# wolfbox/snappy

Measured on AMD Instinct MI355X. Metric: GiB/s hashed (whole node), bit-exact hashes.yaml, 10k x 1 MiB tree, higher is better.
Workload: dtype u64; 1 GPU; C2: ONE on-disk tree (tmpfs) of 10001 files (10 000 x 1 MiB + the 1 MiB archive stand-in) -> hashes.yaml, sharded over 1 rank(s) on 1 distinct GPU(s); bytes=10486808576, kernel=sha512_split_kernel<true>, tree_home=/dev/shm

## Files before the change

### snappy_amd/csrc/hostfill.cpp

```cpp
#include "hostfill.h"

#include <new>

#include <ctype.h>
#include <dirent.h>
#include <errno.h>
#include <sched.h>
#include <stdio.h>
#include <string.h>
#include <sys/syscall.h>
#include <unistd.h>

#include <algorithm>
#include <atomic>

#if defined(__x86_64__)
#include <immintrin.h>
#endif

namespace snaphash {

namespace {

bool read_small_file(const std::string& path, std::string& out)
{
    FILE* f = fopen(path.c_str(), "r");
    if (!f) return false;
    char buf[4096];
    out.clear();
    size_t r;
    while ((r = fread(buf, 1, sizeof buf, f)) > 0) out.append(buf, r);
    fclose(f);
    return true;
}

constexpr int kMpolDefault = 0, kMpolPreferred = 1;
constexpr unsigned kMpolFNode = 1u << 0, kMpolFAddr = 1u << 1;

}

std::vector<int> parse_cpulist(const std::string& text)
{
    std::vector<int> out;
    const char* p = text.c_str();
    while (*p) {
        while (*p && !isdigit((unsigned char)*p)) ++p;
        if (!*p) break;
        char* end = nullptr;
        const long a = strtol(p, &end, 10);
        long b = a;
        p = end;
        if (*p == '-') { b = strtol(p + 1, &end, 10); p = end; }
        if (a < 0 || b < a || b - a > 65536) break;
        for (long c = a; c <= b; ++c) out.push_back((int)c);
    }
    return out;
}

int numa_node_of_pci(const std::string& sysfs_root, const std::string& bdf_in)
{
    std::string bdf = bdf_in;
    for (char& c : bdf) c = (char)tolower((unsigned char)c);
    if (bdf.empty()) return -1;
    std::string text;
    if (!read_small_file(sysfs_root + "/bus/pci/devices/" + bdf + "/numa_node", text)) return -1;
    char* end = nullptr;
    const long v = strtol(text.c_str(), &end, 10);
    if (end == text.c_str()) return -1;
    return v < 0 ? -1 : (int)v;
}

std::vector<int> numa_cpus_of_node(const std::string& sysfs_root, int node)
{
    std::string text;
    if (node < 0 || !read_small_file(sysfs_root + "/devices/system/node/node" + std::to_string(node) + "/cpulist", text)) return {};
    return parse_cpulist(text);
}

std::vector<int> slice_cpus(const std::vector<int>& all, size_t pos, size_t m)
{
    if (m < 2 || pos >= m) return all;
    std::vector<int> mine;
    for (size_t a = 0; a < all.size();) {
        size_t b = a + 1;
        while (b < all.size() && all[b] == all[b - 1] + 1) ++b;
        const size_t len = b - a;
        for (size_t i = a + len * pos / m; i < a + len * (pos + 1) / m; ++i) mine.push_back(all[i]);
        a = b;
    }
    return mine;
}

int numa_node_count(const std::string& sysfs_root)
{
    int n = 0;
    if (DIR* d = opendir((sysfs_root + "/devices/system/node").c_str())) {
        while (struct dirent* de = readdir(d))
            if (!strncmp(de->d_name, "node", 4) && isdigit((unsigned char)de->d_name[4])) ++n;
        closedir(d);
    }
    return n;
}

bool numa_prefer_node(int node, SavedMemPolicy* saved)
{
#if defined(SYS_set_mempolicy) && defined(SYS_get_mempolicy)
    if (node < 0 || node >= 1024) return false;
    saved->valid = syscall(SYS_get_mempolicy, &saved->mode, saved->mask, (unsigned long)1024 + 1, nullptr, 0ul) == 0;
    unsigned long mask[1024 / (8 * sizeof(unsigned long))] = {0};
    mask[(size_t)node / (8 * sizeof(unsigned long))] |= 1ul << ((size_t)node % (8 * sizeof(unsigned long)));
    return syscall(SYS_set_mempolicy, kMpolPreferred, mask, (unsigned long)1024 + 1) == 0;
#else
    (void)node; (void)saved;
    return false;
#endif
}

void numa_restore_policy(const SavedMemPolicy& saved)
{
#if defined(SYS_set_mempolicy)
    if (saved.valid && saved.mode != kMpolDefault &&
        syscall(SYS_set_mempolicy, saved.mode, saved.mask, (unsigned long)1024 + 1) == 0)
        return;
    (void)syscall(SYS_set_mempolicy, kMpolDefault, nullptr, 0ul);
#else
    (void)saved;
#endif
}

int numa_node_of_address(const void* addr)
{
#if defined(SYS_get_mempolicy)
    int node = -1;
    if (syscall(SYS_get_mempolicy, &node, nullptr, 0ul, addr, (unsigned long)(kMpolFNode | kMpolFAddr)) != 0) return -1;
    return node;
#else
    (void)addr;
    return -1;
#endif
}

unsigned cgroup_cpu_quota(const std::string& sysfs_cgroup_root, const std::string& proc_self_cgroup)
{
    std::string text;
    if (!read_small_file(proc_self_cgroup, text)) return 0;
    double best = 0;
    auto take = [&](double quota, double period) {
        if (quota > 0 && period > 0) { const double c = quota / period; if (best == 0 || c < best) best = c; }
    };
    size_t pos = 0;
    while (pos < text.size()) {
        size_t eol = text.find('\n', pos);
        if (eol == std::string::npos) eol = text.size();
        const std::string line = text.substr(pos, eol - pos);
        pos = eol + 1;
        const size_t c1 = line.find(':'), c2 = c1 == std::string::npos ? c1 : line.find(':', c1 + 1);
        if (c2 == std::string::npos) continue;
        const std::string ctrl = line.substr(c1 + 1, c2 - c1 - 1);
        std::string path = line.substr(c2 + 1);
        const bool v2 = ctrl.empty();
        if (!v2) {
            bool has_cpu = false;
            for (size_t a = 0; a <= ctrl.size();) {
                size_t b = ctrl.find(',', a);
                if (b == std::string::npos) b = ctrl.size();
                if (ctrl.compare(a, b - a, "cpu") == 0) has_cpu = true;
                a = b + 1;
            }
            if (!has_cpu) continue;
        }
        const std::string base = sysfs_cgroup_root + (v2 ? "" : "/" + ctrl);
        for (;;) {
            std::string v;
            if (v2) {
                if (read_small_file(base + path + "/cpu.max", v) && v.compare(0, 3, "max") != 0) {
                    char* end = nullptr;
                    const double q = strtod(v.c_str(), &end);
                    const double per = end ? strtod(end, nullptr) : 0;
                    take(q, per);
                }
            } else {
                std::string pv;
                if (read_small_file(base + path + "/cpu.cfs_quota_us", v) && read_small_file(base + path + "/cpu.cfs_period_us", pv))
                    take(strtod(v.c_str(), nullptr), strtod(pv.c_str(), nullptr));
            }
            if (path.empty() || path == "/") break;
            const size_t slash = path.rfind('/');
            path = slash == 0 || slash == std::string::npos ? "/" : path.substr(0, slash);
        }
    }
    if (best <= 0) return 0;
    return (unsigned)std::max(1.0, best + 0.5);
}

unsigned usable_cpus()
{
    unsigned n = 0;
    cpu_set_t set;
    CPU_ZERO(&set);
    if (sched_getaffinity(0, sizeof set, &set) == 0) {
        const int c = CPU_COUNT(&set);
        if (c > 0) n = (unsigned)c;
    }
    if (n == 0) n = std::max(1u, std::thread::hardware_concurrency());
    static const unsigned quota = cgroup_cpu_quota("/sys/fs/cgroup", "/proc/self/cgroup");
    if (quota && quota < n) n = quota;
    return n;
}


FillPool::~FillPool() { stop(); }

void FillPool::stop()
{
    {
        std::lock_guard<std::mutex> lk(mu_);
        quit_ = true;
    }
    cv_work_.notify_all();
    for (auto& t : th_) if (t.joinable()) t.join();
    th_.clear();
    quit_ = false;
}

void FillPool::configure(unsigned max_threads, const std::vector<int>& cpus)
{
    stop();
    max_threads_ = max_threads;
    cpus_ = cpus;
}

void FillPool::worker(unsigned id)
{
    if (!cpus_.empty()) {
        cpu_set_t set, allowed;
        CPU_ZERO(&set);
        CPU_ZERO(&allowed);
        const bool have_allowed = sched_getaffinity(0, sizeof allowed, &allowed) == 0;
        for (int c : cpus_)
            if (c >= 0 && c < CPU_SETSIZE && (!have_allowed || CPU_ISSET(c, &allowed))) CPU_SET(c, &set);
        if (CPU_COUNT(&set) > 0) (void)sched_setaffinity(0, sizeof set, &set);
    }
    uint64_t seen = 0;
    for (;;) {
        const std::function<void(size_t)>* fn;
        size_t n;
        std::atomic<size_t>* next;
        {
            std::unique_lock<std::mutex> lk(mu_);
            cv_work_.wait(lk, [&] { return quit_ || (epoch_ != seen && id < want_); });
            if (quit_) return;
            seen = epoch_;
            fn = fn_; n = n_; next = next_;
        }
        try {
            for (;;) {
                const size_t i = next->fetch_add(1);
                if (i >= n) break;
                (*fn)(i);
            }
        } catch (...) {
            fn_threw_.store(true);
        }
        {
            std::lock_guard<std::mutex> lk(mu_);
            if (--running_ == 0) cv_done_.notify_all();
        }
    }
}

void FillPool::parallel_for(size_t n, unsigned threads, const std::function<void(size_t)>& fn)
{
    if (n == 0) return;
    unsigned helpers = threads > 1 ? std::min(threads - 1, max_threads_) : 0u;
    if (helpers > n - 1) helpers = (unsigned)(n - 1);
    std::atomic<size_t> next{0};
    if (helpers) {
        std::lock_guard<std::mutex> lk(mu_);
        try {
            while (th_.size() < helpers) { const unsigned id = (unsigned)th_.size(); th_.emplace_back(&FillPool::worker, this, id); }
        } catch (...) {
            helpers = (unsigned)th_.size();
        }
        if (helpers) {
            fn_ = &fn; n_ = n; next_ = &next;
            want_ = helpers;
            running_ = helpers;
            ++epoch_;
        }
    }
    if (helpers) cv_work_.notify_all();
    bool threw = false;
    try {
        for (;;) {
            const size_t i = next.fetch_add(1);
            if (i >= n) break;
            fn(i);
        }
    } catch (...) {
        threw = true;
        next.store(n);
    }
    if (helpers) {
        std::unique_lock<std::mutex> lk(mu_);
        cv_done_.wait(lk, [&] { return running_ == 0; });
        want_ = 0;
        fn_ = nullptr; next_ = nullptr;
    }
    if (fn_threw_.exchange(false) || threw) throw std::bad_alloc();
}


void run_on_threads(unsigned T, const std::function<void(unsigned)>& fn)
{
    if (T <= 1) { fn(0); return; }
    static std::mutex mu;
    static FillPool* pool = [] {
        FillPool* p = new FillPool();
        p->configure(64, {});
        return p;
    }();
    static const pid_t born_in = getpid();
    if (T <= 65 && getpid() == born_in && mu.try_lock()) {
        std::lock_guard<std::mutex> lk(mu, std::adopt_lock);
        pool->parallel_for(T, T, [&fn](size_t t) { fn((unsigned)t); });
        return;
    }
    ThreadJoiner th;
    for (unsigned t = 1; t < T; ++t) th.spawn(fn, t);
    fn(0);
    th.join_all();
}


#if defined(__x86_64__)
namespace {
__attribute__((target("avx2"))) void copy_nt_avx2(uint8_t* dst, const uint8_t* src, size_t n)
{
    const size_t head = (64 - ((uintptr_t)dst & 63)) & 63;
    if (head) { memcpy(dst, src, head); dst += head; src += head; n -= head; }
    size_t lines = n / 64;
    while (lines--) {
        const __m256i a = _mm256_loadu_si256((const __m256i*)src);
        const __m256i b = _mm256_loadu_si256((const __m256i*)(src + 32));
        _mm256_stream_si256((__m256i*)dst, a);
        _mm256_stream_si256((__m256i*)(dst + 32), b);
        src += 64; dst += 64;
    }
    n &= 63;
    if (n) memcpy(dst, src, n);
    _mm_sfence();
}
const bool g_have_avx2 = __builtin_cpu_supports("avx2");
}
#endif

void copy_to_staging(void* dst, const void* src, size_t n)
{
#if defined(__x86_64__)
    if (n >= (32u << 10) && g_have_avx2) { copy_nt_avx2((uint8_t*)dst, (const uint8_t*)src, n); return; }
#endif
    memcpy(dst, src, n);
}

}
```

### snappy_amd/csrc/hostfill.h

```cpp
#pragma once
#include <stddef.h>
#include <stdint.h>

#include <atomic>
#include <condition_variable>
#include <functional>
#include <mutex>
#include <new>
#include <string>
#include <thread>
#include <vector>

namespace snaphash {

int numa_node_of_pci(const std::string& sysfs_root, const std::string& bdf);
std::vector<int> numa_cpus_of_node(const std::string& sysfs_root, int node);
std::vector<int> parse_cpulist(const std::string& text);
int numa_node_count(const std::string& sysfs_root);
std::vector<int> slice_cpus(const std::vector<int>& all, size_t pos, size_t m);

struct SavedMemPolicy {
    bool valid = false;
    int mode = 0;
    unsigned long mask[1024 / (8 * sizeof(unsigned long)) + 1] = {0};
};
bool numa_prefer_node(int node, SavedMemPolicy* saved);
void numa_restore_policy(const SavedMemPolicy& saved);
int numa_node_of_address(const void* addr);
unsigned usable_cpus();
unsigned cgroup_cpu_quota(const std::string& sysfs_cgroup_root, const std::string& proc_self_cgroup);

struct ThreadJoiner {
    std::vector<std::thread> th;
    std::atomic<bool> worker_threw{false};
    ThreadJoiner() = default;
    ThreadJoiner(const ThreadJoiner&) = delete;
    ThreadJoiner& operator=(const ThreadJoiner&) = delete;
    ~ThreadJoiner() { join_quietly(); }
    template <class F, class... A> void spawn(F&& f, A&&... a)
    {
        th.emplace_back([this](auto fn, auto... args) {
            try { fn(args...); } catch (...) { worker_threw.store(true); }
        }, std::forward<F>(f), std::forward<A>(a)...);
    }
    void join_quietly()
    {
        for (auto& t : th)
            if (t.joinable()) t.join();
    }
    void join_all()
    {
        join_quietly();
        if (worker_threw.exchange(false)) throw std::bad_alloc();
    }
};

class FillPool {
public:
    FillPool() = default;
    ~FillPool();
    FillPool(const FillPool&) = delete;
    FillPool& operator=(const FillPool&) = delete;
    void configure(unsigned max_threads, const std::vector<int>& cpus);
    void parallel_for(size_t n, unsigned threads, const std::function<void(size_t)>& fn);
    unsigned max_threads() const { return max_threads_; }
    const std::vector<int>& cpus() const { return cpus_; }

private:
    void worker(unsigned id);
    void stop();
    unsigned max_threads_ = 0;
    std::vector<int> cpus_;
    std::vector<std::thread> th_;
    std::mutex mu_;
    std::condition_variable cv_work_, cv_done_;
    uint64_t epoch_ = 0;
    unsigned want_ = 0;
    unsigned running_ = 0;
    bool quit_ = false;
    const std::function<void(size_t)>* fn_ = nullptr;
    std::atomic<bool> fn_threw_{false};
    size_t n_ = 0;
    std::atomic<size_t>* next_ = nullptr;
};

void run_on_threads(unsigned T, const std::function<void(unsigned)>& fn);

void copy_to_staging(void* dst, const void* src, size_t n);

}
```

### snappy_amd/csrc/hostpass.cpp

```cpp
#include "hostpass.h"

#include "hostfill.h"
#include "walk.h"

#include <dirent.h>
#include <errno.h>
#include <string.h>
#include <sys/stat.h>

#include <algorithm>
#include <string_view>
#include <functional>
#include <queue>
#include <thread>

namespace snaphash {


int mode_string(uint32_t st_mode, char out[11])
{
    memcpy(out, "----------", 11);
    if (S_ISDIR(st_mode)) out[0] = 'd';
    else if (S_ISLNK(st_mode)) out[0] = 'l';
    else if (S_ISREG(st_mode)) out[0] = 'f';
    else return SNAPHASH_EMODE;
    static const char rwx[] = "rwxrwxrwx";
    for (int i = 0; i < 9; ++i)
        if (st_mode & (1u << (8 - i))) out[i + 1] = rwx[i];
    return SNAPHASH_OK;
}

int mode_parse(const char* s, uint32_t* st_mode)
{
    if (!s || !s[0]) return SNAPHASH_EPARSE;
    uint32_t m;
    switch (s[0]) {
    case 'd': m = S_IFDIR; break;
    case 'f': m = S_IFREG; break;
    case 'l': m = S_IFLNK; break;
    default: return SNAPHASH_EPARSE;
    }
    static const char rwx[] = "rwxrwxrwx";
    for (int i = 0; i < 9 && s[i + 1]; ++i)
        if (s[i + 1] == rwx[i]) m |= 1u << (8 - i);
    *st_mode = m;
    return SNAPHASH_OK;
}


static int records_from_entries_impl(std::vector<WalkEntry>& ents, std::vector<Record>& out, bool steal)
{
    if (ents.empty()) return SNAPHASH_OK;
    const size_t rootlen = ents[0].path.size();
    const size_t n = ents.size();
    const unsigned T = (unsigned)std::max<size_t>(1, std::min<size_t>(std::min(8u, usable_cpus()), n / 2048));
    std::vector<uint8_t> keep(n, 0);
    std::vector<size_t> kept(T + 1, 0), bad(T, n);
    auto range = [&](unsigned t, size_t& lo, size_t& hi) { lo = n * t / T; hi = n * (t + 1) / T; };
    run_on_threads(T, [&](unsigned t) {
        size_t lo, hi, c = 0;
        range(t, lo, hi);
        for (size_t i = lo; i < hi; ++i) {
            const char* rel = ents[i].path.c_str() + rootlen;
            if (rel[0] == 0 || strncmp(rel, "/DEBIAN", 7) == 0) continue;
            char m[11];
            if (mode_string(ents[i].st.st_mode, m) != SNAPHASH_OK) { bad[t] = i; break; }
            keep[i] = 1;
            ++c;
        }
        kept[t + 1] = c;
    });
    size_t first_bad = n;
    for (unsigned t = 0; t < T; ++t) first_bad = std::min(first_bad, bad[t]);
    if (first_bad < n) return SNAPHASH_EMODE;
    for (unsigned t = 0; t < T; ++t) kept[t + 1] += kept[t];
    const size_t base = out.size();
    out.resize(base + kept[T]);
    run_on_threads(T, [&](unsigned t) {
        size_t lo, hi;
        range(t, lo, hi);
        size_t at = base + kept[t];
        for (size_t i = lo; i < hi; ++i) {
            if (!keep[i]) continue;
            WalkEntry& e = ents[i];
            Record& r = out[at++];
            r.name.assign(e.path.c_str() + rootlen + 1, e.path.size() - rootlen - 1);
            r.st_mode = e.st.st_mode;
            r.is_regular = S_ISREG(e.st.st_mode);
            r.size = r.is_regular ? (int64_t)e.st.st_size : 0;
            if (steal) r.path = std::move(e.path);
            else r.path = e.path;
        }
    });
    return SNAPHASH_OK;
}

size_t first_unemittable_name(const std::vector<Record>& recs)
{
    const size_t n = recs.size();
    const unsigned T = (unsigned)std::max<size_t>(1, std::min<size_t>(std::min(8u, usable_cpus()), n / 2048));
    std::vector<size_t> bad(T, n);
    run_on_threads(T, [&](unsigned t) {
        for (size_t i = n * t / T; i < n * (t + 1) / T; ++i)
            if (!name_emittable(recs[i].name)) { bad[t] = i; break; }
    });
    size_t first = n;
    for (size_t b : bad) first = std::min(first, b);
    return first;
}

int records_from_entries(const std::vector<WalkEntry>& ents, std::vector<Record>& out)
{
    return records_from_entries_impl(const_cast<std::vector<WalkEntry>&>(ents), out, false);
}

int walk_tree(const char* build_dir, std::vector<Record>& out, int* err_no)
{
    std::vector<WalkEntry> ents;
    int e = 0;
    const int wrc = walk_entries(build_dir, ents, &e, nullptr);
    if (err_no) *err_no = e;
    const int rc = records_from_entries_impl(ents, out, true);
    if (rc) return rc;
    return wrc ? SNAPHASH_EIO : SNAPHASH_OK;
}


bool plain_safe_name(const std::string& s)
{
    if (s.empty() || s.size() > 72) return false;
    bool alpha = false;
    for (unsigned char c : s) {
        const bool ok = (c >= 'a' && c <= 'z') || (c >= 'A' && c <= 'Z') || (c >= '0' && c <= '9') || c == '_' ||
                        c == '.' || c == '/' || c == '-' || c == '+';
        if (!ok) return false;
        if ((c >= 'a' && c <= 'z') || (c >= 'A' && c <= 'Z')) alpha = true;
    }
    const unsigned char c0 = s[0];
    if (c0 == '-' || c0 == '.' || c0 == '+' || (c0 >= '0' && c0 <= '9')) return false;
    if (!alpha) return false;
    static const char* const resolved[] = {"y", "Y", "yes", "Yes", "YES", "on", "On", "ON", "n", "N", "no", "No", "NO",
                                           "off", "Off", "OFF", "true", "True", "TRUE", "false", "False", "FALSE",
                                           "null", "Null", "NULL", nullptr};
    if (s.size() <= 5)
        for (int i = 0; resolved[i]; ++i)
            if (s == resolved[i]) return false;
    return true;
}

void hex_lower(const uint8_t d[64], char out[128])
{
    static const char x[] = "0123456789abcdef";
    for (int i = 0; i < 64; ++i) { out[2 * i] = x[d[i] >> 4]; out[2 * i + 1] = x[d[i] & 15]; }
}

static int emit_records(const std::vector<Record>& recs, size_t lo, size_t hi, const uint8_t* file_digests, std::string& out,
                        std::vector<size_t>* hex_at = nullptr)
{
    char hex[128], num[32];
    size_t fi = 0;
    if (hex_at) memset(hex, '0', sizeof hex);
    for (size_t k = lo; k < hi; ++k) {
        const Record& r = recs[k];
        char mode[11];
        int rc = mode_string(r.st_mode, mode);
        if (rc) return rc;
        out += "- name:";
        if (plain_safe_name(r.name)) { out += ' '; out += r.name; }
        else if ((rc = yaml_append_name_scalar(r.name, 7, 4, out)) != SNAPHASH_OK) return rc;
        out += '\n';
        if (r.is_regular) {
            snprintf(num, sizeof num, "%lld", (long long)r.size);
            out += "  size: "; out += num; out += '\n';
            if (!hex_at) hex_lower(file_digests + 64 * fi++, hex);
            out += "  sha512: ";
            if (hex_at) hex_at->push_back(out.size());
            out.append(hex, 128); out += '\n';
        }
        out += "  mode: "; out.append(mode, 10); out += '\n';
    }
    return SNAPHASH_OK;
}

static int emit_yaml_impl(const std::vector<Record>& recs, const uint8_t* archive_digest, const uint8_t* file_digests,
                          std::string& out, std::vector<size_t>* hex_at, unsigned max_threads = 8)
{
    char hex[128];
    out.clear();
    out.reserve(64 + recs.size() * 220);
    if (hex_at) { hex_at->clear(); memset(hex, '0', sizeof hex); }
    else hex_lower(archive_digest, hex);
    out += "archive-sha512: ";
    if (hex_at) hex_at->push_back(out.size());
    out.append(hex, 128);
    out += '\n';
    if (recs.empty()) {
        out += "files: []\n";
        return SNAPHASH_OK;
    }
    out += "files:\n";
    const unsigned T = (unsigned)std::max<size_t>(1, std::min<size_t>(std::min(std::max(1u, max_threads), usable_cpus()), recs.size() / 1024));
    if (T <= 1) return emit_records(recs, 0, recs.size(), file_digests, out, hex_at);
    std::vector<size_t> first_digest(T + 1, 0);
    {
        size_t fi = 0;
        for (unsigned t = 0; t < T; ++t) {
            first_digest[t] = fi;
            for (size_t k = recs.size() * t / T; k < recs.size() * (t + 1) / T; ++k) fi += recs[k].is_regular ? 1 : 0;
        }
    }
    std::vector<std::string> piece(T);
    std::vector<std::vector<size_t>> piece_at(hex_at ? T : 0);
    std::vector<int> prc(T, 0);
    auto work = [&](unsigned t) {
        const size_t lo = recs.size() * t / T, hi = recs.size() * (t + 1) / T;
        piece[t].reserve((hi - lo) * 220);
        prc[t] = emit_records(recs, lo, hi, file_digests ? file_digests + 64 * first_digest[t] : nullptr, piece[t], hex_at ? &piece_at[t] : nullptr);
    };
    run_on_threads(T, work);
    for (unsigned t = 0; t < T; ++t) {
        if (prc[t]) return prc[t];
        if (hex_at)
            for (size_t at : piece_at[t]) hex_at->push_back(out.size() + at);
        out += piece[t];
    }
    return SNAPHASH_OK;
}

int emit_yaml(const std::vector<Record>& recs, const uint8_t archive_digest[64], const uint8_t* file_digests,
              std::string& out)
{
    return emit_yaml_impl(recs, archive_digest, file_digests, out, nullptr);
}

int emit_yaml_skeleton(const std::vector<Record>& recs, YamlSkeleton& sk, unsigned max_threads)
{
    return emit_yaml_impl(recs, nullptr, nullptr, sk.text, &sk.hex_at, max_threads);
}

void yaml_fill_digests(YamlSkeleton& sk, const uint8_t archive_digest[64], const uint8_t* file_digests)
{
    if (sk.hex_at.empty()) return;
    hex_lower(archive_digest, &sk.text[sk.hex_at[0]]);
    const size_t n = sk.hex_at.size() - 1;
    const unsigned T = (unsigned)std::max<size_t>(1, std::min<size_t>(std::min(8u, usable_cpus()), n / 2048));
    auto work = [&](unsigned t) {
        for (size_t i = n * t / T; i < n * (t + 1) / T; ++i) hex_lower(file_digests + 64 * i, &sk.text[sk.hex_at[i + 1]]);
    };
    run_on_threads(T, work);
}


namespace {
constexpr uint32_t kListMagic = 0x4c504e53u;
struct BlobOut {
    std::string b;
    void u32(uint32_t v) { b.append((const char*)&v, 4); }
    void u64(uint64_t v) { b.append((const char*)&v, 8); }
};
struct BlobIn {
    const uint8_t* p;
    size_t n, at = 0;
    bool ok = true;
    uint32_t u32() { uint32_t v = 0; if (at + 4 > n) { ok = false; return 0; } memcpy(&v, p + at, 4); at += 4; return v; }
    uint64_t u64() { uint64_t v = 0; if (at + 8 > n) { ok = false; return 0; } memcpy(&v, p + at, 8); at += 8; return v; }
    const char* bytes(size_t k) { if (k > n - at || at > n) { ok = false; return nullptr; } const char* r = (const char*)p + at; at += k; return r; }
};
bool list_root(const std::string& root, std::vector<std::string>& names)
{
    names.clear();
    DIR* d = opendir(root.c_str());
    if (!d) return false;
    while (struct dirent* de = readdir(d)) {
        if (!strcmp(de->d_name, ".") || !strcmp(de->d_name, "..")) continue;
        names.emplace_back(de->d_name);
    }
    closedir(d);
    std::sort(names.begin(), names.end());
    return true;
}
uint64_t hash_names(const std::vector<std::string>& names)
{
    uint64_t h = 0x9E3779B97F4A7C15ull;
    for (const std::string& s : names)
        for (size_t i = 0; i <= s.size(); ++i) { h = (h ^ (uint8_t)(i < s.size() ? s[i] : 0)) * 0xFF51AFD7ED558CCDull; h ^= h >> 29; }
    return h;
}
}


int shard_listing(const char* build_dir, uint32_t rank, uint32_t world, std::string& blob, int* err_no)
{
    if (err_no) *err_no = 0;
    std::string root(build_dir);
    while (root.size() > 1 && root.back() == '/') root.pop_back();
    struct stat rst;
    if (lstat(root.c_str(), &rst) != 0) { if (err_no) *err_no = errno; return SNAPHASH_EIO; }
    std::vector<std::string> top;
    if (S_ISDIR(rst.st_mode)) (void)list_root(root, top);
    std::vector<uint32_t> mine;
    for (size_t i = 0; i < top.size(); ++i)
        if (i % world == rank) mine.push_back((uint32_t)i);
    std::vector<std::vector<WalkEntry>> sub(mine.size());
    std::vector<int> sub_rc(mine.size(), 0), sub_errno(mine.size(), 0);
    const unsigned T = (unsigned)std::max<size_t>(1, std::min<size_t>(std::min(16u, usable_cpus()), mine.size()));
    std::atomic<size_t> next{0};
    run_on_threads(T, [&](unsigned) {
        for (;;) {
            const size_t k = next.fetch_add(1);
            if (k >= mine.size()) return;
            const std::string& name = top[mine[k]];
            if (name.compare(0, 6, "DEBIAN") == 0) continue;
            sub_rc[k] = walk_entries((root + "/" + name).c_str(), sub[k], &sub_errno[k], nullptr);
        }
    });
    for (size_t k = 0; k < mine.size(); ++k)
        if (sub_rc[k]) { if (err_no) *err_no = sub_errno[k]; return SNAPHASH_EIO; }
    BlobOut o;
    o.u32(kListMagic); o.u32(1); o.u32(world); o.u32(rank); o.u32((uint32_t)top.size()); o.u32((uint32_t)mine.size());
    o.u64(hash_names(top));
    const size_t cut = root.size() + 1;
    for (size_t k = 0; k < mine.size(); ++k) {
        o.u32(mine[k]);
        o.u32((uint32_t)sub[k].size());
        for (const WalkEntry& e : sub[k]) {
            o.u32((uint32_t)e.st.st_mode);
            o.u32((uint32_t)(e.path.size() - cut));
            o.u64(S_ISREG(e.st.st_mode) ? (uint64_t)e.st.st_size : 0);
            o.b.append(e.path, cut, std::string::npos);
        }
    }
    blob.swap(o.b);
    return SNAPHASH_OK;
}

int records_from_listings(const char* build_dir, uint32_t world, const void* const* blobs, const size_t* blob_lens, std::vector<Record>& recs)
{
    std::string root(build_dir);
    while (root.size() > 1 && root.back() == '/') root.pop_back();
    struct Piece { uint32_t r = 0; size_t at = 0; uint32_t n = 0; bool have = false; };
    std::vector<Piece> piece;
    uint32_t n_top = 0;
    uint64_t names_hash = 0;
    for (uint32_t r = 0; r < world; ++r) {
        if (!blobs[r] && blob_lens[r]) return SNAPHASH_EINVAL;
        BlobIn in{(const uint8_t*)blobs[r], blob_lens[r]};
        const uint32_t magic = in.u32(), version = in.u32(), w = in.u32(), rk = in.u32(), nt = in.u32(), nm = in.u32();
        const uint64_t nh = in.u64();
        if (!in.ok || magic != kListMagic || version != 1 || w != world || rk != r) return SNAPHASH_EPARSE;
        if (r == 0) {
            if (nt > (1u << 26)) return SNAPHASH_EPARSE;
            n_top = nt; names_hash = nh; piece.assign(n_top, Piece());
        } else if (nt != n_top || nh != names_hash) return SNAPHASH_EMISMATCH;
        for (uint32_t k = 0; k < nm; ++k) {
            const uint32_t i = in.u32(), ne = in.u32();
            if (!in.ok || i >= n_top || i % world != r || piece[i].have) return SNAPHASH_EPARSE;
            piece[i].r = r; piece[i].at = in.at; piece[i].n = ne; piece[i].have = true;
            for (uint32_t e = 0; e < ne; ++e) {
                (void)in.u32();
                const uint32_t len = in.u32();
                (void)in.u64();
                (void)in.bytes(len);
                if (!in.ok) return SNAPHASH_EPARSE;
            }
        }
        if (in.at != in.n) return SNAPHASH_EPARSE;
    }
    std::vector<size_t> first(n_top + 1, 0);
    for (uint32_t i = 0; i < n_top; ++i) { if (!piece[i].have) return SNAPHASH_EPARSE; first[i + 1] = first[i] + piece[i].n; }
    const size_t total = first[n_top];
    recs.clear();
    recs.resize(total);
    const unsigned T = (unsigned)std::max<size_t>(1, std::min<size_t>({(size_t)std::min(8u, usable_cpus()), total / 1024, (size_t)n_top}));
    std::vector<int> trc(T, SNAPHASH_OK);
    std::vector<size_t> tbad(T, (size_t)-1);
    run_on_threads(T, [&](unsigned t) {
        for (uint32_t i = (uint32_t)((uint64_t)n_top * t / T); i < (uint32_t)((uint64_t)n_top * (t + 1) / T); ++i) {
            BlobIn in{(const uint8_t*)blobs[piece[i].r], blob_lens[piece[i].r]};
            in.at = piece[i].at;
            for (uint32_t e = 0; e < piece[i].n; ++e) {
                const uint32_t mode = in.u32(), len = in.u32();
                const uint64_t size = in.u64();
                const char* name = in.bytes(len);
                int rc = SNAPHASH_OK;
                char m[11];
                if (!in.ok || len == 0 || memchr(name, 0, len)) rc = SNAPHASH_EPARSE;
                else if (mode_string(mode, m) != SNAPHASH_OK) rc = SNAPHASH_EMODE;
                if (rc) { trc[t] = rc; tbad[t] = first[i] + e; return; }
                Record& r = recs[first[i] + e];
                r.name.assign(name, len);
                r.path.reserve(root.size() + 1 + len);
                r.path = root;
                r.path += '/';
                r.path.append(name, len);
                r.st_mode = mode;
                r.is_regular = S_ISREG(mode);
                r.size = r.is_regular ? (int64_t)size : 0;
            }
        }
    });
    size_t bad = (size_t)-1;
    int rc = SNAPHASH_OK;
    for (unsigned t = 0; t < T; ++t)
        if (trc[t] && tbad[t] < bad) { bad = tbad[t]; rc = trc[t]; }
    if (rc) recs.clear();
    return rc;
}


namespace {

int hexval(int c)
{
    if (c >= '0' && c <= '9') return c - '0';
    if (c >= 'a' && c <= 'f') return c - 'a' + 10;
    if (c >= 'A' && c <= 'F') return c - 'A' + 10;
    return -1;
}

bool parse_scalar(const std::string& v, std::string& out)
{
    out.clear();
    if (v.empty()) return true;
    if (v[0] == '\'') {
        size_t i = 1;
        for (; i < v.size(); ++i) {
            if (v[i] == '\'') {
                if (i + 1 < v.size() && v[i + 1] == '\'') { out += '\''; ++i; continue; }
                break;
            }
            out += v[i];
        }
        return i < v.size();
    }
    if (v[0] == '"') {
        size_t i = 1;
        for (; i < v.size() && v[i] != '"'; ++i) {
            if (v[i] != '\\') { out += v[i]; continue; }
            if (++i >= v.size()) return false;
            switch (v[i]) {
            case 'n': out += '\n'; break;
            case 't': out += '\t'; break;
            case 'r': out += '\r'; break;
            case '0': out += '\0'; break;
            case 'a': out += '\a'; break;
            case 'b': out += '\b'; break;
            case 'e': out += '\x1b'; break;
            case 'f': out += '\f'; break;
            case 'v': out += '\v'; break;
            case ' ': out += ' '; break;
            case '"': out += '"'; break;
            case '/': out += '/'; break;
            case '\\': out += '\\'; break;
            case 'N': out += "\xC2\x85"; break;
            case '_': out += "\xC2\xA0"; break;
            case 'L': out += "\xE2\x80\xA8"; break;
            case 'P': out += "\xE2\x80\xA9"; break;
            case 'x': case 'u': case 'U': {
                const int nd = v[i] == 'x' ? 2 : (v[i] == 'u' ? 4 : 8);
                if (i + nd >= v.size()) return false;
                uint32_t cp = 0;
                for (int k = 0; k < nd; ++k) {
                    const int h = hexval(v[i + 1 + k]);
                    if (h < 0) return false;
                    cp = cp * 16 + h;
                }
                i += nd;
                if (cp < 0x80) out += (char)cp;
                else if (cp < 0x800) { out += (char)(0xC0 | (cp >> 6)); out += (char)(0x80 | (cp & 63)); }
                else if (cp < 0x10000) { out += (char)(0xE0 | (cp >> 12)); out += (char)(0x80 | ((cp >> 6) & 63)); out += (char)(0x80 | (cp & 63)); }
                else { out += (char)(0xF0 | (cp >> 18)); out += (char)(0x80 | ((cp >> 12) & 63)); out += (char)(0x80 | ((cp >> 6) & 63)); out += (char)(0x80 | (cp & 63)); }
                break;
            }
            default: return false;
            }
        }
        return i < v.size();
    }
    std::string p = v;
    size_t h = p.find(" #");
    if (h != std::string::npos) p.resize(h);
    while (!p.empty() && (p.back() == ' ' || p.back() == '\t' || p.back() == '\r')) p.pop_back();
    out = p;
    return true;
}

bool split_key(const std::string& line, size_t from, std::string& key, std::string& val)
{
    size_t c = line.find(':', from);
    if (c == std::string::npos) return false;
    key = line.substr(from, c - from);
    size_t v = c + 1;
    while (v < line.size() && line[v] == ' ') ++v;
    val = line.substr(v);
    while (!val.empty() && (val.back() == '\r' || val.back() == ' ')) val.pop_back();
    return true;
}

bool unhex64(const std::string& s, uint8_t out[64])
{
    if (s.size() != 128) return false;
    for (int i = 0; i < 64; ++i) {
        const int a = hexval(s[2 * i]), b = hexval(s[2 * i + 1]);
        if (a < 0 || b < 0) return false;
        out[i] = (uint8_t)(a * 16 + b);
    }
    return true;
}

}

namespace {

int parse_lines(const std::vector<std::string_view>& lines, size_t lo, size_t hi, bool in_files_at_start, ParsedHashes& out, bool* top_level)
{
    bool in_files = in_files_at_start;
    int skip_indent = -1;
    ParsedRecord* cur = nullptr;
    auto indent_of = [](std::string_view l) { size_t k = 0; while (k < l.size() && l[k] == ' ') ++k; return k; };
    std::string line;
    std::string key, val, sv;
    for (size_t li = lo; li < hi; ++li) {
        line.assign(lines[li].data(), lines[li].size());
        while (!line.empty() && (line.back() == '\r')) line.pop_back();
        size_t ind = 0;
        while (ind < line.size() && line[ind] == ' ') ++ind;
        if (in_files && (skip_indent < 0 || (int)ind <= skip_indent) && ind < line.size() && line[ind] != '#') {
            const size_t key_col = line[ind] == '-' ? ind + 2 : ind;
            const size_t colon = line.find(": ", ind);
            if (colon != std::string::npos && colon + 2 < line.size()) {
                while (li + 1 < hi) {
                    std::string_view nx = lines[li + 1];
                    while (!nx.empty() && (nx.back() == '\r' || nx.back() == ' ')) nx.remove_suffix(1);
                    const size_t ni = indent_of(nx);
                    if (nx.empty() || ni <= key_col) break;
                    while (!line.empty() && line.back() == ' ') line.pop_back();
                    line += ' ';
                    line.append(nx.data() + ni, nx.size() - ni);
                    ++li;
                }
            }
        }
        if (ind == line.size() || line[ind] == '#') continue;
        if (line == "---" || line == "...") continue;
        if (skip_indent >= 0) {
            if ((int)ind > skip_indent) continue;
            skip_indent = -1;
        }
        if (ind == 0 && line[0] != '-') {
            if (top_level) *top_level = true;
// ... 157 lines not shown
```

### snappy_amd/csrc/hostpass.h

```cpp
#pragma once
#include <stdint.h>
#include <stdio.h>

#include <string>
#include <vector>

#include "../../include/snaphash.h"

namespace snaphash {

struct Record {
    std::string name;
    std::string path;
    uint32_t st_mode = 0;
    bool is_regular = false;
    int64_t size = 0;
    std::string sha512_hex;
};

struct ParsedRecord {
    std::string name, sha512_hex;
    int64_t size = 0;
    uint32_t st_mode = 0;
    bool has_name = false, has_size = false, has_mode = false;
};
struct ParsedHashes {
    bool has_archive = false;
    std::string archive_hex;
    std::vector<ParsedRecord> files;
};

int mode_string(uint32_t st_mode, char out[11]);
int mode_parse(const char* s, uint32_t* st_mode);
int walk_tree(const char* build_dir, std::vector<Record>& out, int* err_no);
struct WalkEntry;
int records_from_entries(const std::vector<WalkEntry>& ents, std::vector<Record>& out);
bool plain_safe_name(const std::string& s);
int yaml_append_name_scalar(const std::string& s, int column, int indent, std::string& out);
bool name_emittable(const std::string& s);
size_t first_unemittable_name(const std::vector<Record>& recs);
void hex_lower(const uint8_t d[64], char out[128]);
int emit_yaml(const std::vector<Record>& recs, const uint8_t archive_digest[64], const uint8_t* file_digests,
              std::string& out);
struct YamlSkeleton {
    std::string text;
    std::vector<size_t> hex_at;
};
int emit_yaml_skeleton(const std::vector<Record>& recs, YamlSkeleton& out, unsigned max_threads = 8 );
void yaml_fill_digests(YamlSkeleton& sk, const uint8_t archive_digest[64], const uint8_t* file_digests);
int shard_listing(const char* build_dir, uint32_t rank, uint32_t world, std::string& blob, int* err_no);
int records_from_listings(const char* build_dir, uint32_t world, const void* const* blobs, const size_t* blob_lens, std::vector<Record>& recs);
int parse_yaml(const char* text, size_t len, ParsedHashes& out);
bool digest_matches_hex(const uint8_t d[64], const std::string& hex);
int lpt_assign(const uint64_t* lens, size_t n, int nshards, int32_t* shard_of);

}
```

### snappy_amd/csrc/snapbuild.inc

```

namespace {

constexpr uint32_t kSnapBuildOptionsSizeV1 = 16;

struct SnapBuildTemps {
    std::string data, control;
    ~SnapBuildTemps()
    {
        if (!data.empty()) (void)unlink(data.c_str());
        if (!control.empty()) (void)unlink(control.c_str());
    }
};

struct SnapOut {
    int fd = -1;
    HostSha sha;
    uint64_t bytes = 0;
    ~SnapOut() { if (fd >= 0) close(fd); }
    int put(const uint8_t* p, size_t n)
    {
        host_sha512_update(sha, p, n);
        bytes += n;
        size_t off = 0;
        while (off < n) {
            const ssize_t w = write(fd, p + off, n - off);
            if (w < 0) { if (errno == EINTR) continue; return errno; }
            off += (size_t)w;
        }
        return 0;
    }
};

int snap_put_member(snaphash_ctx* x, SnapOut& out, const char* name, int64_t mtime, const uint8_t* data, uint64_t size, const char* path)
{
    int fd = -1;
    struct FdGuard { int& fd; ~FdGuard() { if (fd >= 0) close(fd); } } guard{fd};
    if (path) {
        fd = open(path, O_RDONLY | O_CLOEXEC);
        struct stat sb;
        if (fd < 0 || fstat(fd, &sb) != 0) return fail(x, SNAPHASH_EIO, std::string(path) + ": " + strerror(errno));
        size = (uint64_t)sb.st_size;
    }
    uint8_t h[kArHeader];
    int rc = ar_header(name, mtime, 0100644, size, h);
    if (rc) return fail(x, rc, std::string("ar: member ") + name + " does not fit a header");
    int en = out.put(h, sizeof h);
    if (!en && !path && size) en = out.put(data, (size_t)size);
    if (!en && path) {
        std::vector<uint8_t> buf(4u << 20);
        uint64_t got = 0;
        while (got < size && !en) {
            const ssize_t r = read(fd, buf.data(), (size_t)std::min<uint64_t>(buf.size(), size - got));
            if (r < 0 && errno == EINTR) continue;
            if (r <= 0) return fail(x, SNAPHASH_EIO, std::string(path) + ": " + (r < 0 ? strerror(errno) : "shorter than it was"));
            en = out.put(buf.data(), (size_t)r);
            got += (uint64_t)r;
        }
    }
    if (!en && (size & 1)) en = out.put((const uint8_t*)"\n", 1);
    if (en) return fail(x, SNAPHASH_EIO, std::string("writing the container: ") + strerror(en));
    return SNAPHASH_OK;
}

struct SnapDataMember {
    Encoder& enc;
    const char* name;
    const uint64_t& check_units;
    const double& check_ms;
};

int snap_build_impl(snaphash_ctx* x, const char* source_dir, const char* snap_path, uint32_t flags, int64_t mtime, uint8_t* archive_digest,
                    uint8_t* snap_digest, snaphash_snap_build_stats& st, const SnapDataMember& dm)
{
    const double t0 = now_ms();
    const bool hashes = !(flags & SNAPHASH_BUILD_NO_HASHES);
    SnapBuildTemps tmp;
    SnapOut out;
    out.fd = open(snap_path, O_WRONLY | O_CREAT | O_TRUNC | O_CLOEXEC, 0666);
    if (out.fd < 0) return fail(x, SNAPHASH_EIO, std::string(snap_path) + ": " + strerror(errno));
    host_sha512_init(out.sha);
    tmp.data = std::string(snap_path) + "." + dm.name;
    tmp.control = std::string(snap_path) + ".control.tar.gz";
    const std::string debian = go_clean(std::string(source_dir) + "/DEBIAN");

    GzCheck chk_control;
    chk_control.member = "control.tar.gz";
    const bool check = (flags & SNAPHASH_BUILD_CHECK) != 0;
    uint8_t adig[64];
    char* yaml = nullptr;
    size_t yaml_len = 0;
    struct Free { char*& p; ~Free() { free(p); } } free_yaml{yaml};
    GzipEncoder enc_control(check ? &chk_control : nullptr);
    int rc = tar_create_impl(x, dm.enc, tmp.data.c_str(), source_dir, debian.c_str(), nullptr, nullptr, hashes ? &yaml : nullptr, &yaml_len, adig);
    if (rc) return rc;
    st.data_ms = x->targz.wall_ms;
    st.tar_bytes = x->targz.tar_bytes;
    st.members = x->targz.members;
    st.data_bytes = x->targz.gz_bytes;
    if (hashes) {
        rc = write_yaml_file(x, source_dir, std::string(yaml, yaml_len));
        if (rc) return rc;
    }
    rc = tar_create_impl(x, enc_control, tmp.control.c_str(), debian.c_str(), nullptr, nullptr, nullptr, nullptr, nullptr, nullptr);
    if (rc) return rc;
    st.control_ms = x->targz.wall_ms;
    st.control_bytes = x->targz.gz_bytes;
    st.check_chunks = dm.check_units + chk_control.chunks;
    st.check_ms = dm.check_ms + chk_control.ms;

    const double t_ar = now_ms();
    const int en = out.put((const uint8_t*)kArMagic, 8);
    if (en) return fail(x, SNAPHASH_EIO, std::string(snap_path) + ": " + strerror(en));
    rc = snap_put_member(x, out, "debian-binary", mtime, (const uint8_t*)"2.0\n", 4, nullptr);
    if (!rc) rc = snap_put_member(x, out, "_click-binary", mtime, (const uint8_t*)"0.4\n", 4, nullptr);
    if (!rc) rc = snap_put_member(x, out, "control.tar.gz", mtime, nullptr, 0, tmp.control.c_str());
    if (!rc) rc = snap_put_member(x, out, dm.name, mtime, nullptr, 0, tmp.data.c_str());
    if (rc) return rc;
    const int fd = out.fd;
    out.fd = -1;
    if (close(fd) != 0) return fail(x, SNAPHASH_EIO, std::string(snap_path) + ": " + strerror(errno));
    uint8_t sdig[64];
    host_sha512_final(out.sha, sdig);
    if (snap_digest) memcpy(snap_digest, sdig, 64);
    if (archive_digest) memcpy(archive_digest, adig, 64);
    st.snap_bytes = out.bytes;
    st.ar_ms = now_ms() - t_ar;
    st.wall_ms = now_ms() - t0;
    return SNAPHASH_OK;
}

}

extern "C" {

int snaphash_snap_build(snaphash_ctx* x, const char* source_dir, const char* snap_path, const snaphash_snap_build_options* opt,
                        uint8_t* archive_digest, uint8_t* snap_digest, snaphash_snap_build_stats* stats)
try {
    if (!x || !source_dir || !snap_path || !*snap_path) return fail(x, SNAPHASH_EINVAL, "bad argument");
    static_assert(offsetof(snaphash_snap_build_options, data_codec) == kSnapBuildOptionsSizeV1, "the codec and its options behind the 16 bytes");
    if (opt && opt->struct_size != kSnapBuildOptionsSizeV1 && opt->struct_size < sizeof(snaphash_snap_build_options))
        return fail(x, SNAPHASH_EINVAL, "snaphash_snap_build_options.struct_size");
    if (stats && stats->struct_size < sizeof(snaphash_snap_build_stats)) return fail(x, SNAPHASH_EINVAL, "snaphash_snap_build_stats.struct_size");
    const uint32_t flags = opt ? opt->flags : 0;
    if (flags & ~(uint32_t)(SNAPHASH_BUILD_NO_HASHES | SNAPHASH_BUILD_CHECK)) return fail(x, SNAPHASH_EINVAL, "unknown build flag");
    const int64_t mtime = (opt && opt->mtime >= 0) ? opt->mtime : (int64_t)time(nullptr);
    uint32_t codec = SNAPHASH_DATA_GZ;
    const snaphash_xz_options* xo = nullptr;
    const snaphash_bz2_options* bo = nullptr;
    if (opt && opt->struct_size >= sizeof(snaphash_snap_build_options)) {
        codec = opt->data_codec;
        xo = opt->xz;
        bo = opt->bz2;
        if (codec > SNAPHASH_DATA_XZ) return fail(x, SNAPHASH_EINVAL, "snap build: data_codec is 0 (gz), 1 (bz2) or 2 (xz)");
        if (opt->reserved) return fail(x, SNAPHASH_EINVAL, "snap build: snaphash_snap_build_options.reserved is not 0");
        if ((xo && codec != SNAPHASH_DATA_XZ) || (bo && codec != SNAPHASH_DATA_BZ2))
            return fail(x, SNAPHASH_EINVAL, "snap build: options for a codec that is not data_codec");
    }
    const bool check = (flags & SNAPHASH_BUILD_CHECK) != 0;
    snaphash_snap_build_stats st{};
    st.struct_size = sizeof st;
    auto build = [&](const SnapDataMember& dm) {
        const int rc = snap_build_impl(x, source_dir, snap_path, flags, mtime, archive_digest, snap_digest, st, dm);
        if (rc) (void)unlink(snap_path);
        if (stats) *stats = st;
        return rc;
    };
    if (codec == SNAPHASH_DATA_XZ) {
        uint64_t bs;
        uint32_t chk, filter, level;
        bool self;
        int rc = xz_read_options(x, xo, &bs, &chk, &self, &filter, &level);
        if (rc) return rc;
        XzSelfCheck sc;
        sc.member = "data.tar.xz";
        XzEncoder enc(bs, chk, (self || check) ? &sc : nullptr, filter, level);
        rc = build(SnapDataMember{enc, "data.tar.xz", sc.chunks, sc.ms});
        xz_keep_selfcheck_stats(x, sc);
        xz_keep_filter_stats(x, enc);
        return rc;
    }
    if (codec == SNAPHASH_DATA_BZ2) {
        uint32_t level;
        bool self;
        int rc = bz2_read_options(x, bo, &level, &self);
        if (rc) return rc;
        BzSelfCheck sc;
        sc.member = "data.tar.bz2";
        BzEncoder enc(level, (self || check) ? &sc : nullptr);
        rc = build(SnapDataMember{enc, "data.tar.bz2", sc.blocks, sc.ms});
        bz2_keep_selfcheck_stats(x, sc);
        return rc;
    }
    GzCheck chk_data;
    chk_data.member = "data.tar.gz";
    GzipEncoder enc(check ? &chk_data : nullptr);
    return build(SnapDataMember{enc, "data.tar.gz", chk_data.chunks, chk_data.ms});
} catch (...) {
    if (snap_path) (void)unlink(snap_path);
    return SNAPHASH_ENOMEM;
}

int snaphash_deflate_check_device(snaphash_ctx* x, const void* d_in, size_t n_in, const void* d_z, const uint64_t* z_off, size_t nchunks,
                                  int last_is_final, snaphash_deflate_verdict* verdicts)
try {
    static_assert(sizeof(snaphash_deflate_verdict) == sizeof(DfCheckVerdict), "the verdicts travel as they are");
    if (!x || !z_off || !verdicts || nchunks == 0 || nchunks > 0x7fffffffu || (n_in && !d_in) || (uint64_t)nchunks * kDfCheckChunk < n_in)
        return fail(x, SNAPHASH_EINVAL, "bad argument");
    for (size_t i = 0; i < nchunks; ++i)
        if (z_off[i] > z_off[i + 1]) return fail(x, SNAPHASH_EINVAL, "z_off descends");
    if (z_off[nchunks] && !d_z) return fail(x, SNAPHASH_EINVAL, "bad argument");
    TOP_ENTER(x);
    DevCtx* c = x->d0();
    HIP_TRY(c, hipSetDevice(c->device));
    DevBuf<uint64_t> d_off;
    DevBuf<DfCheckVerdict> d_v;
    HIP_TRY(c, d_off.reserve(nchunks + 1));
    HIP_TRY(c, d_v.reserve(nchunks));
    HIP_TRY(c, hipMemcpyAsync(d_off.data(), z_off, (nchunks + 1) * 8, hipMemcpyHostToDevice, c->stream));
    HIP_TRY(c, hipMemsetAsync(d_v.data(), 0xff, nchunks * sizeof(DfCheckVerdict), c->stream));
    HIP_TRY(c, launch_deflate_check((const uint8_t*)d_in, n_in, (const uint8_t*)d_z, z_off[nchunks], d_off.data(), nullptr, 0, (uint32_t)nchunks,
                                    (uint32_t)nchunks, last_is_final != 0, d_v.data(), c->stream));
    HIP_TRY(c, hipMemcpyAsync(verdicts, d_v.data(), nchunks * sizeof(DfCheckVerdict), hipMemcpyDeviceToHost, c->stream));
    HIP_TRY(c, hipStreamSynchronize(c->stream));
    x->stats.launches = 1;
    end_top(x, t_top0_);
    return SNAPHASH_OK;
} catch (...) {
    return SNAPHASH_ENOMEM;
}

}
```

### snappy_amd/csrc/snaphash_api.cpp

```cpp
#include <dirent.h>
#include <errno.h>
#include <fcntl.h>
#include <hip/hip_runtime.h>
#include <string.h>
#include <sys/resource.h>
#include <sys/stat.h>
#include <time.h>
#include <unistd.h>

#include <algorithm>
#include <atomic>
#include <queue>
#include <chrono>
#include <string>
#include <thread>
#include <unordered_map>
#include <vector>

#include <dlfcn.h>
#include <rccl/rccl.h>

#include <condition_variable>
#include <functional>
#include <future>
#include <memory>
#include <mutex>

#include "batchplan.h"
#include "engine_bufs.h"
#include "gpu_handles.h"
#include "hostfill.h"
#include "hostpass.h"
#include "hostsha.h"
#include "inflate_host.h"
#include "member_hashers.h"
#include "planner.h"
#include "sha512_core.h"
#include "sha512_kernels.h"
#include "snap_core.h"
#include "tarpack.h"
#include "walk.h"

using namespace snaphash;

namespace {

constexpr uint64_t kDefaultStaging = 256ull << 20;

double now_ms()
{
    using namespace std::chrono;
    return duration<double, std::milli>(steady_clock::now().time_since_epoch()).count();
}

}

struct snaphash_ctx;

struct DevCtx {
    int device = 0;
    int index = 0;
    Stream stream;
    Stream copy_stream;
    uint64_t staging = kDefaultStaging;
    uint32_t kernel_pref = SNAPHASH_KERNEL_AUTO;
    uint32_t deflate_depth = 0;
    uint32_t n_xcd = 8;

    std::vector<SubSlot> sub;
    Slot slot[3];
    HashBufs hash;
    Twin<CmpChunk> cmp;
    DeflateBufs z;
    Stream z_stream;
    Stream z2_stream;
    std::vector<Event> z_ev;
    std::vector<Event> z_part_ev;
    InflateBufs inf;
    Bzip2Bufs bz;
    CrcBufs crc;
    Sha256Bufs sha256;
    BcjBufs bcj;
    Event bcj_ev[2];
    hipStream_t bcj_busy = nullptr;
    XzBufs xz;
    XzEncBufs xe;
    BzEncBufs be;
    Stream f_stream;
    uint64_t fout_gen = 0;

    EventLedger ledger;
    bool pending = false;

    std::string pci_bus_id;
    int numa_node = -1;
    int staging_node = -1;
    int64_t fd_budget = 0;
    int64_t fd_call_budget = -1;
    unsigned fill_cap = 12;
    unsigned fill_call_cap = 0;
    snaphash_ctx* owner = nullptr;
    unsigned owner_cpus_per_engine = 0;
    uint64_t staged_calls = 0;
    double fill_thread_s = 0;
    uint64_t fill_bytes = 0;
    FillPool pool;

    snaphash_stats stats{};
    double t_call0 = 0;
    std::string last_error;

    template <class F> void each_buf(F&& f)
    {
        for (Slot& s : slot) s.each(f);
        for (SubSlot& q : sub) q.jobs.each(f);
        hash.each(f);
        cmp.each(f);
        z.each(f);
        inf.each(f);
        bz.each(f);
        crc.each(f);
        sha256.each(f);
        bcj.each(f);
        xz.each(f);
        xe.each(f);
        be.each(f);
    }
};

namespace {
struct Rccl {
    void* lib = nullptr;
    bool tried = false, ok = false;
    std::string why;
    ncclResult_t (*CommInitAll)(ncclComm_t*, int, const int*) = nullptr;
    ncclResult_t (*CommDestroy)(ncclComm_t) = nullptr;
    ncclResult_t (*AllGather)(const void*, void*, size_t, ncclDataType_t, ncclComm_t, hipStream_t) = nullptr;
    ncclResult_t (*GroupStart)() = nullptr;
    ncclResult_t (*GroupEnd)() = nullptr;
    const char* (*GetErrorString)(ncclResult_t) = nullptr;
    std::vector<ncclComm_t> comms;
};
}

struct snaphash_batch;

struct snaphash_ctx {
    std::vector<std::unique_ptr<DevCtx>> dev;
    uint32_t host_threads = 0;
    bool gpu_only = false;
    unsigned cpus = 1;
    unsigned cpus_call = 0;
    double host_rate = 1.4e9;
    PlanCalib calib;
    std::mutex calib_mu;
    uint32_t flags = 0;
    Rccl rccl;
    std::vector<DevBuf<uint8_t>> d_gather;
    snaphash_stats stats{};
    snaphash_stats_ex ex{};
    snaphash_targz_stats targz{};
    snaphash_unpack_stats unpack{};
    snaphash_xz_check_stats xz_check{};
    snaphash_xz_selfcheck_stats xz_selfcheck{};
    snaphash_xz_filter_stats xz_filter{};
    bool unxz_bcj = false;
    snaphash_bz2_selfcheck_stats bz2_selfcheck{};
    snaphash_block_scan_stats block_scan{};
    std::string last_error;
    snaphash_batch* open_batch = nullptr;
    DevCtx* d0() const { return dev[0].get(); }
};

namespace {

int fail(DevCtx* c, int code, const std::string& msg)
{
    if (c) c->last_error = msg;
    return code;
}
int fail(snaphash_ctx* x, int code, const std::string& msg)
{
    if (x) x->last_error = msg;
    return code;
}
int lift(snaphash_ctx* x, DevCtx* c, int rc)
{
    if (rc && x && c) x->last_error = c->last_error;
    return rc;
}
unsigned call_cpus(const snaphash_ctx* x) { return std::max(1u, x->cpus_call ? x->cpus_call : x->cpus); }
#define HIP_TRY(c, expr)                                                                             \
    do {                                                                                             \
        hipError_t e_ = (expr);                                                                      \
        if (e_ != hipSuccess)                                                                        \
            return fail(c, (e_ == hipErrorOutOfMemory) ? SNAPHASH_ENOMEM : SNAPHASH_EDEVICE,         \
                        std::string(#expr) + ": " + hipGetErrorString(e_));                          \
    } while (0)

int span_take(DevCtx* c, Ev kind, Span* sp)
{
    return c->ledger.take(kind, sp) == hipSuccess ? SNAPHASH_OK : fail(c, SNAPHASH_EDEVICE, "hipEventCreate failed");
}
int span_begin(DevCtx* c, Ev kind, hipStream_t s, Span* sp)
{
    if (int rc = span_take(c, kind, sp)) return rc;
    HIP_TRY(c, hipEventRecord(sp->a, s));
    return SNAPHASH_OK;
}
int span_end(DevCtx* c, const Span& sp, hipStream_t s)
{
    HIP_TRY(c, hipEventRecord(sp.b, s));
    return SNAPHASH_OK;
}
float span_ms(const Span& sp) { float ms = 0; return hipEventElapsedTime(&ms, sp.a, sp.b) == hipSuccess ? ms : 0; }
void scratch_spans_done(DevCtx* c) { c->ledger.clear(); }

SpanSums collect_events(DevCtx* c, bool hash_pass = true)
{
    static const bool trace = getenv("SNAPHASH_TRACE_EVENTS") != nullptr;
    const SpanSums sums = sum_spans(c->ledger, [](const Span& sp, float* ms) { return hipEventElapsedTime(ms, sp.a, sp.b) == hipSuccess; });
    c->stats.kernel_ms += sums.hash;
    c->stats.h2d_ms += sums.h2d;
    if (trace && hash_pass && c->ledger.used() > 1) {
        hipEvent_t first = nullptr;
        c->ledger.each([&](Ev kind, const Span& sp) {
            if (!first) first = sp.a;
            float t0 = 0, t1 = 0;
            (void)hipEventElapsedTime(&t0, first, sp.a);
            (void)hipEventElapsedTime(&t1, first, sp.b);
            fprintf(stderr, "snaphash engine %d: %s %7.2f .. %7.2f ms\n", c->index, kind == Ev::Hash ? "kernel" : kind == Ev::H2d ? "h2d   " : "other ", t0, t1);
        });
    }
    c->ledger.clear();
    return sums;
}

}

hipError_t snaphash::gpu_event_create(hipEvent_t* e, unsigned flags) { return flags == hipEventDefault ? hipEventCreate(e) : hipEventCreateWithFlags(e, flags); }
void snaphash::gpu_event_destroy(hipEvent_t e) { (void)hipEventDestroy(e); }
hipError_t snaphash::gpu_stream_create(hipStream_t* s, unsigned flags, int priority)
{
    return priority == kStreamDefaultPriority ? hipStreamCreateWithFlags(s, flags) : hipStreamCreateWithPriority(s, flags, priority);
}
void snaphash::gpu_stream_destroy(hipStream_t s) { (void)hipStreamDestroy(s); }

hipError_t snaphash::devbuf_alloc(Mem kind, void** p, size_t bytes, int numa_node)
{
    if (kind == Mem::Hbm) return hipMalloc(p, bytes);
    SavedMemPolicy saved;
    if (numa_node >= 0 && numa_prefer_node(numa_node, &saved)) {
        const hipError_t e = hipHostMalloc(p, bytes, hipHostMallocNumaUser);
        numa_restore_policy(saved);
        if (e == hipSuccess) return e;
        (void)hipGetLastError();
    }
    return hipHostMalloc(p, bytes, hipHostMallocDefault);
}

void snaphash::devbuf_free(Mem kind, void* p)
{
    if (kind == Mem::Hbm) (void)hipFree(p);
    else (void)hipHostFree(p);
}

namespace {

int ensure_slots(DevCtx* c, int nslots = 2, uint64_t want = 0)
{
    if (want == 0 || want > c->staging) want = c->staging;
    for (int k = 0; k < nslots; ++k) {
        Slot& s = c->slot[k];
        HIP_TRY(c, s.ensure(want, c->numa_node));
        if (c->staging_node < 0) { s.h_buf[0] = 0; c->staging_node = numa_node_of_address(s.h_buf.data()); }
        HIP_TRY(c, s.done.ensure(hipEventDisableTiming));
        HIP_TRY(c, s.copied.ensure(hipEventDisableTiming));
    }
    HIP_TRY(c, c->copy_stream.ensure(hipStreamNonBlocking));
    return SNAPHASH_OK;
}

constexpr size_t kSplitMaxStreams = 32768;
constexpr uint64_t kSplitMinBlocks = 32;

uint64_t job_blocks(const Job& j) { return (j.nbytes >> 7) + 1; }

hipError_t launch_kernel(uint32_t k, const Job* d_jobs, size_t n, DevCtx* c, uint8_t* d_digests, bool staged)
{
    if (k == SNAPHASH_KERNEL_QUAD) return launch_quad(d_jobs, (uint32_t)n, c->hash.d_state.data(), d_digests, c->stream);
    if (k == SNAPHASH_KERNEL_PAIR) return launch_pair(d_jobs, (uint32_t)n, c->hash.d_state.data(), d_digests, c->stream, staged);
    if (k == SNAPHASH_KERNEL_SPLIT) return launch_split(d_jobs, (uint32_t)n, c->hash.d_state.data(), d_digests, c->stream);
    return launch_wide(d_jobs, (uint32_t)n, c->hash.d_state.data(), d_digests, c->stream);
}

size_t plan_kernels(const DevCtx* c, const Job* h_jobs, size_t n, uint32_t* k_head, uint32_t* k_tail)
{
    *k_tail = SNAPHASH_KERNEL_WIDE;
    if (c->kernel_pref == SNAPHASH_KERNEL_WIDE || c->kernel_pref == SNAPHASH_KERNEL_SPLIT ||
        c->kernel_pref == SNAPHASH_KERNEL_PAIR || c->kernel_pref == SNAPHASH_KERNEL_QUAD) {
        *k_head = c->kernel_pref;
        return n;
    }
    *k_head = SNAPHASH_KERNEL_PAIR;
    uint64_t blocks = 0;
    for (size_t i = 0; i < n; ++i) blocks += job_blocks(h_jobs[i]);
    if (n <= kSplitMaxStreams) {
        if (blocks >= kSplitMinBlocks * n) return n;
        *k_head = SNAPHASH_KERNEL_WIDE;
        return n;
    }
    if (job_blocks(h_jobs[0]) >= 8 * job_blocks(h_jobs[kSplitMaxStreams - 1]) &&
        job_blocks(h_jobs[0]) >= kSplitMinBlocks) {
        size_t head = 0;
        while (head < kSplitMaxStreams && job_blocks(h_jobs[head]) >= kSplitMinBlocks) ++head;
        return head;
    }
    *k_head = SNAPHASH_KERNEL_WIDE;
    return n;
}

int launch_jobs(DevCtx* c, Job* h_jobs, Job* d_jobs, size_t n, uint8_t* d_digests, hipEvent_t copied = nullptr)
{
    if (n == 0) return SNAPHASH_OK;
    std::stable_sort(h_jobs, h_jobs + n, [](const Job& a, const Job& b) { return a.nbytes > b.nbytes; });
    if (copied) {
        HIP_TRY(c, hipMemcpyAsync(d_jobs, h_jobs, n * sizeof(Job), hipMemcpyHostToDevice, c->copy_stream));
        HIP_TRY(c, hipEventRecord(copied, c->copy_stream));
        HIP_TRY(c, hipStreamWaitEvent(c->stream, copied, 0));
    } else {
        HIP_TRY(c, hipMemcpyAsync(d_jobs, h_jobs, n * sizeof(Job), hipMemcpyHostToDevice, c->stream));
    }
    uint32_t k_head, k_tail;
    const size_t head = plan_kernels(c, h_jobs, n, &k_head, &k_tail);
    Span ev;
    if (int rc = span_begin(c, Ev::Hash, c->stream, &ev)) return rc;
    const bool staged = copied != nullptr;
    hipError_t e = launch_kernel(k_head, d_jobs, head, c, d_digests, staged);
    if (e == hipSuccess && head < n) e = launch_kernel(k_tail, d_jobs + head, n - head, c, d_digests, staged);
    if (e != hipSuccess) return fail(c, SNAPHASH_EDEVICE, std::string("kernel launch: ") + hipGetErrorString(e));
    if (int rc = span_end(c, ev, c->stream)) return rc;
    c->stats.launches += (head < n) ? 2 : 1;
    c->stats.kernel_used = k_head;
    c->pending = true;
    return SNAPHASH_OK;
}

int sync_ctx(DevCtx* c)
{
    if (!c->pending && c->ledger.used() == 0) return SNAPHASH_OK;
    if (c->copy_stream) HIP_TRY(c, hipStreamSynchronize(c->copy_stream));
    HIP_TRY(c, hipStreamSynchronize(c->stream));
    collect_events(c);
    c->pending = false;
    if (c->t_call0 > 0) { c->stats.wall_ms = now_ms() - c->t_call0; c->t_call0 = 0; }
    return SNAPHASH_OK;
}

void begin_call(DevCtx* c)
{
    c->stats = snaphash_stats{};
    c->t_call0 = now_ms();
    c->last_error.clear();
}


struct FdCache {
    std::vector<int> fd;
    std::atomic<int64_t> held{0};
    int64_t budget = 0;
    explicit FdCache(size_t n, int64_t b) : fd(n, -1), budget(b) {}
    ~FdCache() { for (int f : fd) if (f >= 0) close(f); }
    FdCache(const FdCache&) = delete;
    FdCache& operator=(const FdCache&) = delete;
};

int do_read_op(const Source& s, const ReadOp& op, FdCache* cache = nullptr)
{
    if (s.mem) { copy_to_staging(op.dst, s.mem + op.off, op.n); return 0; }
    int err = 0;
    int fd = cache ? cache->fd[op.src] : -1;
    bool cached = fd >= 0;
    if (fd < 0) {
        for (unsigned tries = 0;; ++tries) {
            fd = open(s.path, O_RDONLY | O_CLOEXEC);
            if (fd >= 0 || (errno != EMFILE && errno != ENFILE) || tries >= 2000) break;
            usleep(tries < 100 ? 200 : 2000);
        }
        if (fd < 0) err = errno;
        else if (cache && !op.to_eof && cache->held.load(std::memory_order_relaxed) < cache->budget) {
            cache->fd[op.src] = fd;
            cache->held.fetch_add(1, std::memory_order_relaxed);
            cached = true;
        }
    }
    uint64_t got = 0;
    while (!err && got < op.n) {
        ssize_t r = pread(fd, op.dst + got, op.n - got, (off_t)(op.off + got));
        if (r < 0) { if (errno == EINTR) continue; err = errno; }
        else if (r == 0) err = EIO;
        else got += (uint64_t)r;
    }
    if (!err && op.to_eof) {
        uint8_t probe;
        ssize_t r;
        do r = pread(fd, &probe, 1, (off_t)(op.off + op.n)); while (r < 0 && errno == EINTR);
        if (r > 0) err = EIO;
        else if (r < 0) err = errno;
    }
    if (fd >= 0 && (!cached || op.to_eof || err)) {
        close(fd);
        if (cached) { cache->fd[op.src] = -1; cache->held.fetch_sub(1, std::memory_order_relaxed); }
    }
    return err;
}

void run_reads(DevCtx* c, const std::vector<Source>& src, const std::vector<ReadOp>& ops, std::atomic<int>& first_err,
               std::atomic<int64_t>& first_err_src, FdCache* cache = nullptr, bool alone = false)
{
    static const int forced = [] {
        const char* e = getenv("SNAPHASH_COPY_THREADS");
        const int v = e ? atoi(e) : 0;
        return (v >= 1 && v <= 256) ? v : 0;
    }();
    const bool from_memory = !ops.empty() && src[ops[0].src].mem != nullptr;
    unsigned cap = forced ? (unsigned)forced : std::min(c->fill_cap, from_memory ? 6u : 12u);
    if (!forced && c->fill_call_cap) cap = std::min(cap, c->fill_call_cap);
    if (!forced && alone && !c->fill_call_cap && c->owner) cap = std::max(cap, std::min(c->fill_cap * 2u, c->owner_cpus_per_engine));
    const unsigned T = (unsigned)std::min<size_t>(cap, std::max<size_t>(1, ops.size() / 4));
    const double t_fill0 = now_ms();
    struct FillAccount {
        DevCtx* c; const std::vector<ReadOp>& ops; unsigned T; double t0;
        ~FillAccount()
        {
            uint64_t b = 0;
            for (const ReadOp& op : ops) b += op.n;
            c->fill_bytes += b;
            c->fill_thread_s += (now_ms() - t0) * 1e-3 * T;
        }
    } account{c, ops, T, t_fill0};
    c->pool.parallel_for(ops.size(), T, [&](size_t i) {
        if (first_err.load(std::memory_order_relaxed)) return;
        const ReadOp& op = ops[i];
        const int err = do_read_op(src[op.src], op, cache);
        if (err) {
            int z = 0;
            if (first_err.compare_exchange_strong(z, err)) first_err_src.store(op.src);
        }
    });
}

struct EngineSpans { float gpu = 0, copy_busy = 0, copy = 0; };
EngineSpans engine_spans(DevCtx* c)
{
    EngineSpans sp;
    if (c->copy_stream) (void)hipStreamSynchronize(c->copy_stream);
    (void)hipStreamSynchronize(c->stream);
    Span first_copy, last_copy, last_kernel, first;
    c->ledger.each([&](Ev kind, const Span& s) {
        if (!first.a) first = s;
        if (kind == Ev::H2d) {
            if (!first_copy.a) first_copy = s;
            last_copy = s;
            sp.copy_busy += span_ms(s);
        } else if (kind == Ev::Hash) last_kernel = s;
    });
    if (first_copy.a) {
        (void)hipEventElapsedTime(&sp.gpu, first_copy.a, (last_kernel.b ? last_kernel : first).b);
        (void)hipEventElapsedTime(&sp.copy, first_copy.a, last_copy.b);
    }
    return sp;
}

int hash_sources(DevCtx* c, const std::vector<Source>& src, uint8_t* digests, uint64_t* states, int* err_no,
                 int64_t* err_src)
{
    const size_t n = src.size();
    if (err_no) *err_no = 0;
    if (err_src) *err_src = -1;
    if (n == 0) return SNAPHASH_OK;
    HIP_TRY(c, hipSetDevice(c->device));
    uint64_t job_bytes = 0;
    bool empty_files = false;
    for (const Source& sc : src) { job_bytes += sc.gpu_len; empty_files |= sc.len == 0 && sc.path != nullptr; }
    const bool from_memory = src[0].mem != nullptr;
    const uint64_t slot_caps[3] = {c->slot[0].cap(), c->slot[1].cap(), c->slot[2].cap()};
    const BatchGeometry g = batch_geometry(job_bytes, n, c->staging, slot_caps, from_memory);
    int rc = ensure_slots(c, (int)g.nslots, g.slot_bytes);
    if (rc) return rc;
    HIP_TRY(c, c->hash.ensure(n, true));
    if (c->sub.size() < g.nsub) c->sub.resize(g.nsub);
    for (unsigned q = 0; q < g.nsub; ++q) {
        SubSlot& ss = c->sub[q];
        HIP_TRY(c, ss.done.ensure(hipEventDisableTiming));
        HIP_TRY(c, ss.copied.ensure(hipEventDisableTiming));
        ss.busy = false;
    }

    c->fill_thread_s = 0;
    c->fill_bytes = 0;
    BatchPlanner plan(src.data(), n, job_bytes, g.S_full, BatchKnobs::from_env());
    std::atomic<int> first_err{0};
    std::atomic<int64_t> first_err_src{-1};
    std::vector<ReadOp> ops;
    FdCache fds(from_memory ? 0 : n, c->fd_call_budget >= 0 ? std::min(c->fd_call_budget, c->fd_budget) : c->fd_budget);
    double t_wait = 0, t_plan = 0, t_read = 0, t_launch = 0;
    const double t_engine0 = now_ms();
    double t_first_copy = 0;
    size_t n_copies = 0;

    while (!plan.active.empty()) {
        const unsigned batch = plan.batch, q = batch % g.nsub;
        SubSlot& sl = c->sub[q];
        uint8_t* const sl_h = c->slot[q / g.per_slot].h_buf.data() + (uint64_t)(q % g.per_slot) * g.S_full;
        uint8_t* const sl_d = c->slot[q / g.per_slot].d_buf.data() + (uint64_t)(q % g.per_slot) * g.S_full;
        const double tb0 = now_ms();
        if (sl.busy) { HIP_TRY(c, hipEventSynchronize(sl.done)); sl.busy = false; }
        const double tb1 = now_ms();
        t_wait += tb1 - tb0;
        HIP_TRY(c, sl.jobs.ensure(plan.active.size()));
        const Batch b = plan.next(sl.jobs.h.data(), ops, (uint64_t)(uintptr_t)sl_h, (uint64_t)(uintptr_t)sl_d);
        c->stats.blocks += b.blocks;
        static const bool trace_batches = getenv("SNAPHASH_TRACE_BATCHES") != nullptr;
        if (trace_batches) trace_batch(stderr, c->index, batch, b, sl.jobs.h.data(), (uint64_t)(uintptr_t)sl_d, plan.active.size());
        if (empty_files)
            for (size_t k = 0; k < b.nj; ++k) {
                const Job& j = sl.jobs.h[k];
                if (j.nbytes == 0 && src[j.idx].len == 0 && src[j.idx].path) ops.push_back(ReadOp{j.idx, 0, 0, sl_h, true});
            }
        const double tb2 = now_ms();
        t_plan += tb2 - tb1;

        run_reads(c, src, ops, first_err, first_err_src, from_memory ? nullptr : &fds, batch == 0);
        if (first_err.load()) break;
        const double tb3 = now_ms();
        t_read += tb3 - tb2;
        if (trace_batches)
            fprintf(stderr, "snaphash engine %d: batch %u: at %.2f ms: waited %.2f, planned %.2f, filled %.2f ms (%zu streams begun, %.1f GB/s)\n", c->index, batch,
                    tb0 - t_engine0, tb1 - tb0, tb2 - tb1, tb3 - tb2, b.n_new, (double)b.used / ((tb3 - tb2) * 1e6 + 1e-9));

        if (b.used) {
            if (batch == 0) t_first_copy = now_ms() - t_engine0;
            ++n_copies;
            Span ev;
            if ((rc = span_begin(c, Ev::H2d, c->copy_stream, &ev))) return rc;
            HIP_TRY(c, hipMemcpyAsync(sl_d, sl_h, b.used, hipMemcpyHostToDevice, c->copy_stream));
            if ((rc = span_end(c, ev, c->copy_stream))) return rc;
        }
        rc = launch_jobs(c, sl.jobs.h.data(), sl.jobs.d.data(), b.nj, c->hash.d_digests.data(), sl.copied);
        if (rc) return rc;
        HIP_TRY(c, hipEventRecord(sl.done, c->stream));
        sl.busy = true;
        t_launch += now_ms() - tb3;
    }

    const double ts0 = now_ms();
    static const bool trace_tree = getenv("SNAPHASH_TRACE_TREE") != nullptr;
    const EngineSpans sp = trace_tree && c->ledger.used() > 1 ? engine_spans(c) : EngineSpans{};
    rc = sync_ctx(c);
    if (trace_tree)
        fprintf(stderr, "snaphash engine %d: %u batches; waiting for a slot %.1f ms, planning %.1f ms, reads %.1f ms, enqueue %.1f ms, drain %.1f ms; "
                        "first copy enqueued at %.2f ms, copies busy %.2f of %.2f ms, first copy -> last kernel %.2f ms, engine %.2f ms\n",
                c->index, plan.batch, t_wait, t_plan, t_read, t_launch, now_ms() - ts0, t_first_copy, sp.copy_busy, sp.copy, sp.gpu, now_ms() - t_engine0);
    for (SubSlot& ss : c->sub) ss.busy = false;
    if (rc) return rc;
    if (first_err.load()) {
        const int64_t s = first_err_src.load();
        if (err_no) *err_no = first_err.load();
        if (err_src) *err_src = s;
        return fail(c, SNAPHASH_EIO,
                    std::string(s >= 0 && src[s].path ? src[s].path : "<buffer>") + ": " + strerror(first_err.load()));
    }
    if (digests) HIP_TRY(c, hipMemcpy(digests, c->hash.d_digests.data(), n * 64, hipMemcpyDeviceToHost));
    if (states) HIP_TRY(c, hipMemcpy(states, c->hash.d_state.data(), n * 64, hipMemcpyDeviceToHost));
    for (size_t i = 0; i < n; ++i) c->stats.bytes_hashed += src[i].gpu_len;
    c->stats.streams = n;
    if (c->owner) {
        std::lock_guard<std::mutex> lk(c->owner->calib_mu);
        const double planned = c->owner->ex.planned_gpu_ms, took = now_ms() - t_engine0;
        const bool take_fill = c->staged_calls++ > 0 && !(planned > 0 && took > 3.0 * planned);
        c->owner->calib.observe_call(!from_memory, (double)c->fill_bytes, (double)n, (double)n_copies, c->stats.h2d_ms * 1e-3, c->fill_thread_s, take_fill);
    }
    return SNAPHASH_OK;
}


bool rccl_load(snaphash_ctx* x)
{
    Rccl& r = x->rccl;
    if (r.tried) return r.ok;
    r.tried = true;
    for (const char* name : {"librccl.so.1", "librccl.so", "/opt/rocm/lib/librccl.so.1"}) {
        r.lib = dlopen(name, RTLD_NOW | RTLD_LOCAL);
        if (r.lib) break;
    }
    if (!r.lib) { r.why = "librccl.so not found"; return false; }
    r.CommInitAll = (decltype(r.CommInitAll))dlsym(r.lib, "ncclCommInitAll");
    r.CommDestroy = (decltype(r.CommDestroy))dlsym(r.lib, "ncclCommDestroy");
    r.AllGather = (decltype(r.AllGather))dlsym(r.lib, "ncclAllGather");
    r.GroupStart = (decltype(r.GroupStart))dlsym(r.lib, "ncclGroupStart");
    r.GroupEnd = (decltype(r.GroupEnd))dlsym(r.lib, "ncclGroupEnd");
    r.GetErrorString = (decltype(r.GetErrorString))dlsym(r.lib, "ncclGetErrorString");
    if (!r.CommInitAll || !r.CommDestroy || !r.AllGather || !r.GroupStart || !r.GroupEnd) {
        r.why = "librccl.so lacks a required symbol";
        return false;
    }
    std::vector<int> devs;
    for (auto& d : x->dev) devs.push_back(d->device);
    std::vector<int> uniq = devs;
    std::sort(uniq.begin(), uniq.end());
    if (std::adjacent_find(uniq.begin(), uniq.end()) != uniq.end()) {
        r.why = "a device ordinal repeats in the ctx (RCCL needs one rank per GPU)";
        return false;
    }
    r.comms.assign(devs.size(), nullptr);
    const ncclResult_t e = r.CommInitAll(r.comms.data(), (int)devs.size(), devs.data());
    if (e != ncclSuccess) {
        r.why = std::string("ncclCommInitAll: ") + (r.GetErrorString ? r.GetErrorString(e) : "error");
        r.comms.clear();
        return false;
    }
    r.ok = true;
    return true;
}

int gather_digest_slabs(snaphash_ctx* x, const std::vector<size_t>& cnt, size_t kmax, std::vector<uint8_t>& rows)
{
    const size_t nd = x->dev.size();
    rows.assign(nd * kmax * 64, 0);
    const double t0 = now_ms();
    bool use_rccl = !(x->flags & SNAPHASH_FLAG_NO_RCCL) && rccl_load(x);
    if (use_rccl) {
        x->d_gather.resize(nd);
        for (size_t d = 0; d < nd; ++d) {
            DevCtx* c = x->dev[d].get();
            HIP_TRY(c, hipSetDevice(c->device));
            if (x->d_gather[d].reserve(nd * kmax * 64) != hipSuccess)
                return fail(x, SNAPHASH_ENOMEM, "hipMalloc of the gather buffer failed");
            HIP_TRY(x, c->hash.ensure(kmax, true));
        }
        Rccl& r = x->rccl;
        ncclResult_t e = r.GroupStart();
        for (size_t d = 0; d < nd && e == ncclSuccess; ++d) {
            DevCtx* c = x->dev[d].get();
            (void)hipSetDevice(c->device);
            e = r.AllGather(c->hash.d_digests.data(), x->d_gather[d].data(), kmax * 64, ncclUint8, r.comms[d], c->stream);
        }
        const ncclResult_t e2 = r.GroupEnd();
        if (e == ncclSuccess) e = e2;
        if (e != ncclSuccess) {
            r.ok = false;
            r.why = std::string("RCCL all-gather: ") + (r.GetErrorString ? r.GetErrorString(e) : "error");
            use_rccl = false;
        }
    }
    if (use_rccl) {
        Rccl& r = x->rccl;
        (void)r;
        for (size_t d = 0; d < nd; ++d) {
            DevCtx* c = x->dev[d].get();
            HIP_TRY(c, hipSetDevice(c->device));
            HIP_TRY(c, hipStreamSynchronize(c->stream));
        }
        DevCtx* c0 = x->d0();
        HIP_TRY(c0, hipSetDevice(c0->device));
        HIP_TRY(c0, hipMemcpy(rows.data(), x->d_gather[0].data(), nd * kmax * 64, hipMemcpyDeviceToHost));
        x->ex.gather_kind = 1;
        if (x->flags & SNAPHASH_FLAG_CHECK_GATHER) {
            std::vector<uint8_t> own(kmax * 64);
            for (size_t d = 0; d < nd; ++d) {
                DevCtx* c = x->dev[d].get();
                HIP_TRY(c, hipSetDevice(c->device));
                if (cnt[d]) HIP_TRY(c, hipMemcpy(own.data(), c->hash.d_digests.data(), cnt[d] * 64, hipMemcpyDeviceToHost));
                if (memcmp(own.data(), rows.data() + d * kmax * 64, cnt[d] * 64) != 0)
                    return fail(x, SNAPHASH_EDEVICE, "RCCL-gathered digest slab differs from the device's own copy");
            }
            x->ex.gather_checked = 1;
        }
    } else {
        for (size_t d = 0; d < nd; ++d) {
            DevCtx* c = x->dev[d].get();
            HIP_TRY(c, hipSetDevice(c->device));
            if (cnt[d]) HIP_TRY(c, hipMemcpy(rows.data() + d * kmax * 64, c->hash.d_digests.data(), cnt[d] * 64, hipMemcpyDeviceToHost));
        }
        x->ex.gather_kind = 2;
    }
    x->ex.gather_ms = now_ms() - t0;
    return SNAPHASH_OK;
}


double measure_host_rate()
{
    static std::mutex mu;
    static double smoothed = 0;
    std::vector<uint8_t> buf(512u << 10, 0x5a);
    HostSha hs;
    uint8_t out[64];
    double rate[5];
    int n = 0;
    for (int rep = 0; rep < 5; ++rep) {
        host_sha512_init(hs);
        const double t0 = now_ms();
        host_sha512_update(hs, buf.data(), buf.size());
        host_sha512_final(hs, out);
        const double dt = (now_ms() - t0) * 1e-3;
        if (dt > 0) rate[n++] = (double)buf.size() / dt;
    }
    if (n == 0) return 0.40e9;
    std::sort(rate, rate + n);
    const double median = rate[n / 2];
    if (!(median > 50e6)) return 0.40e9;
    std::lock_guard<std::mutex> lk(mu);
    smoothed = smoothed > 0 ? 0.75 * smoothed + 0.25 * median : median;
    return smoothed;
}

int64_t open_descriptors()
{
    DIR* d = opendir("/proc/self/fd");
    if (!d) return 0;
    int64_t n = 0;
    while (struct dirent* e = readdir(d))
        if (e->d_name[0] != '.') ++n;
    closedir(d);
    return n > 0 ? n - 1 : 0;
}

PlanModel plan_model_of(const snaphash_ctx* x, bool from_files)
{
    PlanModel m;
    m.n_devices = (unsigned)x->dev.size();
    m.cpus = call_cpus(x);
    m.fill_threads = std::min(x->d0()->fill_cap, from_files ? 12u : 6u);
    if (x->cpus_call) m.fill_threads = std::max(1u, std::min(m.fill_threads, x->cpus_call > 2u ? x->cpus_call - 1u : 1u));
    if (host_sha512_x8_available()) m.host_lane_gain = from_files ? 2.4 : 3.2;
    m.host_threads = x->host_threads;
    m.from_files = from_files;
    m.host_rate = from_files ? x->host_rate * 0.9 : x->host_rate;
    {
        std::lock_guard<std::mutex> lk(const_cast<snaphash_ctx*>(x)->calib_mu);
        x->calib.apply(m);
    }
    return m;
}


void merge_stats(snaphash_ctx* x)
{
    snaphash_stats t{};
    for (auto& d : x->dev) {
        const snaphash_stats& s = d->stats;
        t.bytes_hashed += s.bytes_hashed;
        t.blocks += s.blocks;
        t.streams += s.streams;
        t.launches += s.launches;
        if (s.launches) t.kernel_used = s.kernel_used;
        t.kernel_ms = std::max(t.kernel_ms, s.kernel_ms);
        t.h2d_ms = std::max(t.h2d_ms, s.h2d_ms);
    }
    x->ex.gpu_bytes = t.bytes_hashed;
    t.bytes_hashed += x->ex.host_bytes;
    t.streams += x->ex.host_streams;
    t.wall_ms = x->stats.wall_ms;
    x->stats = t;
}

void begin_top(snaphash_ctx* x)
{
    x->stats = snaphash_stats{};
    x->ex = snaphash_stats_ex{};
    x->ex.struct_size = sizeof(snaphash_stats_ex);
    x->ex.n_devices = (uint32_t)x->dev.size();
    x->last_error.clear();
    for (auto& d : x->dev) { begin_call(d.get()); d->t_call0 = 0; }
}

bool keep_on_device_planned(const snaphash_ctx* x, size_t nd) { return nd > 1 || (x->flags & SNAPHASH_FLAG_FORCE_GATHER); }

int hash_sources_top(snaphash_ctx* x, std::vector<Source>& src, uint8_t* digests, int32_t* status, int64_t* bad_out = nullptr)
{
    if (bad_out) *bad_out = -1;
    const size_t n = src.size();
    if (status) for (size_t i = 0; i < n; ++i) status[i] = 0;
    if (n == 0) return SNAPHASH_OK;
    const size_t nd = x->dev.size();
    for (Source& s : src) s.gpu_len = s.len;
    std::vector<uint8_t> on_host(n, 0);
    unsigned plan_threads = 0;
    const double t_hash0 = now_ms();
    struct HashClock {
        snaphash_ctx* x; double t0;
        ~HashClock() { x->ex.hash_ms = now_ms() - t0; }
    } hash_clock{x, t_hash0};
    if (!x->gpu_only) {
        std::vector<uint64_t> lens(n);
        for (size_t i = 0; i < n; ++i) lens[i] = src[i].len;
        PlanResult plan = plan_streams(lens.data(), n, plan_model_of(x, src[0].path != nullptr));
        on_host.swap(plan.on_host);
        plan_threads = plan.host_threads;
        x->ex.planned_gpu_ms = plan.gpu_seconds * 1e3;
        x->ex.planned_host_ms = plan.host_seconds * 1e3;
        x->ex.planned_threads = plan.host_threads;
        x->ex.plan_ms = now_ms() - t_hash0;
    }

    std::vector<uint32_t> gidx;
    std::vector<uint32_t> hidx;
    for (size_t i = 0; i < n; ++i) (on_host[i] ? hidx : gidx).push_back((uint32_t)i);
    std::vector<std::vector<uint32_t>> member(nd);
    if (nd == 1) {
        member[0] = gidx;
    } else {
        std::vector<uint64_t> lens(gidx.size());
        for (size_t k = 0; k < gidx.size(); ++k) lens[k] = src[gidx[k]].len;
        std::vector<int32_t> shard(gidx.size());
        if (!gidx.empty()) lpt_assign(lens.data(), lens.size(), (int)nd, shard.data());
        for (size_t k = 0; k < gidx.size(); ++k) member[shard[k]].push_back(gidx[k]);
    }

    if (keep_on_device_planned(x, nd)) {
        size_t kmax = 1;
        for (size_t d = 0; d < nd; ++d) kmax = std::max(kmax, member[d].size());
        for (size_t d = 0; d < nd; ++d) {
            DevCtx* c = x->dev[d].get();
            HIP_TRY(c, hipSetDevice(c->device));
            HIP_TRY(x, c->hash.ensure(kmax, true));
        }
    }
    struct DevJob { std::vector<Source> sub; std::vector<uint8_t> dig; int rc = 0, err_no = 0; int64_t err_src = -1; };
    std::vector<DevJob> job(nd);
    const bool keep_on_device = nd > 1 || (x->flags & SNAPHASH_FLAG_FORCE_GATHER);
    std::vector<double> gbusy(nd, 0.0);
    auto run_dev = [&](size_t d) {
        const double tg0 = now_ms();
        struct Busy { double& out; double t0; ~Busy() { out = now_ms() - t0; } } busy{gbusy[d], tg0};
        DevJob& J = job[d];
        J.sub.reserve(member[d].size());
        for (uint32_t g : member[d]) J.sub.push_back(src[g]);
        if (!keep_on_device) J.dig.resize(J.sub.size() * 64);
        J.rc = hash_sources(x->dev[d].get(), J.sub, keep_on_device ? nullptr : J.dig.data(), nullptr, &J.err_no, &J.err_src);
    };

    std::atomic<size_t> hnext{0};
    std::atomic<int> herr{0};
    std::atomic<int64_t> herr_src{-1};
    unsigned nh = hidx.empty() ? 0u : std::max(1u, std::min<unsigned>(plan_threads, (unsigned)hidx.size()));
    const bool gpu_part = !gidx.empty();
    const bool spare_cores = 2u * nh <= call_cpus(x);
    std::vector<double> hbusy(std::max(1u, nh), 0.0);
    std::stable_sort(hidx.begin(), hidx.end(), [&](uint32_t a, uint32_t b) { return src[a].len > src[b].len; });
    uint64_t host_bytes_planned = 0;
    for (uint32_t g : hidx) host_bytes_planned += src[g].len;
    const uint64_t alone_from = nh ? host_bytes_planned / nh / 4 : 0;
    size_t n_lane_streams = 0;
    for (uint32_t g : hidx) n_lane_streams += src[g].len < alone_from || alone_from == 0;
    unsigned host_lanes = nh ? (unsigned)std::min<size_t>(8, (n_lane_streams + nh - 1) / nh) : 1u;
    for (auto& d : x->dev) d->fd_call_budget = -1;
    if (src[0].path != nullptr) {
        struct rlimit rl;
        int64_t soft = 1024;
        if (getrlimit(RLIMIT_NOFILE, &rl) == 0) soft = rl.rlim_cur == RLIM_INFINITY ? 65536 : (int64_t)rl.rlim_cur;
        const int64_t held = soft < 8192 ? open_descriptors() + 16 : 0;
        const int64_t reserve = std::max<int64_t>(held, std::min<int64_t>(512, soft / 2));
        const int64_t transient = gpu_part ? (int64_t)std::min(x->d0()->fill_cap, 12u) * (int64_t)nd : 0;
        const int64_t pool = std::max<int64_t>(2, soft - reserve - transient);
        int64_t lanes_fds = (int64_t)nh * host_lanes;
        const int64_t lanes_cap = gpu_part ? std::max<int64_t>(1, pool / 2) : pool;
        if (lanes_fds > lanes_cap) {
            if ((int64_t)nh > lanes_cap) nh = (unsigned)lanes_cap;
            host_lanes = (unsigned)std::max<int64_t>(1, lanes_cap / nh);
            lanes_fds = (int64_t)nh * host_lanes;
        }
        for (auto& d : x->dev) d->fd_call_budget = std::max<int64_t>(0, (pool - lanes_fds) / (int64_t)nd);
    }
    auto run_host = [&](unsigned t) {
        const double t0 = now_ms();
        int64_t bad = -1;
        const int err = host_sha512_many(
            host_lanes,
            [&]() -> int64_t {
                if (herr.load()) return -1;
                const size_t k = hnext.fetch_add(1);
                return k < hidx.size() ? (int64_t)hidx[k] : -1;
            },
            [&](int64_t g) {
                HostStream h;
                h.mem = src[g].mem;
                h.path = src[g].mem ? nullptr : src[g].path;
                h.len = src[g].len;
                h.digest = digests + 64 * (size_t)g;
                h.read_ahead = spare_cores;
                h.alone = alone_from != 0 && src[g].len >= alone_from;
                return h;
            },
            &bad);
        if (err) {
            int z = 0;
            if (herr.compare_exchange_strong(z, err)) herr_src.store(bad);
        }
        hbusy[t] = now_ms() - t0;
    };

    ThreadJoiner th, dth;
    try {
        for (unsigned t = gpu_part ? 0u : 1u; t < nh; ++t) th.spawn(run_host, t);
        if (gpu_part && nd > 1)
            for (size_t d = 0; d < nd; ++d) dth.spawn(run_dev, d);
    } catch (...) {
        int z = 0;
        herr.compare_exchange_strong(z, EAGAIN);
        th.join_all();
        dth.join_all();
        return fail(x, SNAPHASH_ENOMEM, "could not start a worker thread");
    }
    if (!gpu_part && !x->gpu_only) {
        std::lock_guard<std::mutex> lk(x->calib_mu);
        x->calib.relax(src[0].path != nullptr);
    }
    if (!gpu_part) { if (nh) run_host(0); }
    else if (nd == 1) run_dev(0);
    dth.join_all();
    th.join_all();

    for (uint32_t g : hidx) { x->ex.host_bytes += src[g].len; }
    x->ex.host_streams = hidx.size();
    for (double b : hbusy) x->ex.host_ms = std::max(x->ex.host_ms, b);
    for (double b : gbusy) x->ex.gpu_ms = std::max(x->ex.gpu_ms, b);
    x->ex.host_threads_run = nh;
    if (!x->gpu_only && x->ex.planned_host_ms > 0 && !herr.load() &&
        now_ms() - t_hash0 <= 3.0 * std::max(x->ex.planned_host_ms, x->ex.planned_gpu_ms)) {
        std::lock_guard<std::mutex> lk(x->calib_mu);
        x->calib.observe_host(x->ex.planned_host_ms * 1e-3, x->ex.host_ms * 1e-3);
    }

    int64_t bad = -1;
    int bad_errno = 0, bad_rc = 0;
    DevCtx* bad_dev = nullptr;
    for (size_t d = 0; d < nd; ++d) {
        if (!job[d].rc) continue;
        const int64_t g = job[d].err_src >= 0 ? (int64_t)member[d][job[d].err_src] : (int64_t)n;
        if (bad < 0 || g < bad) { bad = g; bad_errno = job[d].err_no; bad_rc = job[d].rc; bad_dev = x->dev[d].get(); }
    }
    if (herr.load() && (bad < 0 || herr_src.load() < bad)) {
        bad = herr_src.load();
        bad_errno = herr.load();
        bad_rc = SNAPHASH_EIO;
        bad_dev = nullptr;
        x->last_error = std::string(src[bad].path ? src[bad].path : "<buffer>") + ": " + strerror(bad_errno);
    }
    if (bad_rc) {
        if (bad_dev) x->last_error = bad_dev->last_error;
        if (status && bad >= 0 && bad < (int64_t)n) status[bad] = bad_errno;
        if (bad_out && bad >= 0 && bad < (int64_t)n) *bad_out = bad;
        merge_stats(x);
        return bad_rc;
    }

    if (!gpu_part) {
    } else if (!keep_on_device) {
        for (size_t k = 0; k < member[0].size(); ++k) memcpy(digests + 64 * (size_t)member[0][k], job[0].dig.data() + 64 * k, 64);
    } else {
        std::vector<size_t> cnt(nd);
        size_t kmax = 1;
        for (size_t d = 0; d < nd; ++d) { cnt[d] = member[d].size(); kmax = std::max(kmax, cnt[d]); }
        std::vector<uint8_t> rows;
        int rc = gather_digest_slabs(x, cnt, kmax, rows);
        if (rc) { merge_stats(x); return rc; }
        for (size_t d = 0; d < nd; ++d)
            for (size_t k = 0; k < cnt[d]; ++k) memcpy(digests + 64 * (size_t)member[d][k], rows.data() + (d * kmax + k) * 64, 64);
    }
    merge_stats(x);
    return SNAPHASH_OK;
}

static int64_t first_bad_path(const char* const* paths, size_t n, int* err, const Source* src = nullptr)
{
    for (size_t i = 0; i < n; ++i) {
        struct stat st;
        int e = 0;
        if (stat(paths[i], &st) != 0) e = errno;
        else if (S_ISDIR(st.st_mode)) e = EISDIR;
        else if (access(paths[i], R_OK) != 0) e = errno;
        else if (src && S_ISREG(st.st_mode) && (uint64_t)st.st_size != src[i].len) e = EIO;
        if (e) { *err = e; return (int64_t)i; }
    }
    return -1;
}

int hash_paths(snaphash_ctx* x, const char* const* paths, size_t n, const int64_t* sizes, uint8_t* digests, int32_t* status)
{
    std::vector<Source> src(n);
    for (size_t i = 0; i < n; ++i) {
        if (!paths[i]) return fail(x, SNAPHASH_EINVAL, "NULL path");
        src[i].path = paths[i];
        if (sizes && sizes[i] >= 0) src[i].len = (uint64_t)sizes[i];
    }
    {
        const unsigned T = (unsigned)std::max<size_t>(1, std::min<size_t>(std::min(12u, std::max(1u, std::thread::hardware_concurrency())), n / 2048));
        std::vector<int64_t> bad(T, -1);
        auto work = [&](unsigned t) {
            const size_t lo = n * t / T, hi = n * (t + 1) / T;
            for (size_t i = lo; i < hi; ++i) {
                if (sizes && sizes[i] >= 0) continue;
                struct stat st;
                if (stat(paths[i], &st) != 0 || S_ISDIR(st.st_mode)) { bad[t] = (int64_t)i; return; }
                src[i].len = (uint64_t)st.st_size;
            }
        };
        ThreadJoiner th;
        for (unsigned t = 1; t < T; ++t) th.spawn(work, t);
        work(0);
        th.join_all();
        int64_t first = -1;
        for (unsigned t = 0; t < T; ++t) if (bad[t] >= 0 && (first < 0 || bad[t] < first)) first = bad[t];
        if (first >= 0) {
            int err = EIO;
            int64_t b = first_bad_path(paths, (size_t)first + 1, &err);
            if (b < 0) b = first;
            if (status) { for (size_t k = 0; k < n; ++k) status[k] = 0; status[b] = err; }
            return fail(x, SNAPHASH_EIO, std::string(paths[b]) + ": " + strerror(err));
        }
    }
    int64_t tripped = -1;
    const int rc = hash_sources_top(x, src, digests, status, &tripped);
    if (rc == SNAPHASH_EIO) {
        int err = 0;
        const int64_t bad = first_bad_path(paths, tripped >= 0 ? std::min(n, (size_t)tripped + 1) : n, &err, src.data());
        if (bad >= 0) {
            if (status) { for (size_t k = 0; k < n; ++k) status[k] = 0; status[bad] = err; }
            return fail(x, SNAPHASH_EIO, std::string(paths[bad]) + ": " + strerror(err));
        }
    }
    return rc;
}

void end_top(snaphash_ctx* x, double t0) { x->stats.wall_ms = now_ms() - t0; }

}


extern "C" {

int snaphash_abi_version(void) { return SNAPHASH_ABI_VERSION; }

static thread_local std::string g_init_error;

static int init_fail(int code, const std::string& what, hipError_t e = hipSuccess)
try {
    g_init_error = what + (e != hipSuccess ? std::string(": ") + hipGetErrorString(e) : std::string());
    return code;
} catch (...) {
    return SNAPHASH_ENOMEM;
}

static void destroy_dev(DevCtx* c)
{
    (void)hipSetDevice(c->device);
    if (c->stream) (void)hipStreamSynchronize(c->stream);
    if (c->copy_stream) (void)hipStreamSynchronize(c->copy_stream);
    c->each_buf(Release());
}

static void calibrate_at_init(snaphash_ctx* x)
{
    if (getenv("SNAPHASH_NO_CALIBRATION")) return;
    DevCtx* c = x->d0();
    if (hipSetDevice(c->device) != hipSuccess) { (void)hipGetLastError(); return; }
    constexpr uint64_t kProbe = 8u << 20;
    if (c->staging < kProbe) return;
    if (ensure_slots(c, 1, kProbe) != SNAPHASH_OK) { c->last_error.clear(); (void)hipGetLastError(); return; }
    Slot& s = c->slot[0];
    const size_t big = (size_t)kProbe, small = big / 4;
    StageClock<2> clk;
    bool ok = clk.enable() == hipSuccess;
    if (ok) {
        ok = hipMemcpyAsync(s.d_buf.data(), s.h_buf.data(), small, hipMemcpyHostToDevice, c->copy_stream) == hipSuccess;
        ok = ok && clk.mark(0, c->copy_stream) == hipSuccess;
        ok = ok && hipMemcpyAsync(s.d_buf.data(), s.h_buf.data(), small, hipMemcpyHostToDevice, c->copy_stream) == hipSuccess;
        ok = ok && clk.mark(1, c->copy_stream) == hipSuccess;
        ok = ok && hipMemcpyAsync(s.d_buf.data(), s.h_buf.data(), big, hipMemcpyHostToDevice, c->copy_stream) == hipSuccess;
        ok = ok && clk.mark(2, c->copy_stream) == hipSuccess;
        ok = ok && hipStreamSynchronize(c->copy_stream) == hipSuccess;
        const float t_small = ok ? clk.ms(0) : 0, t_big = ok ? clk.ms(1) : 0;
        ok = ok && t_small > 0 && t_big > 0;
        if (ok && t_big > t_small) x->calib.observe_dma((double)(big - small), (double)(t_big - t_small) * 1e-3);
    }
    if (!ok) (void)hipGetLastError();
}

int snaphash_init(const snaphash_config* cfg, snaphash_ctx** out)
try {
    if (!out) return SNAPHASH_EINVAL;
    *out = nullptr;
    g_init_error.clear();
    int ndev = 0;
    hipError_t e = hipGetDeviceCount(&ndev);
    if (e != hipSuccess || ndev <= 0) return init_fail(SNAPHASH_EDEVICE, "hipGetDeviceCount found no device", e);
    const bool v1 = cfg && cfg->struct_size >= offsetof(snaphash_config, devices);
    const bool v2 = cfg && cfg->struct_size >= sizeof(snaphash_config);
    std::vector<int> devs;
    if (v2 && cfg->n_devices > 0) {
        if (!cfg->devices) return init_fail(SNAPHASH_EINVAL, "n_devices > 0 with a NULL device list");
        if (cfg->n_devices == 1 && cfg->devices[0] == -1) {
            for (int d = 0; d < ndev; ++d) devs.push_back(d);
        } else {
            for (uint32_t k = 0; k < cfg->n_devices; ++k) devs.push_back(cfg->devices[k]);
        }
        if (cfg->stream && devs.size() > 1) return init_fail(SNAPHASH_EINVAL, "a caller stream needs a single-device ctx");
    } else if (!cfg && getenv("SNAPHASH_DEVICES")) {
        const char* p = getenv("SNAPHASH_DEVICES");
        if (!strcmp(p, "all") || !strcmp(p, "-1")) {
            for (int d = 0; d < ndev; ++d) devs.push_back(d);
        } else {
            while (*p) {
                char* end = nullptr;
                const long d = strtol(p, &end, 10);
                if (end == p || (*end && *end != ',')) return init_fail(SNAPHASH_EINVAL, "SNAPHASH_DEVICES: expected \"all\" or a comma-separated list of ordinals");
                devs.push_back((int)d);
                p = *end ? end + 1 : end;
            }
            if (devs.empty()) return init_fail(SNAPHASH_EINVAL, "SNAPHASH_DEVICES is empty");
        }
    } else {
        int dev = v1 ? cfg->device : -1;
        if (dev < 0 && (e = hipGetDevice(&dev)) != hipSuccess) return init_fail(SNAPHASH_EDEVICE, "hipGetDevice", e);
        devs.push_back(dev);
    }
    if (devs.size() > 64) return init_fail(SNAPHASH_EINVAL, "more than 64 engines");
    std::unique_ptr<snaphash_ctx> x(new (std::nothrow) snaphash_ctx());
    if (!x) return SNAPHASH_ENOMEM;
    const unsigned ncpu = usable_cpus();
    x->cpus = ncpu;
    if (v2) {
        x->flags = cfg->flags;
        x->host_threads = std::min<uint32_t>(cfg->host_threads, 256);
    }
    if (!cfg && getenv("SNAPHASH_HOST_THREADS")) {
        x->host_threads = (uint32_t)std::min<unsigned long>(strtoul(getenv("SNAPHASH_HOST_THREADS"), nullptr, 10), 256);
        if (x->host_threads == 0) x->flags |= SNAPHASH_FLAG_GPU_ONLY;
    }
    x->gpu_only = (x->flags & SNAPHASH_FLAG_GPU_ONLY) != 0;
    if (!x->gpu_only) x->host_rate = measure_host_rate();
    const char* sysfs_env = getenv("SNAPHASH_SYSFS_ROOT");
    const std::string sysfs = sysfs_env && *sysfs_env ? sysfs_env : "/sys";
    const bool numa_on = !(x->flags & SNAPHASH_FLAG_NO_NUMA) && numa_node_count(sysfs) > 1;
    const unsigned fill_cap = std::max(2u, std::min(12u, ncpu / (unsigned)devs.size()));
    int64_t fd_budget = 0;
    {
        struct rlimit rl;
        if (getrlimit(RLIMIT_NOFILE, &rl) == 0) {
            const rlim_t want = rl.rlim_max == RLIM_INFINITY ? 65536 : std::min<rlim_t>(rl.rlim_max, 65536);
            const bool keep = (cfg && cfg->struct_size >= sizeof(snaphash_config) && (cfg->flags & SNAPHASH_FLAG_KEEP_RLIMIT)) || getenv("SNAPHASH_KEEP_RLIMIT");
            if (!keep && rl.rlim_cur != RLIM_INFINITY && rl.rlim_cur < want) {
                struct rlimit up = rl;
                up.rlim_cur = want;
                if (setrlimit(RLIMIT_NOFILE, &up) == 0) rl = up;
            }
            const int64_t soft = rl.rlim_cur == RLIM_INFINITY ? 65536 : (int64_t)rl.rlim_cur;
            fd_budget = std::max<int64_t>(0, std::min<int64_t>(soft - 512, 32768)) / (int64_t)devs.size();
        }
    }
    for (size_t k = 0; k < devs.size(); ++k) {
        const int dev = devs[k];
        if (dev < 0 || dev >= ndev) {
            for (auto& d : x->dev) destroy_dev(d.get());
            return init_fail(SNAPHASH_EINVAL, "device ordinal out of range");
        }
        hipDeviceProp_t prop;
        int rc = SNAPHASH_OK;
        std::string why;
        if ((e = hipGetDeviceProperties(&prop, dev)) != hipSuccess) { rc = SNAPHASH_EDEVICE; why = "hipGetDeviceProperties"; }
        else if (strncmp(prop.gcnArchName, "gfx950", 6) != 0) {
            rc = SNAPHASH_EDEVICE;
            e = hipSuccess;
            why = std::string("device is ") + prop.gcnArchName + ", this library is built for gfx950 only";
        } else if ((e = hipSetDevice(dev)) != hipSuccess) { rc = SNAPHASH_EDEVICE; why = "hipSetDevice"; }
        std::unique_ptr<DevCtx> c(rc ? nullptr : new (std::nothrow) DevCtx());
        if (!rc && !c) rc = SNAPHASH_ENOMEM;
        if (!rc) {
            c->device = dev;
            c->index = (int)k;
            if (v1) {
                if (cfg->staging_bytes) c->staging = (cfg->staging_bytes + kAlign - 1) & ~(uint64_t)(kAlign - 1);
                c->kernel_pref = cfg->kernel;
                if (cfg->deflate_depth) c->deflate_depth = std::min<uint32_t>(std::max<uint32_t>(cfg->deflate_depth, 4u), 256u) & ~3u;
                if (c->kernel_pref == SNAPHASH_KERNEL_QUAD && !have_quad_kernel()) {
                    rc = SNAPHASH_EINVAL;
                    e = hipSuccess;
                    why = "SNAPHASH_KERNEL_QUAD is not in this build (make QUAD=1)";
                }
                if (cfg->stream) c->stream.adopt((hipStream_t)cfg->stream);
            }
        }
        if (!rc) {
            if (c->staging < (1u << 16)) c->staging = 1u << 16;
            c->fill_cap = fill_cap;
            c->fd_budget = fd_budget;
            if (!cfg && getenv("SNAPHASH_DEFLATE_DEPTH"))
                c->deflate_depth = std::min<uint32_t>(std::max<uint32_t>((uint32_t)strtoul(getenv("SNAPHASH_DEFLATE_DEPTH"), nullptr, 10), 4u), 256u) & ~3u;
            {
                int xcc = 0;
                if (hipDeviceGetAttribute(&xcc, hipDeviceAttributeNumberOfXccs, dev) == hipSuccess && xcc >= 1 && xcc <= 64) c->n_xcd = (uint32_t)xcc;
                else (void)hipGetLastError();
            }
            std::vector<int> cpus;
            char bdf[64] = {0};
            if (hipDeviceGetPCIBusId(bdf, (int)sizeof bdf, dev) == hipSuccess) c->pci_bus_id = bdf;
            else (void)hipGetLastError();
            if (numa_on) {
                c->numa_node = numa_node_of_pci(sysfs, c->pci_bus_id);
                cpus = numa_cpus_of_node(sysfs, c->numa_node);
            }
            c->pool.configure(256, cpus);
            if ((e = c->stream.ensure(hipStreamNonBlocking)) != hipSuccess) { rc = SNAPHASH_EDEVICE; why = "hipStreamCreateWithFlags"; }
        }
        if (rc) {
            for (auto& d : x->dev) destroy_dev(d.get());
            return init_fail(rc, why, e);
        }
        x->dev.push_back(std::move(c));
    }
    if (numa_on && x->dev.size() > 1) {
        for (size_t k = 0; k < x->dev.size(); ++k) {
            DevCtx* c = x->dev[k].get();
            if (c->numa_node < 0) continue;
            size_t m = 0, pos = 0;
            for (size_t j = 0; j < x->dev.size(); ++j)
                if (x->dev[j]->numa_node == c->numa_node) { if (j == k) pos = m; ++m; }
            if (m < 2) continue;
            const std::vector<int> mine = slice_cpus(numa_cpus_of_node(sysfs, c->numa_node), pos, m);
            if (!mine.empty()) c->pool.configure(256, mine);
        }
    }
    for (auto& d : x->dev) { d->owner = x.get(); d->owner_cpus_per_engine = std::max(1u, ncpu / (unsigned)x->dev.size()); }
    if (!x->gpu_only) calibrate_at_init(x.get());
    *out = x.release();
    return SNAPHASH_OK;
} catch (...) {
    return SNAPHASH_ENOMEM;
}

void snaphash_destroy(snaphash_ctx* x)
{
    if (!x) return;
    if (x->open_batch) snaphash_batch_abort(x->open_batch);
    for (size_t d = 0; d < x->d_gather.size(); ++d)
        if (x->d_gather[d].data()) { (void)hipSetDevice(x->dev[d]->device); x->d_gather[d].reset(); }
    if (x->rccl.ok)
        for (ncclComm_t c : x->rccl.comms) if (c) (void)x->rccl.CommDestroy(c);
    for (auto& d : x->dev) destroy_dev(d.get());
    delete x;
}

#define TOP_ENTER(x)                                                                  \
    if ((x)->open_batch) return fail((x), SNAPHASH_EINVAL, "a streaming batch is open on this ctx"); \
    for (auto& d_ : (x)->dev) {                                                       \
        (void)hipSetDevice(d_->device);                                               \
        int rc_ = sync_ctx(d_.get());                                                 \
        if (rc_) return lift((x), d_.get(), rc_);                                     \
    }                                                                                 \
    begin_top(x);                                                                     \
    const double t_top0_ = now_ms()

int snaphash_sha512_files(snaphash_ctx* x, const char* const* paths, size_t n, uint8_t* digests, int32_t* status)
try {
    if (!x || (n && (!paths || !digests))) return fail(x, SNAPHASH_EINVAL, "bad argument");
    TOP_ENTER(x);
    int rc = hash_paths(x, paths, n, nullptr, digests, status);
    end_top(x, t_top0_);
    return rc;
} catch (...) {
    return SNAPHASH_ENOMEM;
}

int snaphash_sha512_buffers(snaphash_ctx* x, const void* const* bufs, const uint64_t* lens, size_t n, uint8_t* digests)
try {
    if (!x || (n && (!bufs || !lens || !digests))) return fail(x, SNAPHASH_EINVAL, "bad argument");
    TOP_ENTER(x);
    std::vector<Source> src(n);
    for (size_t i = 0; i < n; ++i) {
        if (!bufs[i] && lens[i]) return fail(x, SNAPHASH_EINVAL, "NULL buffer with non-zero length");
        src[i].mem = bufs[i] ? (const uint8_t*)bufs[i] : (const uint8_t*)"";
        src[i].len = lens[i];
    }
    int rc = hash_sources_top(x, src, digests, nullptr);
    end_top(x, t_top0_);
    return rc;
} catch (...) {
    return SNAPHASH_ENOMEM;
}

int snaphash_sha512_device(snaphash_ctx* x, const void* d_base, const uint64_t* offsets, const uint64_t* lens,
                           size_t n, void* d_digests)
try {
    if (!x || (n && (!d_base || !offsets || !lens || !d_digests))) return fail(x, SNAPHASH_EINVAL, "bad argument");
    if (((uintptr_t)d_base & 15) != 0) return fail(x, SNAPHASH_EINVAL, "d_base must be 16-byte aligned");
    if (n > 0xffffffffull) return fail(x, SNAPHASH_EINVAL, "too many streams");
    if (x->open_batch) return fail(x, SNAPHASH_EINVAL, "a streaming batch is open on this ctx");
    DevCtx* c = x->d0();
    HIP_TRY(c, hipSetDevice(c->device));
    int rc = sync_ctx(c);
    if (rc) return lift(x, c, rc);
    begin_top(x);
    begin_call(c);
    if (n == 0) return SNAPHASH_OK;
    HIP_TRY(x, c->hash.ensure(n, false, n));
    for (size_t i = 0; i < n; ++i) {
        if (offsets[i] & 15) return fail(x, SNAPHASH_EINVAL, "offsets must be 16-byte aligned");
        if (lens[i] >> 35) return fail(x, SNAPHASH_EINVAL, "a resident stream is limited to 32 GiB per call (32-bit block counters)");
        Job& j = c->hash.jobs.h[i];
        j.data = (uint64_t)(uintptr_t)d_base + offsets[i];
        j.nbytes = lens[i];
        j.total_prev = 0;
        j.idx = (uint32_t)i;
        j.flags = kJobFirst | kJobFinal;
        c->stats.bytes_hashed += lens[i];
        c->stats.blocks += padded_blocks(lens[i], true);
    }
    c->stats.streams = n;
    return lift(x, c, launch_jobs(c, c->hash.jobs.h.data(), c->hash.jobs.d.data(), n, (uint8_t*)d_digests));
} catch (...) {
    return SNAPHASH_ENOMEM;
}

static_assert(sizeof(snaphash_sha512_job) == sizeof(Job), "the public job is the kernels' Job");
static_assert(SNAPHASH_JOB_FIRST == kJobFirst && SNAPHASH_JOB_FINAL == kJobFinal, "the public flags are the kernels'");

int snaphash_sha512_jobs_device(snaphash_ctx* x, uint32_t kernel, int staged, const snaphash_sha512_job* jobs, size_t n, size_t n_rows,
                                void* d_state, void* d_digests)
try {
    if (!x || (n && (!jobs || !d_state || !d_digests))) return fail(x, SNAPHASH_EINVAL, "bad argument");
    if (x->open_batch) return fail(x, SNAPHASH_EINVAL, "a streaming batch is open on this ctx");
    if (kernel != SNAPHASH_KERNEL_WIDE && kernel != SNAPHASH_KERNEL_SPLIT && kernel != SNAPHASH_KERNEL_PAIR &&
        !(kernel == SNAPHASH_KERNEL_QUAD && have_quad_kernel()))
        return fail(x, SNAPHASH_EINVAL, "sha512 jobs: the kernel is WIDE, SPLIT or PAIR (QUAD in a build that has it)");
    if (n > 0xffffffffull || n_rows > 0xffffffffull) return fail(x, SNAPHASH_EINVAL, "sha512 jobs: too many jobs or rows");
    if (((uintptr_t)d_state & 7) != 0 || ((uintptr_t)d_digests & 15) != 0) return fail(x, SNAPHASH_EINVAL, "sha512 jobs: d_state must be 8-byte, d_digests 16-byte aligned");
    std::vector<bool> named(n_rows, false);
    for (size_t i = 0; i < n; ++i) {
        const snaphash_sha512_job& j = jobs[i];
        const bool fin = (j.flags & SNAPHASH_JOB_FINAL) != 0;
        if (j.flags & ~(SNAPHASH_JOB_FIRST | SNAPHASH_JOB_FINAL)) return fail(x, SNAPHASH_EINVAL, "sha512 jobs: unknown flag bits");
        if (j.data & 15) return fail(x, SNAPHASH_EINVAL, "sha512 jobs: a segment's address must be 16-byte aligned");
        if (j.nbytes >> 35) return fail(x, SNAPHASH_EINVAL, "sha512 jobs: a segment is limited to 32 GiB (32-bit block counters)");
        if (!fin && (j.nbytes & 127)) return fail(x, SNAPHASH_EINVAL, "sha512 jobs: a segment that is not final is a whole number of blocks");
        if (!fin && (j.flags & SNAPHASH_JOB_FIRST) && j.nbytes == 0) return fail(x, SNAPHASH_EINVAL, "sha512 jobs: a first segment that is not final holds a block at least");
        if (j.idx >= n_rows) return fail(x, SNAPHASH_EINVAL, "sha512 jobs: idx is not a row");
        if (named[j.idx]) return fail(x, SNAPHASH_EINVAL, "sha512 jobs: two jobs name one row");
        named[j.idx] = true;
    }
    if (n == 0) return SNAPHASH_OK;
    TOP_ENTER(x);
    DevCtx* c = x->d0();
    auto run = [&]() -> int {
        HIP_TRY(c, hipSetDevice(c->device));
        HIP_TRY(c, c->hash.jobs.ensure(n));
        Job* h = c->hash.jobs.h.data();
        for (size_t i = 0; i < n; ++i) h[i] = Job{jobs[i].data, jobs[i].nbytes, jobs[i].total_prev, jobs[i].idx, jobs[i].flags};
        HIP_TRY(c, hipMemcpyAsync(c->hash.jobs.d.data(), h, n * sizeof(Job), hipMemcpyHostToDevice, c->stream));
        const Job* d = c->hash.jobs.d.data();
        hipError_t e;
        if (kernel == SNAPHASH_KERNEL_QUAD) e = launch_quad(d, (uint32_t)n, (uint64_t*)d_state, (uint8_t*)d_digests, c->stream);
        else if (kernel == SNAPHASH_KERNEL_PAIR) e = launch_pair(d, (uint32_t)n, (uint64_t*)d_state, (uint8_t*)d_digests, c->stream, staged != 0);
        else if (kernel == SNAPHASH_KERNEL_SPLIT) e = launch_split(d, (uint32_t)n, (uint64_t*)d_state, (uint8_t*)d_digests, c->stream);
        else e = launch_wide(d, (uint32_t)n, (uint64_t*)d_state, (uint8_t*)d_digests, c->stream);
        const hipError_t es = hipStreamSynchronize(c->stream);
        if (e != hipSuccess) return fail(c, SNAPHASH_EDEVICE, std::string("kernel launch: ") + hipGetErrorString(e));
        HIP_TRY(c, es);
        return SNAPHASH_OK;
    };
    const int rc = run();
    if (rc) return lift(x, c, rc);
    x->stats.launches = 1;
    x->stats.kernel_used = kernel;
    x->stats.streams = n;
    end_top(x, t_top0_);
    return SNAPHASH_OK;
} catch (...) {
    return SNAPHASH_ENOMEM;
}

int snaphash_sync(snaphash_ctx* x)
try {
    if (!x) return SNAPHASH_EINVAL;
    for (auto& d : x->dev) {
        HIP_TRY(d.get(), hipSetDevice(d->device));
        int rc = sync_ctx(d.get());
        if (rc) return lift(x, d.get(), rc);
    }
    const double wall = x->d0()->stats.wall_ms;
    merge_stats(x);
    if (x->stats.wall_ms == 0) x->stats.wall_ms = wall;
    return SNAPHASH_OK;
} catch (...) {
    return SNAPHASH_ENOMEM;
}


static int tree_impl(snaphash_ctx* x, const char* build_dir, const char* data_tar, const uint8_t* archive_digest,
                     std::string& yaml)
{
    struct stat st;
    if (data_tar && stat(data_tar, &st) != 0) return fail(x, SNAPHASH_EIO, std::string(data_tar) + ": " + strerror(errno));
    std::vector<Record> recs;
    int en = 0;
    const double tw0 = now_ms();
    int rc = walk_tree(build_dir, recs, &en);
    const double tw1 = now_ms();
    if (rc) return fail(x, rc, rc == SNAPHASH_EIO ? std::string(build_dir) + ": " + strerror(en) : "Unknown file mode");
    if (const size_t b = first_unemittable_name(recs); b < recs.size())
        return fail(x, SNAPHASH_ENAME, "name outside what the YAML emitter restates (yamlscalar.cpp): " + recs[b].name);
    std::vector<const char*> paths;
    std::vector<int64_t> sizes;
    if (data_tar) { paths.push_back(data_tar); sizes.push_back(-1); }
    for (const Record& r : recs)
        if (r.is_regular) { paths.push_back(r.path.c_str()); sizes.push_back(r.size); }
    std::vector<uint8_t> dig(paths.size() * 64 + 64);
    const double th0 = now_ms();
    const bool early_yaml = recs.size() >= 2048;
    YamlSkeleton sk;
    int sk_rc = SNAPHASH_OK;
    ThreadJoiner skt;
    if (early_yaml) skt.spawn([&recs, &sk, &sk_rc] { sk_rc = emit_yaml_skeleton(recs, sk, 1); });
    rc = hash_paths(x, paths.data(), paths.size(), sizes.data(), dig.data(), nullptr);
    skt.join_all();
    const double th1 = now_ms();
    if (rc) return rc;
    const uint8_t* arch = data_tar ? dig.data() : archive_digest;
    const uint8_t* files = data_tar ? dig.data() + 64 : dig.data();
    if (early_yaml) {
        rc = sk_rc;
        if (!rc) { yaml_fill_digests(sk, arch, files); yaml.swap(sk.text); }
    } else {
        rc = emit_yaml(recs, arch, files, yaml);
    }
    static const bool trace_tree = getenv("SNAPHASH_TRACE_TREE") != nullptr;
    if (trace_tree)
        fprintf(stderr, "snaphash tree: walk %.1f ms (%zu records), hash %.1f ms (%zu streams), yaml %.1f ms (%zu bytes)\n", tw1 - tw0,
                recs.size(), th1 - th0, paths.size(), now_ms() - th1, yaml.size());
    return rc;
}

static int write_yaml_file(snaphash_ctx* x, const char* build_dir, const std::string& y)
{
    const std::string dir = std::string(build_dir) + "/DEBIAN";
    const std::string path = dir + "/hashes.yaml";
    int fd = open(path.c_str(), O_WRONLY | O_CREAT | O_TRUNC | O_CLOEXEC, 0644);
    if (fd < 0) return fail(x, SNAPHASH_EIO, path + ": " + strerror(errno));
    size_t off = 0;
    while (off < y.size()) {
        ssize_t w = write(fd, y.data() + off, y.size() - off);
        if (w < 0) { if (errno == EINTR) continue; int e = errno; close(fd); return fail(x, SNAPHASH_EIO, path + ": " + strerror(e)); }
        off += (size_t)w;
    }
    close(fd);
    return SNAPHASH_OK;
}

int snaphash_tree_ex(snaphash_ctx* x, const char* build_dir, const char* data_tar, const uint8_t* archive_digest,
                     int write_file, char** yaml_out, size_t* yaml_len)
try {
    if (!x || !build_dir || (!data_tar && !archive_digest) || (!write_file && !yaml_out)) return fail(x, SNAPHASH_EINVAL, "bad argument");
    if (yaml_out) *yaml_out = nullptr;
    if (write_file) {
        const std::string dir = std::string(build_dir) + "/DEBIAN";
        (void)mkdir(dir.c_str(), 0755);
    }
    const double t_in = now_ms();
    TOP_ENTER(x);
    std::string y;
    int rc = tree_impl(x, build_dir, data_tar, archive_digest, y);
    const double t_impl = now_ms();
    if (!rc && write_file) rc = write_yaml_file(x, build_dir, y);
    end_top(x, t_top0_);
    if (rc) return rc;
    if (yaml_out) {
        char* p = (char*)malloc(y.size() + 1);
        if (!p) return fail(x, SNAPHASH_ENOMEM, "malloc");
        memcpy(p, y.data(), y.size());
        p[y.size()] = 0;
        *yaml_out = p;
    }
    if (yaml_len) *yaml_len = y.size();
    static const bool trace_tree = getenv("SNAPHASH_TRACE_TREE") != nullptr;
    if (trace_tree)
        fprintf(stderr, "snaphash tree_ex: entry %.2f ms, the pass %.2f ms, the caller's copy of the YAML %.2f ms\n", t_top0_ - t_in, t_impl - t_top0_, now_ms() - t_impl);
    return SNAPHASH_OK;
} catch (...) {
    return SNAPHASH_ENOMEM;
}

int snaphash_tree(snaphash_ctx* x, const char* build_dir, const char* data_tar, char** yaml_out, size_t* yaml_len)
try {
    if (!x || !build_dir || !data_tar || !yaml_out) return fail(x, SNAPHASH_EINVAL, "bad argument");
    return snaphash_tree_ex(x, build_dir, data_tar, nullptr, 0, yaml_out, yaml_len);
} catch (...) {
    return SNAPHASH_ENOMEM;
}

int snaphash_write_hashes(snaphash_ctx* x, const char* build_dir, const char* data_tar)
try {
    if (!x || !build_dir || !data_tar) return fail(x, SNAPHASH_EINVAL, "bad argument");
    return snaphash_tree_ex(x, build_dir, data_tar, nullptr, 1, nullptr, nullptr);
} catch (...) {
    return SNAPHASH_ENOMEM;
}

static int mismatch(snaphash_ctx* c, snaphash_mismatch* m, int kind, const std::string& name)
{
    if (m) {
        m->kind = kind;
        m->reserved = 0;
        snprintf(m->name, sizeof m->name, "%s", name.c_str());
    }
    static const char* const what[] = {"", "missing on disk", "not in hashes.yaml", "size differs", "sha512 differs",
                                       "mode differs", "archive-sha512 differs"};
    return fail(c, SNAPHASH_EMISMATCH, name + ": " + what[kind]);
}

static int verify_impl(snaphash_ctx* x, const char* inst_dir, const char* data_tar, const uint8_t* archive_digest, const char* yaml,
                       size_t yaml_len, snaphash_mismatch* first, const std::function<bool(const Record&, uint8_t*)>& have_digest)
{
    const double t_top0_ = now_ms();
    ParsedHashes ph;
    int rc = parse_yaml(yaml, yaml_len, ph);
    if (rc) return fail(x, rc, "hashes.yaml: parse error");
    std::vector<Record> recs;
    int en = 0;
    rc = walk_tree(inst_dir, recs, &en);
    if (rc) return fail(x, rc, rc == SNAPHASH_EIO ? std::string(inst_dir) + ": " + strerror(en) : "Unknown file mode");

    size_t i = 0, j = 0;
    while (i < ph.files.size() && j < recs.size()) {
        if (ph.files[i].name == recs[j].name) { ++i; ++j; continue; }
        bool on_disk = false;
        for (size_t k = j; k < recs.size(); ++k)
            if (recs[k].name == ph.files[i].name) { on_disk = true; break; }
        return on_disk ? mismatch(x, first, 2, recs[j].name) : mismatch(x, first, 1, ph.files[i].name);
    }
    if (i < ph.files.size()) return mismatch(x, first, 1, ph.files[i].name);
    if (j < recs.size()) return mismatch(x, first, 2, recs[j].name);

    for (size_t k = 0; k < recs.size(); ++k) {
        const ParsedRecord& p = ph.files[k];
        const Record& r = recs[k];
        char a[11], b[11];
        if (mode_string(p.st_mode, a) || mode_string(r.st_mode, b) || memcmp(a, b, 10) != 0) return mismatch(x, first, 5, r.name);
        if (r.is_regular) {
            if (!p.has_size || p.size != r.size) return mismatch(x, first, 3, r.name);
        } else if (p.has_size || !p.sha512_hex.empty()) {
            return mismatch(x, first, 3, r.name);
        }
    }
    if (data_tar && (!ph.has_archive || ph.archive_hex.size() != 128)) return mismatch(x, first, 6, "archive-sha512");
    std::vector<const char*> paths;
    std::vector<int64_t> sizes;
    std::vector<size_t> owner;
    std::vector<uint8_t> held(recs.size() * 64 + 64), is_held(recs.size() + 1, 0);
    if (data_tar && !archive_digest) { paths.push_back(data_tar); sizes.push_back(-1); owner.push_back((size_t)-1); }
    for (size_t k = 0; k < recs.size(); ++k) {
        if (!recs[k].is_regular) continue;
        if (have_digest && have_digest(recs[k], held.data() + 64 * k)) { is_held[k] = 1; continue; }
        paths.push_back(recs[k].path.c_str()); sizes.push_back(recs[k].size); owner.push_back(k);
    }
    std::vector<uint8_t> dig(paths.size() * 64 + 64);
    rc = (paths.empty() && have_digest) ? 0 : hash_paths(x, paths.data(), paths.size(), sizes.data(), dig.data(), nullptr);
    end_top(x, t_top0_);
    if (rc) return rc;
    if (data_tar && archive_digest && !digest_matches_hex(archive_digest, ph.archive_hex)) return mismatch(x, first, 6, "archive-sha512");
    std::vector<const uint8_t*> of(recs.size(), nullptr);
    for (size_t q = 0; q < paths.size(); ++q) {
        if (owner[q] == (size_t)-1) {
            if (!digest_matches_hex(dig.data() + 64 * q, ph.archive_hex)) return mismatch(x, first, 6, "archive-sha512");
        } else {
            of[owner[q]] = dig.data() + 64 * q;
        }
    }
    for (size_t k = 0; k < recs.size(); ++k) {
        if (is_held[k]) of[k] = held.data() + 64 * k;
        if (of[k] && !digest_matches_hex(of[k], ph.files[k].sha512_hex)) return mismatch(x, first, 4, recs[k].name);
    }
    return SNAPHASH_OK;
}

int snaphash_verify(snaphash_ctx* x, const char* inst_dir, const char* data_tar, const char* yaml, size_t yaml_len,
                    snaphash_mismatch* first)
try {
    if (!x || !inst_dir || !yaml) return fail(x, SNAPHASH_EINVAL, "bad argument");
    TOP_ENTER(x);
    (void)t_top0_;
    return verify_impl(x, inst_dir, data_tar, nullptr, yaml, yaml_len, first, {});
} catch (...) {
    return SNAPHASH_ENOMEM;
}

void snaphash_free(void* p) { free(p); }

struct snaphash_shard {
    std::vector<Record> recs;
    std::string tar_path;
    std::vector<const char*> all_paths;
    std::vector<int64_t> all_sizes;
    std::vector<int32_t> shard_of;
    std::vector<uint32_t> row_of;
    std::vector<uint32_t> mine;
    std::vector<const char*> my_paths;
    std::vector<int64_t> my_sizes;
    uint32_t rank = 0, world = 1;
    uint32_t local_ranks = 0;
    size_t rows = 1;
    uint64_t my_bytes = 0;
    YamlSkeleton sk;
    int sk_rc = SNAPHASH_OK;
    bool sk_used = false;
    std::thread sk_thread;
    ~snaphash_shard() { if (sk_thread.joinable()) sk_thread.join(); }
};

static int finish_shard_plan(std::unique_ptr<snaphash_shard>& sh, const char* data_tar, int64_t tar_size)
{
    const uint32_t rank = sh->rank, world = sh->world;
    if (first_unemittable_name(sh->recs) < sh->recs.size()) return SNAPHASH_ENAME;
    sh->tar_path = data_tar;
    sh->all_paths.reserve(sh->recs.size() + 1);
    sh->all_sizes.reserve(sh->recs.size() + 1);
    sh->all_paths.push_back(sh->tar_path.c_str());
    sh->all_sizes.push_back(tar_size);
    for (const Record& r : sh->recs)
        if (r.is_regular) { sh->all_paths.push_back(r.path.c_str()); sh->all_sizes.push_back(r.size); }
    const size_t n = sh->all_paths.size();
    std::vector<uint64_t> lens(n);
    for (size_t i = 0; i < n; ++i) lens[i] = (uint64_t)sh->all_sizes[i];
    sh->shard_of.assign(n, 0);
    if (world > 1) lpt_assign(lens.data(), n, (int)world, sh->shard_of.data());
    std::vector<uint32_t> count(world, 0);
    sh->row_of.resize(n);
    for (size_t i = 0; i < n; ++i) sh->row_of[i] = count[sh->shard_of[i]]++;
    sh->rows = 1;
    for (uint32_t c : count) sh->rows = std::max<size_t>(sh->rows, c);
    for (size_t i = 0; i < n; ++i)
        if ((uint32_t)sh->shard_of[i] == rank) {
            sh->mine.push_back((uint32_t)i);
            sh->my_paths.push_back(sh->all_paths[i]);
            sh->my_sizes.push_back(i == 0 ? -1 : sh->all_sizes[i]);
            sh->my_bytes += lens[i];
        }
    if (sh->recs.size() >= 2048) {
        snaphash_shard* p = sh.get();
        try {
            sh->sk_thread = std::thread([p] {
                try { p->sk_rc = emit_yaml_skeleton(p->recs, p->sk, 1); } catch (...) { p->sk_rc = SNAPHASH_ENOMEM; }
            });
            sh->sk_used = true;
        } catch (...) { sh->sk_used = false; }
    }
    return SNAPHASH_OK;
}

int snaphash_shard_plan(const char* build_dir, const char* data_tar, uint32_t rank, uint32_t world, snaphash_shard** out)
try {
    if (!build_dir || !data_tar || !out || world == 0 || rank >= world || world > 4096) return SNAPHASH_EINVAL;
    *out = nullptr;
    struct stat st;
    if (stat(data_tar, &st) != 0) return SNAPHASH_EIO;
    std::unique_ptr<snaphash_shard> sh(new snaphash_shard());
    sh->rank = rank;
    sh->world = world;
    int en = 0;
    const double tp0 = now_ms();
    int rc = walk_tree(build_dir, sh->recs, &en);
    if (rc) { errno = en; return rc; }
    const double tp1 = now_ms();
    rc = finish_shard_plan(sh, data_tar, (int64_t)st.st_size);
    if (rc) return rc;
    static const bool trace_tree = getenv("SNAPHASH_TRACE_TREE") != nullptr;
    if (trace_tree)
        fprintf(stderr, "snaphash shard plan: walk %.2f ms (%zu records), names + lists + LPT over %u ranks %.2f ms\n", tp1 - tp0, sh->recs.size(), world, now_ms() - tp1);
    *out = sh.release();
    return SNAPHASH_OK;
} catch (...) {
    return SNAPHASH_ENOMEM;
}

int snaphash_shard_list(const char* build_dir, uint32_t rank, uint32_t world, void** blob_out, size_t* blob_len)
try {
    if (!build_dir || !blob_out || !blob_len || world == 0 || rank >= world || world > 4096) return SNAPHASH_EINVAL;
    *blob_out = nullptr;
    *blob_len = 0;
    std::string blob;
    int en = 0;
    const int rc = shard_listing(build_dir, rank, world, blob, &en);
    if (rc) { errno = en; return rc; }
    void* p = malloc(blob.size() ? blob.size() : 1);
    if (!p) return SNAPHASH_ENOMEM;
    memcpy(p, blob.data(), blob.size());
    *blob_out = p;
    *blob_len = blob.size();
    return SNAPHASH_OK;
} catch (...) {
    return SNAPHASH_ENOMEM;
}

int snaphash_shard_plan_from(const char* build_dir, const char* data_tar, uint32_t rank, uint32_t world, const void* const* blobs,
                             const size_t* blob_lens, snaphash_shard** out)
try {
    if (!build_dir || !data_tar || !blobs || !blob_lens || !out || world == 0 || rank >= world || world > 4096) return SNAPHASH_EINVAL;
    *out = nullptr;
    struct stat st;
    if (stat(data_tar, &st) != 0) return SNAPHASH_EIO;
    const double tp0 = now_ms();
    std::unique_ptr<snaphash_shard> sh(new snaphash_shard());
    sh->rank = rank;
    sh->world = world;
    int rc = records_from_listings(build_dir, world, blobs, blob_lens, sh->recs);
    if (rc) return rc;
    const double tp1 = now_ms();
    rc = finish_shard_plan(sh, data_tar, (int64_t)st.st_size);
    if (rc) return rc;
    static const bool trace_tree = getenv("SNAPHASH_TRACE_TREE") != nullptr;
    if (trace_tree)
        fprintf(stderr, "snaphash shard plan from %u ranks' listings: records %.2f ms (%zu), names + lists + LPT %.2f ms\n", world, tp1 - tp0, sh->recs.size(), now_ms() - tp1);
    *out = sh.release();
    return SNAPHASH_OK;
} catch (...) {
    return SNAPHASH_ENOMEM;
}

size_t snaphash_shard_rows(const snaphash_shard* sh) { return sh ? sh->rows : 0; }
size_t snaphash_shard_count(const snaphash_shard* sh) { return sh ? sh->mine.size() : 0; }
uint64_t snaphash_shard_bytes(const snaphash_shard* sh) { return sh ? sh->my_bytes : 0; }
size_t snaphash_shard_streams(const snaphash_shard* sh) { return sh ? sh->all_paths.size() : 0; }
const char* snaphash_shard_path(const snaphash_shard* sh, size_t k) { return sh && k < sh->my_paths.size() ? sh->my_paths[k] : nullptr; }

int snaphash_shard_hash(snaphash_ctx* x, snaphash_shard* sh, uint8_t* slab)
try {
    if (!x || !sh || !slab) return fail(x, SNAPHASH_EINVAL, "bad argument");
    TOP_ENTER(x);
    memset(slab, 0, sh->rows * 64);
    unsigned ranks_here = sh->local_ranks;
    for (const char* name : {"LOCAL_WORLD_SIZE", "OMPI_COMM_WORLD_LOCAL_SIZE", "MPI_LOCALNRANKS"}) {
        if (ranks_here) break;
        const char* e = getenv(name);
        const long v = e ? strtol(e, nullptr, 10) : 0;
        if (v >= 1 && v <= 4096) ranks_here = (unsigned)v;
    }
    if (!ranks_here) {
        int ndev = 0;
        if (hipGetDeviceCount(&ndev) != hipSuccess || ndev < 1) ndev = 1;
        ranks_here = std::min<unsigned>(sh->world, (unsigned)ndev);
    }
    ranks_here = std::max(1u, std::min(ranks_here, sh->world));
    struct Share {
        snaphash_ctx* x;
        ~Share()
        {
            x->cpus_call = 0;
            for (auto& d : x->dev) d->fill_call_cap = 0;
        }
    } share{x};
    if (ranks_here > 1) {
        x->cpus_call = std::max(1u, x->cpus / ranks_here);
        for (auto& d : x->dev) d->fill_call_cap = std::max(2u, x->cpus_call > 1u ? x->cpus_call - 1u : 1u);
    }
    const int rc = hash_paths(x, sh->my_paths.data(), sh->my_paths.size(), sh->my_sizes.data(), slab, nullptr);
    end_top(x, t_top0_);
    return rc;
} catch (...) {
    return SNAPHASH_ENOMEM;
}

int snaphash_shard_emit(const snaphash_shard* sh_c, const uint8_t* slabs, char** yaml_out, size_t* yaml_len)
try {
    if (!sh_c || !slabs || !yaml_out) return SNAPHASH_EINVAL;
    snaphash_shard* sh = const_cast<snaphash_shard*>(sh_c);
    *yaml_out = nullptr;
    const size_t n = sh->all_paths.size();
    std::vector<uint8_t> dig(n * 64);
    for (size_t i = 0; i < n; ++i)
        memcpy(dig.data() + 64 * i, slabs + ((size_t)sh->shard_of[i] * sh->rows + sh->row_of[i]) * 64, 64);
    std::string y;
    int rc;
    if (sh->sk_used) {
        if (sh->sk_thread.joinable()) sh->sk_thread.join();
        rc = sh->sk_rc;
        if (!rc) {
            YamlSkeleton filled = sh->sk;
            yaml_fill_digests(filled, dig.data(), dig.data() + 64);
            y.swap(filled.text);
        }
    } else {
// ... 1158 lines not shown
```

### snappy_amd/csrc/walk.cpp

```cpp
#include "walk.h"

#include "hostfill.h"

#include <dirent.h>
#include <errno.h>
#include <fcntl.h>
#include <string.h>

#include <stdio.h>
#include <stdlib.h>

#include <algorithm>
#include <atomic>
#include <chrono>
#include <thread>

namespace snaphash {

namespace {

struct Child {
    std::string name;
    unsigned char type = DT_UNKNOWN;
    struct stat st;
    bool have_st = false;
    int lstat_errno = 0;
    int64_t dir = -1;
};
struct DirList {
    std::string path;
    bool open_failed = false;
    std::vector<Child> kids;
    DIR* kept = nullptr;
    DirList() = default;
    DirList(DirList&& o) noexcept : path(std::move(o.path)), open_failed(o.open_failed), kids(std::move(o.kids)), kept(o.kept) { o.kept = nullptr; }
    DirList& operator=(DirList&& o) noexcept
    {
        if (this != &o) { release(); path = std::move(o.path); open_failed = o.open_failed; kids = std::move(o.kids); kept = o.kept; o.kept = nullptr; }
        return *this;
    }
    DirList(const DirList&) = delete;
    DirList& operator=(const DirList&) = delete;
    ~DirList() { release(); }
    void release() { if (kept) { closedir(kept); kept = nullptr; } }
};

constexpr int kKeptDirs = 192;
std::atomic<int> g_kept_dirs{0};

void list_dir(DirList& dl)
{
    DIR* d = opendir(dl.path.c_str());
    if (!d) { dl.open_failed = true; return; }
    while (struct dirent* de = readdir(d)) {
        if (!strcmp(de->d_name, ".") || !strcmp(de->d_name, "..")) continue;
        Child c;
        c.name = de->d_name;
        c.type = de->d_type;
        dl.kids.push_back(std::move(c));
    }
    if (dl.kids.size() >= 16 && g_kept_dirs.fetch_add(1) < kKeptDirs) dl.kept = d;
    else { if (dl.kids.size() >= 16) g_kept_dirs.fetch_sub(1); closedir(d); }
    std::sort(dl.kids.begin(), dl.kids.end(), [](const Child& a, const Child& b) { return a.name < b.name; });
    for (Child& c : dl.kids)
        if (c.type == DT_UNKNOWN) {
            if (lstat((dl.path + "/" + c.name).c_str(), &c.st) != 0) c.lstat_errno = errno;
            else { c.have_st = true; c.type = S_ISDIR(c.st.st_mode) ? DT_DIR : DT_REG; }
        }
}

unsigned walk_threads(size_t items, size_t per_thread)
{
    return (unsigned)std::max<size_t>(1, std::min<size_t>(std::min(16u, usable_cpus()), items / per_thread));
}

void list_tree(const std::string& root, std::vector<DirList>& dirs)
{
    dirs.clear();
    dirs.emplace_back();
    dirs[0].path = root;
    size_t lo = 0;
    while (lo < dirs.size()) {
        const size_t hi = dirs.size();
        const unsigned T = walk_threads(hi - lo, 4);
        std::atomic<size_t> next{lo};
        run_on_threads(T, [&](unsigned) {
            for (;;) {
                const size_t i = next.fetch_add(1);
                if (i >= hi) return;
                list_dir(dirs[i]);
            }
        });
        for (size_t i = lo; i < hi; ++i)
            for (size_t k = 0; k < dirs[i].kids.size(); ++k)
                if (dirs[i].kids[k].type == DT_DIR && !dirs[i].kids[k].lstat_errno) {
                    dirs[i].kids[k].dir = (int64_t)dirs.size();
                    DirList sub;
                    sub.path = dirs[i].path + "/" + dirs[i].kids[k].name;
                    dirs.push_back(std::move(sub));
                }
        lo = hi;
    }
}

}

int walk_entries(const char* root_c, std::vector<WalkEntry>& ents, int* err_no, std::string* err_path)
{
    std::string root(root_c);
    while (root.size() > 1 && root.back() == '/') root.pop_back();
    if (err_no) *err_no = 0;
    ents.clear();
    ents.resize(1);
    ents[0].path = root;
    if (lstat(root.c_str(), &ents[0].st) != 0) {
        if (err_no) *err_no = errno;
        if (err_path) *err_path = root;
        ents.clear();
        return -1;
    }
    ents[0].have_st = true;
    if (!S_ISDIR(ents[0].st.st_mode)) return 0;
    const bool trace = getenv("SNAPHASH_TRACE_TREE") != nullptr;
    const auto t0 = std::chrono::steady_clock::now();
    std::vector<DirList> dirs;
    list_tree(root, dirs);
    const auto t1 = std::chrono::steady_clock::now();

    const size_t nd = dirs.size();
    std::vector<size_t> count(nd, 0), start(nd, 0);
    for (size_t d = nd; d-- > 0;) {
        if (dirs[d].open_failed) { count[d] = 1; continue; }
        size_t c = 0;
        for (const Child& k : dirs[d].kids) c += 1 + (k.dir >= 0 ? count[(size_t)k.dir] : 0);
        count[d] = c;
    }
    start[0] = 1;
    struct Task { uint32_t dir, k0, k1; size_t first; };
    std::vector<Task> tasks;
    for (size_t d = 0; d < nd; ++d) {
        if (dirs[d].open_failed) { tasks.push_back(Task{(uint32_t)d, 0, 0, start[d]}); continue; }
        size_t at = start[d];
        const std::vector<Child>& kids = dirs[d].kids;
        for (size_t k = 0; k < kids.size(); ++k) {
            if (k % 256 == 0) tasks.push_back(Task{(uint32_t)d, (uint32_t)k, (uint32_t)std::min(kids.size(), k + 256), at});
            if (kids[k].dir >= 0) { start[(size_t)kids[k].dir] = at + 1; at += 1 + count[(size_t)kids[k].dir]; }
            else at += 1;
        }
    }
    const size_t n = 1 + count[0];
    ents.resize(n);

    const unsigned T = walk_threads(n, 512);
    std::vector<int64_t> bad(T, -1);
    std::vector<int> bad_errno(T, 0);
    std::atomic<size_t> next{0};
    auto work = [&](unsigned t) {
        auto fail = [&](size_t idx, int e) { if (bad[t] < 0 || (int64_t)idx < bad[t]) { bad[t] = (int64_t)idx; bad_errno[t] = e; } };
        for (;;) {
            const size_t ti = next.fetch_add(1);
            if (ti >= tasks.size()) return;
            const Task& tk = tasks[ti];
            const DirList& dl = dirs[tk.dir];
            if (dl.open_failed) {
                WalkEntry& e = ents[tk.first];
                e.path = dl.path;
                if (lstat(e.path.c_str(), &e.st) != 0) fail(tk.first, errno);
                else e.have_st = true;
                continue;
            }
            size_t at = tk.first;
            for (uint32_t k = tk.k0; k < tk.k1; ++k) {
                const Child& c = dl.kids[k];
                WalkEntry& e = ents[at];
                e.path.reserve(dl.path.size() + 1 + c.name.size());
                e.path = dl.path;
                e.path += '/';
                e.path += c.name;
                if (c.lstat_errno) fail(at, c.lstat_errno);
                else if (c.have_st) { e.st = c.st; e.have_st = true; }
                else if ((dl.kept ? fstatat(dirfd(dl.kept), c.name.c_str(), &e.st, AT_SYMLINK_NOFOLLOW) : lstat(e.path.c_str(), &e.st)) != 0) fail(at, errno);
                else e.have_st = true;
                at += 1 + (c.dir >= 0 ? count[(size_t)c.dir] : 0);
            }
        }
    };
    struct ReleaseDirs {
        std::vector<DirList>& dirs;
        ~ReleaseDirs()
        {
            int n = 0;
            for (DirList& d : dirs) if (d.kept) { d.release(); ++n; }
            g_kept_dirs.fetch_sub(n);
        }
    } release_dirs{dirs};
    run_on_threads(T, work);
    if (trace) {
        const auto t2 = std::chrono::steady_clock::now();
        fprintf(stderr, "snaphash walk: listing %zu directories (readdir + sort) %.2f ms, paths + Lstat of %zu entries on %u threads %.2f ms\n", nd,
                std::chrono::duration<double, std::milli>(t1 - t0).count(), n, T, std::chrono::duration<double, std::milli>(t2 - t1).count());
    }
    int64_t first_bad = -1;
    int first_errno = 0;
    for (unsigned t = 0; t < T; ++t)
        if (bad[t] >= 0 && (first_bad < 0 || bad[t] < first_bad)) { first_bad = bad[t]; first_errno = bad_errno[t]; }
    if (first_bad < 0) return 0;
    if (err_no) *err_no = first_errno;
    if (err_path) *err_path = ents[(size_t)first_bad].path;
    ents.resize((size_t)first_bad);
    return -1;
}

}
```

Before: 49.55 GiB/s.

## Plan next batch during reads, sweep tree in one pass, pinned digest readback

The engine loop now plans batch N+1 on the calling thread while helper threads fill batch N, spilling job lists to a scratch buffer when the target slot is still busy. The directory walk is replaced by a single-pass sweep that lists, stats and builds records directly, in place of walking entries and then converting them. Digests are read back through the pinned staging buffer, and the sync no longer double-synchronizes for tracing. The yaml fill gains an overload writing into an external buffer, and the yaml write call skips one string copy. These changes aim to cut serial host time around the GPU hashing, at the cost of more complex ordering and error-handling paths.

Result: no change. 49.96 GiB/s, median of 4 (+0.8%).

```diff
diff --git a/snappy_amd/csrc/hostfill.cpp b/snappy_amd/csrc/hostfill.cpp
--- a/snappy_amd/csrc/hostfill.cpp
+++ b/snappy_amd/csrc/hostfill.cpp
@@ -269,9 +269,9 @@
     }
 }
 
-void FillPool::parallel_for(size_t n, unsigned threads, const std::function<void(size_t)>& fn)
-{
-    if (n == 0) return;
+void FillPool::parallel_for(size_t n, unsigned threads, const std::function<void(size_t)>& fn, const std::function<void()>* first)
+{
+    if (n == 0) { if (first) (*first)(); return; }
     unsigned helpers = threads > 1 ? std::min(threads - 1, max_threads_) : 0u;
     if (helpers > n - 1) helpers = (unsigned)(n - 1);
     std::atomic<size_t> next{0};
@@ -292,6 +292,7 @@
     if (helpers) cv_work_.notify_all();
     bool threw = false;
     try {
+        if (first) (*first)();
         for (;;) {
             const size_t i = next.fetch_add(1);
             if (i >= n) break;
diff --git a/snappy_amd/csrc/hostfill.h b/snappy_amd/csrc/hostfill.h
--- a/snappy_amd/csrc/hostfill.h
+++ b/snappy_amd/csrc/hostfill.h
@@ -62,7 +62,7 @@
     FillPool(const FillPool&) = delete;
     FillPool& operator=(const FillPool&) = delete;
     void configure(unsigned max_threads, const std::vector<int>& cpus);
-    void parallel_for(size_t n, unsigned threads, const std::function<void(size_t)>& fn);
+    void parallel_for(size_t n, unsigned threads, const std::function<void(size_t)>& fn, const std::function<void()>* first = nullptr);
     unsigned max_threads() const { return max_threads_; }
     const std::vector<int>& cpus() const { return cpus_; }
 
diff --git a/snappy_amd/csrc/hostpass.cpp b/snappy_amd/csrc/hostpass.cpp
--- a/snappy_amd/csrc/hostpass.cpp
+++ b/snappy_amd/csrc/hostpass.cpp
@@ -2,6 +2,7 @@
 
 #include "hostfill.h"
 #include "walk.h"
+#include "walk_sweep.h"
 
 #include <dirent.h>
 #include <errno.h>
@@ -48,7 +49,7 @@
 }
 
 
-static int records_from_entries_impl(std::vector<WalkEntry>& ents, std::vector<Record>& out, bool steal)
+int records_from_entries(const std::vector<WalkEntry>& ents, std::vector<Record>& out)
 {
     if (ents.empty()) return SNAPHASH_OK;
     const size_t rootlen = ents[0].path.size();
@@ -82,14 +83,13 @@
         size_t at = base + kept[t];
         for (size_t i = lo; i < hi; ++i) {
             if (!keep[i]) continue;
-            WalkEntry& e = ents[i];
+            const WalkEntry& e = ents[i];
             Record& r = out[at++];
             r.name.assign(e.path.c_str() + rootlen + 1, e.path.size() - rootlen - 1);
             r.st_mode = e.st.st_mode;
             r.is_regular = S_ISREG(e.st.st_mode);
             r.size = r.is_regular ? (int64_t)e.st.st_size : 0;
-            if (steal) r.path = std::move(e.path);
-            else r.path = e.path;
+            r.path = e.path;
         }
     });
     return SNAPHASH_OK;
@@ -109,20 +109,35 @@
     return first;
 }
 
-int records_from_entries(const std::vector<WalkEntry>& ents, std::vector<Record>& out)
-{
-    return records_from_entries_impl(const_cast<std::vector<WalkEntry>&>(ents), out, false);
+namespace {
+struct RecordSink {
+    using Out = Record;
+    static std::string& path(Record& r) { return r.path; }
+    static const std::string& path(const Record& r) { return r.path; }
+    static int finish(Record& r, size_t rootlen, const struct stat& st)
+    {
+        const char* rel = r.path.c_str() + rootlen;
+        if (rel[0] == 0 || strncmp(rel, "/DEBIAN", 7) == 0) return 0;
+        char m[11];
+        if (mode_string(st.st_mode, m) != SNAPHASH_OK) return SNAPHASH_EMODE;
+        r.name.assign(rel + 1, r.path.size() - rootlen - 1);
+        r.st_mode = st.st_mode;
+        r.is_regular = S_ISREG(st.st_mode);
+        r.size = r.is_regular ? (int64_t)st.st_size : 0;
+        return 1;
+    }
+};
 }
 
 int walk_tree(const char* build_dir, std::vector<Record>& out, int* err_no)
 {
-    std::vector<WalkEntry> ents;
-    int e = 0;
-    const int wrc = walk_entries(build_dir, ents, &e, nullptr);
-    if (err_no) *err_no = e;
-    const int rc = records_from_entries_impl(ents, out, true);
-    if (rc) return rc;
-    return wrc ? SNAPHASH_EIO : SNAPHASH_OK;
+    if (err_no) *err_no = 0;
+    const size_t base = out.size();
+    SweepError err;
+    if (sweep_tree<RecordSink>(build_dir, out, &err) == 0) return SNAPHASH_OK;
+    if (err.code) { out.resize(base); return err.code; }
+    if (err_no) *err_no = err.err_no;
+    return SNAPHASH_EIO;
 }
 
 
@@ -240,12 +255,17 @@
 
 void yaml_fill_digests(YamlSkeleton& sk, const uint8_t archive_digest[64], const uint8_t* file_digests)
 {
+    yaml_fill_digests(sk, &sk.text[0], archive_digest, file_digests);
+}
+
+void yaml_fill_digests(const YamlSkeleton& sk, char* text, const uint8_t archive_digest[64], const uint8_t* file_digests)
+{
     if (sk.hex_at.empty()) return;
-    hex_lower(archive_digest, &sk.text[sk.hex_at[0]]);
+    hex_lower(archive_digest, text + sk.hex_at[0]);
     const size_t n = sk.hex_at.size() - 1;
     const unsigned T = (unsigned)std::max<size_t>(1, std::min<size_t>(std::min(8u, usable_cpus()), n / 2048));
     auto work = [&](unsigned t) {
-        for (size_t i = n * t / T; i < n * (t + 1) / T; ++i) hex_lower(file_digests + 64 * i, &sk.text[sk.hex_at[i + 1]]);
+        for (size_t i = n * t / T; i < n * (t + 1) / T; ++i) hex_lower(file_digests + 64 * i, text + sk.hex_at[i + 1]);
     };
     run_on_threads(T, work);
 }
diff --git a/snappy_amd/csrc/hostpass.h b/snappy_amd/csrc/hostpass.h
--- a/snappy_amd/csrc/hostpass.h
+++ b/snappy_amd/csrc/hostpass.h
@@ -48,6 +48,7 @@
 };
 int emit_yaml_skeleton(const std::vector<Record>& recs, YamlSkeleton& out, unsigned max_threads = 8 );
 void yaml_fill_digests(YamlSkeleton& sk, const uint8_t archive_digest[64], const uint8_t* file_digests);
+void yaml_fill_digests(const YamlSkeleton& sk, char* text, const uint8_t archive_digest[64], const uint8_t* file_digests);
 int shard_listing(const char* build_dir, uint32_t rank, uint32_t world, std::string& blob, int* err_no);
 int records_from_listings(const char* build_dir, uint32_t world, const void* const* blobs, const size_t* blob_lens, std::vector<Record>& recs);
 int parse_yaml(const char* text, size_t len, ParsedHashes& out);
diff --git a/snappy_amd/csrc/snapbuild.inc b/snappy_amd/csrc/snapbuild.inc
--- a/snappy_amd/csrc/snapbuild.inc
+++ b/snappy_amd/csrc/snapbuild.inc
@@ -98,7 +98,7 @@
     st.members = x->targz.members;
     st.data_bytes = x->targz.gz_bytes;
     if (hashes) {
-        rc = write_yaml_file(x, source_dir, std::string(yaml, yaml_len));
+        rc = write_yaml_file(x, source_dir, yaml, yaml_len);
         if (rc) return rc;
     }
     rc = tar_create_impl(x, enc_control, tmp.control.c_str(), debian.c_str(), nullptr, nullptr, nullptr, nullptr, nullptr, nullptr);
diff --git a/snappy_amd/csrc/snaphash_api.cpp b/snappy_amd/csrc/snaphash_api.cpp
--- a/snappy_amd/csrc/snaphash_api.cpp
+++ b/snappy_amd/csrc/snaphash_api.cpp
@@ -144,6 +144,14 @@
 }
 
 struct snaphash_batch;
+
+struct TreeLeftovers {
+    std::vector<snaphash::Record> recs;
+    std::vector<snaphash::Source> src;
+    std::vector<uint8_t> dig;
+    snaphash::YamlSkeleton sk;
+    std::string yaml;
+};
 
 struct snaphash_ctx {
     std::vector<std::unique_ptr<DevCtx>> dev;
@@ -169,6 +177,7 @@
     snaphash_block_scan_stats block_scan{};
     std::string last_error;
     snaphash_batch* open_batch = nullptr;
+    std::unique_ptr<TreeLeftovers> leftovers;
     DevCtx* d0() const { return dev[0].get(); }
 };
 
@@ -346,11 +355,14 @@
     return SNAPHASH_OK;
 }
 
-int sync_ctx(DevCtx* c)
+struct EngineSpans { float gpu = 0, copy_busy = 0, copy = 0; };
+EngineSpans engine_spans(DevCtx* c);
+int sync_ctx(DevCtx* c, EngineSpans* spans = nullptr)
 {
     if (!c->pending && c->ledger.used() == 0) return SNAPHASH_OK;
     if (c->copy_stream) HIP_TRY(c, hipStreamSynchronize(c->copy_stream));
     HIP_TRY(c, hipStreamSynchronize(c->stream));
+    if (spans && c->ledger.used() > 1) *spans = engine_spans(c);
     collect_events(c);
     c->pending = false;
     if (c->t_call0 > 0) { c->stats.wall_ms = now_ms() - c->t_call0; c->t_call0 = 0; }
@@ -416,7 +428,7 @@
 }
 
 void run_reads(DevCtx* c, const std::vector<Source>& src, const std::vector<ReadOp>& ops, std::atomic<int>& first_err,
-               std::atomic<int64_t>& first_err_src, FdCache* cache = nullptr, bool alone = false)
+               std::atomic<int64_t>& first_err_src, FdCache* cache = nullptr, bool alone = false, const std::function<void()>* ahead = nullptr)
 {
     static const int forced = [] {
         const char* e = getenv("SNAPHASH_COPY_THREADS");
@@ -447,15 +459,12 @@
             int z = 0;
             if (first_err.compare_exchange_strong(z, err)) first_err_src.store(op.src);
         }
-    });
-}
-
-struct EngineSpans { float gpu = 0, copy_busy = 0, copy = 0; };
+    }, ahead);
+}
+
 EngineSpans engine_spans(DevCtx* c)
 {
     EngineSpans sp;
-    if (c->copy_stream) (void)hipStreamSynchronize(c->copy_stream);
-    (void)hipStreamSynchronize(c->stream);
     Span first_copy, last_copy, last_kernel, first;
     c->ledger.each([&](Ev kind, const Span& s) {
         if (!first.a) first = s;
@@ -502,66 +511,114 @@
     BatchPlanner plan(src.data(), n, job_bytes, g.S_full, BatchKnobs::from_env());
     std::atomic<int> first_err{0};
     std::atomic<int64_t> first_err_src{-1};
-    std::vector<ReadOp> ops;
     FdCache fds(from_memory ? 0 : n, c->fd_call_budget >= 0 ? std::min(c->fd_call_budget, c->fd_budget) : c->fd_budget);
     double t_wait = 0, t_plan = 0, t_read = 0, t_launch = 0;
     const double t_engine0 = now_ms();
     double t_first_copy = 0;
     size_t n_copies = 0;
-
-    while (!plan.active.empty()) {
-        const unsigned batch = plan.batch, q = batch % g.nsub;
-        SubSlot& sl = c->sub[q];
-        uint8_t* const sl_h = c->slot[q / g.per_slot].h_buf.data() + (uint64_t)(q % g.per_slot) * g.S_full;
-        uint8_t* const sl_d = c->slot[q / g.per_slot].d_buf.data() + (uint64_t)(q % g.per_slot) * g.S_full;
+    static const bool trace_batches = getenv("SNAPHASH_TRACE_BATCHES") != nullptr;
+
+    struct Planned {
+        Batch b;
+        unsigned batch = 0, q = 0;
+        size_t left = 0;
+        bool in_pinned = false;
+        double ms = 0;
+        std::vector<ReadOp> ops;
+        std::vector<Job> spill;
+        uint8_t *sl_h = nullptr, *sl_d = nullptr;
+    } planned[2];
+    auto plan_batch = [&](Planned& p, const Planned* filling) -> int {
+        const double t0 = now_ms();
+        p.batch = plan.batch;
+        p.q = p.batch % g.nsub;
+        SubSlot& sl = c->sub[p.q];
+        p.sl_h = c->slot[p.q / g.per_slot].h_buf.data() + (uint64_t)(p.q % g.per_slot) * g.S_full;
+        p.sl_d = c->slot[p.q / g.per_slot].d_buf.data() + (uint64_t)(p.q % g.per_slot) * g.S_full;
+        p.in_pinned = !sl.busy && !(filling && filling->q == p.q);
+        Job* jobs;
+        if (p.in_pinned) {
+            HIP_TRY(c, sl.jobs.ensure(plan.active.size()));
+            jobs = sl.jobs.h.data();
+        } else {
+            p.spill.resize(plan.active.size());
+            jobs = p.spill.data();
+        }
+        p.b = plan.next(jobs, p.ops, (uint64_t)(uintptr_t)p.sl_h, (uint64_t)(uintptr_t)p.sl_d);
+        p.left = plan.active.size();
+        if (empty_files)
+            for (size_t k = 0; k < p.b.nj; ++k) {
+                const Job& j = jobs[k];
+                if (j.nbytes == 0 && src[j.idx].len == 0 && src[j.idx].path) p.ops.push_back(ReadOp{j.idx, 0, 0, p.sl_h, true});
+            }
+        p.ms = now_ms() - t0;
+        t_plan += p.ms;
+        return SNAPHASH_OK;
+    };
+
+    const bool any = !plan.active.empty();
+    if (any && (rc = plan_batch(planned[0], nullptr))) return rc;
+    for (unsigned cur = 0; any; cur ^= 1) {
+        Planned& p = planned[cur];
+        SubSlot& sl = c->sub[p.q];
         const double tb0 = now_ms();
         if (sl.busy) { HIP_TRY(c, hipEventSynchronize(sl.done)); sl.busy = false; }
         const double tb1 = now_ms();
         t_wait += tb1 - tb0;
-        HIP_TRY(c, sl.jobs.ensure(plan.active.size()));
-        const Batch b = plan.next(sl.jobs.h.data(), ops, (uint64_t)(uintptr_t)sl_h, (uint64_t)(uintptr_t)sl_d);
-        c->stats.blocks += b.blocks;
-        static const bool trace_batches = getenv("SNAPHASH_TRACE_BATCHES") != nullptr;
-        if (trace_batches) trace_batch(stderr, c->index, batch, b, sl.jobs.h.data(), (uint64_t)(uintptr_t)sl_d, plan.active.size());
-        if (empty_files)
-            for (size_t k = 0; k < b.nj; ++k) {
-                const Job& j = sl.jobs.h[k];
-                if (j.nbytes == 0 && src[j.idx].len == 0 && src[j.idx].path) ops.push_back(ReadOp{j.idx, 0, 0, sl_h, true});
-            }
+        if (!p.in_pinned) {
+            HIP_TRY(c, sl.jobs.ensure(p.spill.size()));
+            memcpy(sl.jobs.h.data(), p.spill.data(), p.b.nj * sizeof(Job));
+        }
+        c->stats.blocks += p.b.blocks;
+        if (trace_batches) trace_batch(stderr, c->index, p.batch, p.b, sl.jobs.h.data(), (uint64_t)(uintptr_t)p.sl_d, p.left);
         const double tb2 = now_ms();
-        t_plan += tb2 - tb1;
-
-        run_reads(c, src, ops, first_err, first_err_src, from_memory ? nullptr : &fds, batch == 0);
+
+        int rc_ahead = SNAPHASH_OK;
+        const std::function<void()> ahead = [&] { rc_ahead = plan_batch(planned[cur ^ 1], &p); };
+        run_reads(c, src, p.ops, first_err, first_err_src, from_memory ? nullptr : &fds, p.batch == 0, p.left ? &ahead : nullptr);
         if (first_err.load()) break;
+        if (rc_ahead) return rc_ahead;
         const double tb3 = now_ms();
         t_read += tb3 - tb2;
         if (trace_batches)
-            fprintf(stderr, "snaphash engine %d: batch %u: at %.2f ms: waited %.2f, planned %.2f, filled %.2f ms (%zu streams begun, %.1f GB/s)\n", c->index, batch,
-                    tb0 - t_engine0, tb1 - tb0, tb2 - tb1, tb3 - tb2, b.n_new, (double)b.used / ((tb3 - tb2) * 1e6 + 1e-9));
-
-        if (b.used) {
-            if (batch == 0) t_first_copy = now_ms() - t_engine0;
+            fprintf(stderr, "snaphash engine %d: batch %u: at %.2f ms: waited %.2f, planned %.2f (ahead, beside the fill before), took over %.2f, filled %.2f ms (%zu streams begun, %.1f GB/s)\n",
+                    c->index, p.batch, tb0 - t_engine0, tb1 - tb0, p.ms, tb2 - tb1, tb3 - tb2, p.b.n_new, (double)p.b.used / ((tb3 - tb2) * 1e6 + 1e-9));
+
+        if (p.b.used) {
+            if (p.batch == 0) t_first_copy = now_ms() - t_engine0;
             ++n_copies;
             Span ev;
             if ((rc = span_begin(c, Ev::H2d, c->copy_stream, &ev))) return rc;
-            HIP_TRY(c, hipMemcpyAsync(sl_d, sl_h, b.used, hipMemcpyHostToDevice, c->copy_stream));
+            HIP_TRY(c, hipMemcpyAsync(p.sl_d, p.sl_h, p.b.used, hipMemcpyHostToDevice, c->copy_stream));
             if ((rc = span_end(c, ev, c->copy_stream))) return rc;
         }
-        rc = launch_jobs(c, sl.jobs.h.data(), sl.jobs.d.data(), b.nj, c->hash.d_digests.data(), sl.copied);
+        rc = launch_jobs(c, sl.jobs.h.data(), sl.jobs.d.data(), p.b.nj, c->hash.d_digests.data(), sl.copied);
         if (rc) return rc;
         HIP_TRY(c, hipEventRecord(sl.done, c->stream));
         sl.busy = true;
         t_launch += now_ms() - tb3;
+        if (!p.left) break;
     }
 
     const double ts0 = now_ms();
     static const bool trace_tree = getenv("SNAPHASH_TRACE_TREE") != nullptr;
-    const EngineSpans sp = trace_tree && c->ledger.used() > 1 ? engine_spans(c) : EngineSpans{};
-    rc = sync_ctx(c);
+    EngineSpans sp;
+    rc = sync_ctx(c, trace_tree ? &sp : nullptr);
+    const double ts1 = now_ms();
+    if (!rc && !first_err.load() && digests) {
+        uint8_t* const pin = c->slot[0].h_buf.size() >= n * 64 ? c->slot[0].h_buf.data() : nullptr;
+        if (pin) {
+            HIP_TRY(c, hipMemcpyAsync(pin, c->hash.d_digests.data(), n * 64, hipMemcpyDeviceToHost, c->stream));
+            HIP_TRY(c, hipStreamSynchronize(c->stream));
+            memcpy(digests, pin, n * 64);
+        } else {
+            HIP_TRY(c, hipMemcpy(digests, c->hash.d_digests.data(), n * 64, hipMemcpyDeviceToHost));
+        }
+    }
     if (trace_tree)
         fprintf(stderr, "snaphash engine %d: %u batches; waiting for a slot %.1f ms, planning %.1f ms, reads %.1f ms, enqueue %.1f ms, drain %.1f ms; "
-                        "first copy enqueued at %.2f ms, copies busy %.2f of %.2f ms, first copy -> last kernel %.2f ms, engine %.2f ms\n",
-                c->index, plan.batch, t_wait, t_plan, t_read, t_launch, now_ms() - ts0, t_first_copy, sp.copy_busy, sp.copy, sp.gpu, now_ms() - t_engine0);
+                        "digests read back %.2f ms; first copy enqueued at %.2f ms, copies busy %.2f of %.2f ms, first copy -> last kernel %.2f ms, engine %.2f ms\n",
+                c->index, plan.batch, t_wait, t_plan, t_read, t_launch, ts1 - ts0, now_ms() - ts1, t_first_copy, sp.copy_busy, sp.copy, sp.gpu, now_ms() - t_engine0);
     for (SubSlot& ss : c->sub) ss.busy = false;
     if (rc) return rc;
     if (first_err.load()) {
@@ -571,7 +628,6 @@
         return fail(c, SNAPHASH_EIO,
                     std::string(s >= 0 && src[s].path ? src[s].path : "<buffer>") + ": " + strerror(first_err.load()));
     }
-    if (digests) HIP_TRY(c, hipMemcpy(digests, c->hash.d_digests.data(), n * 64, hipMemcpyDeviceToHost));
     if (states) HIP_TRY(c, hipMemcpy(states, c->hash.d_state.data(), n * 64, hipMemcpyDeviceToHost));
     for (size_t i = 0; i < n; ++i) c->stats.bytes_hashed += src[i].gpu_len;
     c->stats.streams = n;
@@ -807,9 +863,12 @@
 
     std::vector<uint32_t> gidx;
     std::vector<uint32_t> hidx;
+    gidx.reserve(n);
     for (size_t i = 0; i < n; ++i) (on_host[i] ? hidx : gidx).push_back((uint32_t)i);
+    const bool direct = nd == 1 && hidx.empty() && !keep_on_device_planned(x, nd);
     std::vector<std::vector<uint32_t>> member(nd);
-    if (nd == 1) {
+    if (direct) {
+    } else if (nd == 1) {
         member[0] = gidx;
     } else {
         std::vector<uint64_t> lens(gidx.size());
@@ -836,6 +895,10 @@
         const double tg0 = now_ms();
         struct Busy { double& out; double t0; ~Busy() { out = now_ms() - t0; } } busy{gbusy[d], tg0};
         DevJob& J = job[d];
+        if (direct) {
+            J.rc = hash_sources(x->dev[d].get(), src, digests, nullptr, &J.err_no, &J.err_src);
+            return;
+        }
         J.sub.reserve(member[d].size());
         for (uint32_t g : member[d]) J.sub.push_back(src[g]);
         if (!keep_on_device) J.dig.resize(J.sub.size() * 64);
@@ -939,7 +1002,7 @@
     DevCtx* bad_dev = nullptr;
     for (size_t d = 0; d < nd; ++d) {
         if (!job[d].rc) continue;
-        const int64_t g = job[d].err_src >= 0 ? (int64_t)member[d][job[d].err_src] : (int64_t)n;
+        const int64_t g = job[d].err_src < 0 ? (int64_t)n : direct ? job[d].err_src : (int64_t)member[d][job[d].err_src];
         if (bad < 0 || g < bad) { bad = g; bad_errno = job[d].err_no; bad_rc = job[d].rc; bad_dev = x->dev[d].get(); }
     }
     if (herr.load() && (bad < 0 || herr_src.load() < bad)) {
@@ -957,7 +1020,7 @@
         return bad_rc;
     }
 
-    if (!gpu_part) {
+    if (!gpu_part || direct) {
     } else if (!keep_on_device) {
         for (size_t k = 0; k < member[0].size(); ++k) memcpy(digests + 64 * (size_t)member[0][k], job[0].dig.data() + 64 * k, 64);
     } else {
@@ -974,37 +1037,32 @@
     return SNAPHASH_OK;
 }
 
-static int64_t first_bad_path(const char* const* paths, size_t n, int* err, const Source* src = nullptr)
+static int64_t first_bad_path(const Source* src, size_t n, int* err, bool with_lengths)
 {
     for (size_t i = 0; i < n; ++i) {
         struct stat st;
         int e = 0;
-        if (stat(paths[i], &st) != 0) e = errno;
+        if (stat(src[i].path, &st) != 0) e = errno;
         else if (S_ISDIR(st.st_mode)) e = EISDIR;
-        else if (access(paths[i], R_OK) != 0) e = errno;
-        else if (src && S_ISREG(st.st_mode) && (uint64_t)st.st_size != src[i].len) e = EIO;
+        else if (access(src[i].path, R_OK) != 0) e = errno;
+        else if (with_lengths && S_ISREG(st.st_mode) && (uint64_t)st.st_size != src[i].len) e = EIO;
         if (e) { *err = e; return (int64_t)i; }
     }
     return -1;
 }
 
-int hash_paths(snaphash_ctx* x, const char* const* paths, size_t n, const int64_t* sizes, uint8_t* digests, int32_t* status)
-{
-    std::vector<Source> src(n);
-    for (size_t i = 0; i < n; ++i) {
-        if (!paths[i]) return fail(x, SNAPHASH_EINVAL, "NULL path");
-        src[i].path = paths[i];
-        if (sizes && sizes[i] >= 0) src[i].len = (uint64_t)sizes[i];
-    }
-    {
-        const unsigned T = (unsigned)std::max<size_t>(1, std::min<size_t>(std::min(12u, std::max(1u, std::thread::hardware_concurrency())), n / 2048));
+int hash_file_sources(snaphash_ctx* x, std::vector<Source>& src, const std::vector<uint32_t>& unknown, uint8_t* digests, int32_t* status)
+{
+    const size_t n = src.size();
+    if (!unknown.empty()) {
+        const size_t nu = unknown.size();
+        const unsigned T = (unsigned)std::max<size_t>(1, std::min<size_t>(std::min(12u, std::max(1u, std::thread::hardware_concurrency())), nu / 2048));
         std::vector<int64_t> bad(T, -1);
         auto work = [&](unsigned t) {
-            const size_t lo = n * t / T, hi = n * (t + 1) / T;
-            for (size_t i = lo; i < hi; ++i) {
-                if (sizes && sizes[i] >= 0) continue;
+            for (size_t k = nu * t / T; k < nu * (t + 1) / T; ++k) {
+                const uint32_t i = unknown[k];
                 struct stat st;
-                if (stat(paths[i], &st) != 0 || S_ISDIR(st.st_mode)) { bad[t] = (int64_t)i; return; }
+                if (stat(src[i].path, &st) != 0 || S_ISDIR(st.st_mode)) { bad[t] = (int64_t)i; return; }
                 src[i].len = (uint64_t)st.st_size;
             }
         };
@@ -1016,23 +1074,36 @@
         for (unsigned t = 0; t < T; ++t) if (bad[t] >= 0 && (first < 0 || bad[t] < first)) first = bad[t];
         if (first >= 0) {
             int err = EIO;
-            int64_t b = first_bad_path(paths, (size_t)first + 1, &err);
+            int64_t b = first_bad_path(src.data(), (size_t)first + 1, &err, false);
             if (b < 0) b = first;
             if (status) { for (size_t k = 0; k < n; ++k) status[k] = 0; status[b] = err; }
-            return fail(x, SNAPHASH_EIO, std::string(paths[b]) + ": " + strerror(err));
+            return fail(x, SNAPHASH_EIO, std::string(src[b].path) + ": " + strerror(err));
         }
     }
     int64_t tripped = -1;
     const int rc = hash_sources_top(x, src, digests, status, &tripped);
     if (rc == SNAPHASH_EIO) {
         int err = 0;
-        const int64_t bad = first_bad_path(paths, tripped >= 0 ? std::min(n, (size_t)tripped + 1) : n, &err, src.data());
+        const int64_t bad = first_bad_path(src.data(), tripped >= 0 ? std::min(n, (size_t)tripped + 1) : n, &err, true);
         if (bad >= 0) {
             if (status) { for (size_t k = 0; k < n; ++k) status[k] = 0; status[bad] = err; }
-            return fail(x, SNAPHASH_EIO, std::string(paths[bad]) + ": " + strerror(err));
+            return fail(x, SNAPHASH_EIO, std::string(src[bad].path) + ": " + strerror(err));
         }
     }
     return rc;
+}
+
+int hash_paths(snaphash_ctx* x, const char* const* paths, size_t n, const int64_t* sizes, uint8_t* digests, int32_t* status)
+{
+    std::vector<Source> src(n);
+    std::vector<uint32_t> unknown;
+    for (size_t i = 0; i < n; ++i) {
+        if (!paths[i]) return fail(x, SNAPHASH_EINVAL, "NULL path");
+        src[i].path = paths[i];
+        if (sizes && sizes[i] >= 0) src[i].len = (uint64_t)sizes[i];
+        else unknown.push_back((uint32_t)i);
+    }
+    return hash_file_sources(x, src, unknown, digests, status);
 }
 
 void end_top(snaphash_ctx* x, double t0) { x->stats.wall_ms = now_ms() - t0; }
@@ -1399,11 +1470,12 @@
 
 
 static int tree_impl(snaphash_ctx* x, const char* build_dir, const char* data_tar, const uint8_t* archive_digest,
-                     std::string& yaml)
+                     TreeLeftovers& L, char** handover, size_t* yaml_len)
 {
     struct stat st;
     if (data_tar && stat(data_tar, &st) != 0) return fail(x, SNAPHASH_EIO, std::string(data_tar) + ": " + strerror(errno));
-    std::vector<Record> recs;
+    std::unique_ptr<TreeLeftovers> old = std::move(x->leftovers);
+    std::vector<Record>& recs = L.recs;
     int en = 0;
     const double tw0 = now_ms();
     int rc = walk_tree(build_dir, recs, &en);
@@ -1411,46 +1483,69 @@
     if (rc) return fail(x, rc, rc == SNAPHASH_EIO ? std::string(build_dir) + ": " + strerror(en) : "Unknown file mode");
     if (const size_t b = first_unemittable_name(recs); b < recs.size())
         return fail(x, SNAPHASH_ENAME, "name outside what the YAML emitter restates (yamlscalar.cpp): " + recs[b].name);
-    std::vector<const char*> paths;
-    std::vector<int64_t> sizes;
-    if (data_tar) { paths.push_back(data_tar); sizes.push_back(-1); }
+    std::vector<Source>& src = L.src;
+    std::vector<uint32_t> unknown;
+    src.reserve(recs.size() + 1);
+    if (data_tar) {
+        src.emplace_back();
+        src.back().path = data_tar;
+        unknown.push_back(0);
+    }
     for (const Record& r : recs)
-        if (r.is_regular) { paths.push_back(r.path.c_str()); sizes.push_back(r.size); }
-    std::vector<uint8_t> dig(paths.size() * 64 + 64);
+        if (r.is_regular) {
+            src.emplace_back();
+            src.back().path = r.path.c_str();
+            src.back().len = (uint64_t)r.size;
+        }
+    std::vector<uint8_t>& dig = L.dig;
+    dig.resize(src.size() * 64 + 64);
     const double th0 = now_ms();
     const bool early_yaml = recs.size() >= 2048;
-    YamlSkeleton sk;
+    YamlSkeleton& sk = L.sk;
     int sk_rc = SNAPHASH_OK;
+    std::unique_ptr<char, decltype(&free)> ybuf(nullptr, &free);
     ThreadJoiner skt;
-    if (early_yaml) skt.spawn([&recs, &sk, &sk_rc] { sk_rc = emit_yaml_skeleton(recs, sk, 1); });
-    rc = hash_paths(x, paths.data(), paths.size(), sizes.data(), dig.data(), nullptr);
+    if (early_yaml)
+        skt.spawn([&recs, &sk, &sk_rc, &ybuf, &old, handover] {
+            sk_rc = emit_yaml_skeleton(recs, sk, 1);
+            if (!sk_rc && handover) {
+                ybuf.reset((char*)malloc(sk.text.size() + 1));
+                if (ybuf) memcpy(ybuf.get(), sk.text.c_str(), sk.text.size() + 1);
+            }
+            old.reset();
+        });
+    rc = hash_file_sources(x, src, unknown, dig.data(), nullptr);
     skt.join_all();
     const double th1 = now_ms();
     if (rc) return rc;
     const uint8_t* arch = data_tar ? dig.data() : archive_digest;
     const uint8_t* files = data_tar ? dig.data() + 64 : dig.data();
+    size_t len = 0;
     if (early_yaml) {
         rc = sk_rc;
-        if (!rc) { yaml_fill_digests(sk, arch, files); yaml.swap(sk.text); }
+        if (!rc && ybuf) { yaml_fill_digests(sk, ybuf.get(), arch, files); len = sk.text.size(); *handover = ybuf.release(); }
+        else if (!rc) { yaml_fill_digests(sk, arch, files); L.yaml.swap(sk.text); len = L.yaml.size(); }
     } else {
-        rc = emit_yaml(recs, arch, files, yaml);
-    }
+        rc = emit_yaml(recs, arch, files, L.yaml);
+        len = L.yaml.size();
+    }
+    if (yaml_len) *yaml_len = len;
     static const bool trace_tree = getenv("SNAPHASH_TRACE_TREE") != nullptr;
     if (trace_tree)
         fprintf(stderr, "snaphash tree: walk %.1f ms (%zu records), hash %.1f ms (%zu streams), yaml %.1f ms (%zu bytes)\n", tw1 - tw0,
-                recs.size(), th1 - th0, paths.size(), now_ms() - th1, yaml.size());
+                recs.size(), th1 - th0, src.size(), now_ms() - th1, len);
     return rc;
 }
 
-static int write_yaml_file(snaphash_ctx* x, const char* build_dir, const std::string& y)
+static int write_yaml_file(snaphash_ctx* x, const char* build_dir, const char* y, size_t y_len)
 {
     const std::string dir = std::string(build_dir) + "/DEBIAN";
     const std::string path = dir + "/hashes.yaml";
     int fd = open(path.c_str(), O_WRONLY | O_CREAT | O_TRUNC | O_CLOEXEC, 0644);
     if (fd < 0) return fail(x, SNAPHASH_EIO, path + ": " + strerror(errno));
     size_t off = 0;
-    while (off < y.size()) {
-        ssize_t w = write(fd, y.data() + off, y.size() - off);
+    while (off < y_len) {
+        ssize_t w = write(fd, y + off, y_len - off);
         if (w < 0) { if (errno == EINTR) continue; int e = errno; close(fd); return fail(x, SNAPHASH_EIO, path + ": " + strerror(e)); }
         off += (size_t)w;
     }
@@ -1469,24 +1564,29 @@
     }
     const double t_in = now_ms();
     TOP_ENTER(x);
-    std::string y;
-    int rc = tree_impl(x, build_dir, data_tar, archive_digest, y);
+    std::unique_ptr<TreeLeftovers> L(new TreeLeftovers());
+    char* owned = nullptr;
+    size_t len = 0;
+    int rc = tree_impl(x, build_dir, data_tar, archive_digest, *L, yaml_out ? &owned : nullptr, &len);
+    std::unique_ptr<char, decltype(&free)> own(owned, &free);
+    const char* y = owned ? owned : L->yaml.data();
     const double t_impl = now_ms();
-    if (!rc && write_file) rc = write_yaml_file(x, build_dir, y);
+    if (!rc && write_file) rc = write_yaml_file(x, build_dir, y, len);
     end_top(x, t_top0_);
-    if (rc) return rc;
-    if (yaml_out) {
-        char* p = (char*)malloc(y.size() + 1);
-        if (!p) return fail(x, SNAPHASH_ENOMEM, "malloc");
-        memcpy(p, y.data(), y.size());
-        p[y.size()] = 0;
-        *yaml_out = p;
-    }
-    if (yaml_len) *yaml_len = y.size();
+    if (!rc && yaml_out && !owned) {
+        own.reset((char*)malloc(len + 1));
+        if (!own) rc = fail(x, SNAPHASH_ENOMEM, "malloc");
+        else { memcpy(own.get(), y, len); own.get()[len] = 0; }
+    }
+    if (!rc && yaml_out) *yaml_out = own.release();
+    if (!rc && yaml_len) *yaml_len = len;
+    const double t_out = now_ms();
+    x->leftovers = std::move(L);
     static const bool trace_tree = getenv("SNAPHASH_TRACE_TREE") != nullptr;
     if (trace_tree)
-        fprintf(stderr, "snaphash tree_ex: entry %.2f ms, the pass %.2f ms, the caller's copy of the YAML %.2f ms\n", t_top0_ - t_in, t_impl - t_top0_, now_ms() - t_impl);
-    return SNAPHASH_OK;
+        fprintf(stderr, "snaphash tree_ex: entry %.2f ms, the pass %.2f ms, the caller's YAML %.2f ms (%s), records and lists left with the ctx in %.2f ms\n", t_top0_ - t_in,
+                t_impl - t_top0_, t_out - t_impl, owned ? "handed over" : "copied", now_ms() - t_out);
+    return rc;
 } catch (...) {
     return SNAPHASH_ENOMEM;
 }
diff --git a/snappy_amd/csrc/walk.cpp b/snappy_amd/csrc/walk.cpp
--- a/snappy_amd/csrc/walk.cpp
+++ b/snappy_amd/csrc/walk.cpp
@@ -1,213 +1,33 @@
 #include "walk.h"
 
-#include "hostfill.h"
-
-#include <dirent.h>
-#include <errno.h>
-#include <fcntl.h>
-#include <string.h>
-
-#include <stdio.h>
-#include <stdlib.h>
-
-#include <algorithm>
-#include <atomic>
-#include <chrono>
-#include <thread>
+#include "walk_sweep.h"
 
 namespace snaphash {
 
 namespace {
 
-struct Child {
-    std::string name;
-    unsigned char type = DT_UNKNOWN;
-    struct stat st;
-    bool have_st = false;
-    int lstat_errno = 0;
-    int64_t dir = -1;
+struct EntrySink {
+    using Out = WalkEntry;
+    static std::string& path(WalkEntry& e) { return e.path; }
+    static const std::string& path(const WalkEntry& e) { return e.path; }
+    static int finish(WalkEntry& e, size_t, const struct stat& st)
+    {
+        e.st = st;
+        e.have_st = true;
+        return 1;
+    }
 };
-struct DirList {
-    std::string path;
-    bool open_failed = false;
-    std::vector<Child> kids;
-    DIR* kept = nullptr;
-    DirList() = default;
-    DirList(DirList&& o) noexcept : path(std::move(o.path)), open_failed(o.open_failed), kids(std::move(o.kids)), kept(o.kept) { o.kept = nullptr; }
-    DirList& operator=(DirList&& o) noexcept
-    {
-        if (this != &o) { release(); path = std::move(o.path); open_failed = o.open_failed; kids = std::move(o.kids); kept = o.kept; o.kept = nullptr; }
-        return *this;
-    }
-    DirList(const DirList&) = delete;
-    DirList& operator=(const DirList&) = delete;
-    ~DirList() { release(); }
-    void release() { if (kept) { closedir(kept); kept = nullptr; } }
-};
-
-constexpr int kKeptDirs = 192;
-std::atomic<int> g_kept_dirs{0};
-
-void list_dir(DirList& dl)
-{
-    DIR* d = opendir(dl.path.c_str());
-    if (!d) { dl.open_failed = true; return; }
-    while (struct dirent* de = readdir(d)) {
-        if (!strcmp(de->d_name, ".") || !strcmp(de->d_name, "..")) continue;
-        Child c;
-        c.name = de->d_name;
-        c.type = de->d_type;
-        dl.kids.push_back(std::move(c));
-    }
-    if (dl.kids.size() >= 16 && g_kept_dirs.fetch_add(1) < kKeptDirs) dl.kept = d;
-    else { if (dl.kids.size() >= 16) g_kept_dirs.fetch_sub(1); closedir(d); }
-    std::sort(dl.kids.begin(), dl.kids.end(), [](const Child& a, const Child& b) { return a.name < b.name; });
-    for (Child& c : dl.kids)
-        if (c.type == DT_UNKNOWN) {
-            if (lstat((dl.path + "/" + c.name).c_str(), &c.st) != 0) c.lstat_errno = errno;
-            else { c.have_st = true; c.type = S_ISDIR(c.st.st_mode) ? DT_DIR : DT_REG; }
-        }
-}
-
-unsigned walk_threads(size_t items, size_t per_thread)
-{
-    return (unsigned)std::max<size_t>(1, std::min<size_t>(std::min(16u, usable_cpus()), items / per_thread));
-}
-
-void list_tree(const std::string& root, std::vector<DirList>& dirs)
-{
-    dirs.clear();
-    dirs.emplace_back();
-    dirs[0].path = root;
-    size_t lo = 0;
-    while (lo < dirs.size()) {
-        const size_t hi = dirs.size();
-        const unsigned T = walk_threads(hi - lo, 4);
-        std::atomic<size_t> next{lo};
-        run_on_threads(T, [&](unsigned) {
-            for (;;) {
-                const size_t i = next.fetch_add(1);
-                if (i >= hi) return;
-                list_dir(dirs[i]);
-            }
-        });
-        for (size_t i = lo; i < hi; ++i)
-            for (size_t k = 0; k < dirs[i].kids.size(); ++k)
-                if (dirs[i].kids[k].type == DT_DIR && !dirs[i].kids[k].lstat_errno) {
-                    dirs[i].kids[k].dir = (int64_t)dirs.size();
-                    DirList sub;
-                    sub.path = dirs[i].path + "/" + dirs[i].kids[k].name;
-                    dirs.push_back(std::move(sub));
-                }
-        lo = hi;
-    }
-}
 
 }
 
-int walk_entries(const char* root_c, std::vector<WalkEntry>& ents, int* err_no, std::string* err_path)
+int walk_entries(const char* root, std::vector<WalkEntry>& ents, int* err_no, std::string* err_path)
 {
-    std::string root(root_c);
-    while (root.size() > 1 && root.back() == '/') root.pop_back();
     if (err_no) *err_no = 0;
     ents.clear();
-    ents.resize(1);
-    ents[0].path = root;
-    if (lstat(root.c_str(), &ents[0].st) != 0) {
-        if (err_no) *err_no = errno;
-        if (err_path) *err_path = root;
-        ents.clear();
-        return -1;
-    }
-    ents[0].have_st = true;
-    if (!S_ISDIR(ents[0].st.st_mode)) return 0;
-    const bool trace = getenv("SNAPHASH_TRACE_TREE") != nullptr;
-    const auto t0 = std::chrono::steady_clock::now();
-    std::vector<DirList> dirs;
-    list_tree(root, dirs);
-    const auto t1 = std::chrono::steady_clock::now();
-
-    const size_t nd = dirs.size();
-    std::vector<size_t> count(nd, 0), start(nd, 0);
-    for (size_t d = nd; d-- > 0;) {
-        if (dirs[d].open_failed) { count[d] = 1; continue; }
-        size_t c = 0;
-        for (const Child& k : dirs[d].kids) c += 1 + (k.dir >= 0 ? count[(size_t)k.dir] : 0);
-        count[d] = c;
-    }
-    start[0] = 1;
-    struct Task { uint32_t dir, k0, k1; size_t first; };
-    std::vector<Task> tasks;
-    for (size_t d = 0; d < nd; ++d) {
-        if (dirs[d].open_failed) { tasks.push_back(Task{(uint32_t)d, 0, 0, start[d]}); continue; }
-        size_t at = start[d];
-        const std::vector<Child>& kids = dirs[d].kids;
-        for (size_t k = 0; k < kids.size(); ++k) {
-            if (k % 256 == 0) tasks.push_back(Task{(uint32_t)d, (uint32_t)k, (uint32_t)std::min(kids.size(), k + 256), at});
-            if (kids[k].dir >= 0) { start[(size_t)kids[k].dir] = at + 1; at += 1 + count[(size_t)kids[k].dir]; }
-            else at += 1;
-        }
-    }
-    const size_t n = 1 + count[0];
-    ents.resize(n);
-
-    const unsigned T = walk_threads(n, 512);
-    std::vector<int64_t> bad(T, -1);
-    std::vector<int> bad_errno(T, 0);
-    std::atomic<size_t> next{0};
-    auto work = [&](unsigned t) {
-        auto fail = [&](size_t idx, int e) { if (bad[t] < 0 || (int64_t)idx < bad[t]) { bad[t] = (int64_t)idx; bad_errno[t] = e; } };
-        for (;;) {
-            const size_t ti = next.fetch_add(1);
-            if (ti >= tasks.size()) return;
-            const Task& tk = tasks[ti];
-            const DirList& dl = dirs[tk.dir];
-            if (dl.open_failed) {
-                WalkEntry& e = ents[tk.first];
-                e.path = dl.path;
-                if (lstat(e.path.c_str(), &e.st) != 0) fail(tk.first, errno);
-                else e.have_st = true;
-                continue;
-            }
-            size_t at = tk.first;
-            for (uint32_t k = tk.k0; k < tk.k1; ++k) {
-                const Child& c = dl.kids[k];
-                WalkEntry& e = ents[at];
-                e.path.reserve(dl.path.size() + 1 + c.name.size());
-                e.path = dl.path;
-                e.path += '/';
-                e.path += c.name;
-                if (c.lstat_errno) fail(at, c.lstat_errno);
-                else if (c.have_st) { e.st = c.st; e.have_st = true; }
-                else if ((dl.kept ? fstatat(dirfd(dl.kept), c.name.c_str(), &e.st, AT_SYMLINK_NOFOLLOW) : lstat(e.path.c_str(), &e.st)) != 0) fail(at, errno);
-                else e.have_st = true;
-                at += 1 + (c.dir >= 0 ? count[(size_t)c.dir] : 0);
-            }
-        }
-    };
-    struct ReleaseDirs {
-        std::vector<DirList>& dirs;
-        ~ReleaseDirs()
-        {
-            int n = 0;
-            for (DirList& d : dirs) if (d.kept) { d.release(); ++n; }
-            g_kept_dirs.fetch_sub(n);
-        }
-    } release_dirs{dirs};
-    run_on_threads(T, work);
-    if (trace) {
-        const auto t2 = std::chrono::steady_clock::now();
-        fprintf(stderr, "snaphash walk: listing %zu directories (readdir + sort) %.2f ms, paths + Lstat of %zu entries on %u threads %.2f ms\n", nd,
-                std::chrono::duration<double, std::milli>(t1 - t0).count(), n, T, std::chrono::duration<double, std::milli>(t2 - t1).count());
-    }
-    int64_t first_bad = -1;
-    int first_errno = 0;
-    for (unsigned t = 0; t < T; ++t)
-        if (bad[t] >= 0 && (first_bad < 0 || bad[t] < first_bad)) { first_bad = bad[t]; first_errno = bad_errno[t]; }
-    if (first_bad < 0) return 0;
-    if (err_no) *err_no = first_errno;
-    if (err_path) *err_path = ents[(size_t)first_bad].path;
-    ents.resize((size_t)first_bad);
+    SweepError err;
+    if (sweep_tree<EntrySink>(root, ents, &err) == 0) return 0;
+    if (err_no) *err_no = err.err_no;
+    if (err_path) *err_path = err.path;
     return -1;
 }
 
diff --git a/snappy_amd/csrc/walk_sweep.h b/snappy_amd/csrc/walk_sweep.h
--- /dev/null
+++ b/snappy_amd/csrc/walk_sweep.h
@@ -0,0 +1,234 @@
+#pragma once
+#include <dirent.h>
+#include <errno.h>
+#include <fcntl.h>
+#include <stdint.h>
+#include <stdio.h>
+#include <stdlib.h>
+#include <string.h>
+#include <sys/stat.h>
+
+#include <algorithm>
+#include <atomic>
+#include <chrono>
+#include <memory>
+#include <string>
+#include <vector>
+
+#include "hostfill.h"
+
+namespace snaphash {
+
+constexpr int kKeptDirs = 192;
+inline std::atomic<int> g_kept_dirs{0};
+constexpr size_t kTaskEntries = 256;
+
+struct SweepError {
+    int code = 0;
+    int err_no = 0;
+    std::string path;
+};
+
+template <class Sink>
+int sweep_tree(const char* root_c, std::vector<typename Sink::Out>& out, SweepError* err)
+{
+    using Out = typename Sink::Out;
+    enum : uint8_t { kDropped = 0, kKept = 1, kLstatFailed = 2, kRefused = 3 };
+    struct Dir;
+    struct Item {
+        Out ent;
+        Dir* sub = nullptr;
+        int32_t err = 0;
+        uint8_t state = kDropped;
+    };
+    struct Dir {
+        std::string path;
+        std::vector<Item> items;
+        DIR* kept = nullptr;
+        std::atomic<int> chunks_left{0};
+        Dir* parent = nullptr;
+        size_t n_all = 0;
+        std::atomic<size_t> n_kept{0};
+        size_t first_all = 0, first_kept = 0;
+        ~Dir() { release(); }
+        void release() { if (kept) { closedir(kept); kept = nullptr; g_kept_dirs.fetch_sub(1); } }
+    };
+    struct Task { Dir* dir; uint32_t k0, k1; bool list; };
+    struct Found { std::vector<std::unique_ptr<Dir>> dirs; std::vector<Task> tasks; };
+
+    std::string root(root_c);
+    while (root.size() > 1 && root.back() == '/') root.pop_back();
+    const size_t rootlen = root.size();
+    const size_t base = out.size();
+    struct stat rst;
+    if (lstat(root.c_str(), &rst) != 0) {
+        *err = SweepError{0, errno, root};
+        return -1;
+    }
+    {
+        Out r;
+        Sink::path(r) = root;
+        const int f = Sink::finish(r, rootlen, rst);
+        if (f == 1) out.push_back(std::move(r));
+        else if (f != 0) { *err = SweepError{f, 0, root}; return -1; }
+    }
+    if (!S_ISDIR(rst.st_mode)) return 0;
+    const bool trace = getenv("SNAPHASH_TRACE_TREE") != nullptr;
+    const auto t0 = std::chrono::steady_clock::now();
+
+    auto stat_items = [rootlen](Dir& d, size_t k0, size_t k1, int dfd, Found& found) {
+        size_t kept = 0;
+        for (size_t k = k0; k < k1; ++k) {
+            Item& it = d.items[k];
+            const std::string& p = Sink::path(it.ent);
+            struct stat st;
+            if ((dfd >= 0 ? fstatat(dfd, p.c_str() + d.path.size() + 1, &st, AT_SYMLINK_NOFOLLOW) : lstat(p.c_str(), &st)) != 0) {
+                it.state = kLstatFailed;
+                it.err = errno;
+                continue;
+            }
+            if (S_ISDIR(st.st_mode)) {
+                found.dirs.emplace_back(new Dir());
+                it.sub = found.dirs.back().get();
+                it.sub->path = p;
+                it.sub->parent = &d;
+                found.tasks.push_back(Task{it.sub, 0, 0, true});
+            }
+            const int f = Sink::finish(it.ent, rootlen, st);
+            it.state = f == 1 ? kKept : f == 0 ? kDropped : kRefused;
+            if (it.state == kRefused) it.err = f;
+            kept += f == 1;
+        }
+        d.n_kept.fetch_add(kept, std::memory_order_relaxed);
+    };
+    auto list_dir = [&stat_items, rootlen](Dir& d, Found& found) {
+        struct Open {
+            DIR* d;
+            ~Open() { if (d) closedir(d); }
+        } dd{opendir(d.path.c_str())};
+        if (!dd.d) {
+            d.items.resize(1);
+            d.n_all = 1;
+            Item& it = d.items[0];
+            Sink::path(it.ent) = d.path;
+            struct stat st;
+            if (lstat(d.path.c_str(), &st) != 0) { it.state = kLstatFailed; it.err = errno; return; }
+            const int f = Sink::finish(it.ent, rootlen, st);
+            it.state = f == 1 ? kKept : f == 0 ? kDropped : kRefused;
+            if (it.state == kRefused) it.err = f;
+            d.n_kept.store(f == 1);
+            return;
+        }
+        const size_t plen = d.path.size() + 1;
+        while (struct dirent* de = readdir(dd.d)) {
+            if (!strcmp(de->d_name, ".") || !strcmp(de->d_name, "..")) continue;
+            d.items.emplace_back();
+            std::string& p = Sink::path(d.items.back().ent);
+            p.reserve(plen + strlen(de->d_name));
+            p = d.path;
+            p += '/';
+            p += de->d_name;
+        }
+        std::sort(d.items.begin(), d.items.end(), [plen](const Item& a, const Item& b) {
+            return Sink::path(a.ent).compare(plen, std::string::npos, Sink::path(b.ent), plen, std::string::npos) < 0;
+        });
+        const size_t n = d.items.size(), first = std::min(n, kTaskEntries);
+        d.n_all = n;
+        if (n > first) {
+            int chunks = 0;
+            for (size_t k = first; k < n; k += kTaskEntries, ++chunks)
+                found.tasks.push_back(Task{&d, (uint32_t)k, (uint32_t)std::min(n, k + kTaskEntries), false});
+            d.chunks_left.store(chunks);
+        }
+        stat_items(d, 0, first, dirfd(dd.d), found);
+        if (n > first) {
+            if (g_kept_dirs.fetch_add(1) < kKeptDirs) { d.kept = dd.d; dd.d = nullptr; }
+            else g_kept_dirs.fetch_sub(1);
+        }
+    };
+
+    std::vector<std::unique_ptr<Dir>> dirs;
+    dirs.emplace_back(new Dir());
+    dirs[0]->path = root;
+    std::vector<Task> tasks{Task{dirs[0].get(), 0, 0, true}};
+    std::vector<size_t> round_end{1};
+    unsigned max_threads = 1;
+    while (!tasks.empty()) {
+        size_t weight = 0;
+        for (const Task& t : tasks) weight += t.list ? 1 : 4;
+        const unsigned T = (unsigned)std::max<size_t>(1, std::min<size_t>(std::min(16u, usable_cpus()), weight / 4));
+        max_threads = std::max(max_threads, T);
+        std::vector<Found> found(T);
+        std::atomic<size_t> next{0};
+        run_on_threads(T, [&](unsigned t) {
+            for (;;) {
+                const size_t i = next.fetch_add(1);
+                if (i >= tasks.size()) return;
+                const Task& tk = tasks[i];
+                if (tk.list) { list_dir(*tk.dir, found[t]); continue; }
+                stat_items(*tk.dir, tk.k0, tk.k1, tk.dir->kept ? dirfd(tk.dir->kept) : -1, found[t]);
+                if (tk.dir->chunks_left.fetch_sub(1) == 1) tk.dir->release();
+            }
+        });
+        tasks.clear();
+        for (Found& f : found) {
+            for (auto& d : f.dirs) dirs.push_back(std::move(d));
+            tasks.insert(tasks.end(), f.tasks.begin(), f.tasks.end());
+        }
+        round_end.push_back(dirs.size());
+    }
+    const auto t1 = std::chrono::steady_clock::now();
+
+    for (size_t i = dirs.size(); i-- > 1;) {
+        Dir& d = *dirs[i];
+        d.parent->n_all += d.n_all;
+        d.parent->n_kept.fetch_add(d.n_kept.load(std::memory_order_relaxed), std::memory_order_relaxed);
+    }
+    dirs[0]->first_all = 1;
+    dirs[0]->first_kept = out.size();
+    const size_t n_out = out.size() + dirs[0]->n_kept.load();
+    out.resize(n_out);
+    const auto t2 = std::chrono::steady_clock::now();
+    struct Bad { size_t at_all = (size_t)-1, at_kept = 0; const Item* it = nullptr; };
+    std::vector<Bad> bads(max_threads);
+    for (size_t r = 0; r + 1 < round_end.size(); ++r) {
+        const size_t lo = r ? round_end[r - 1] : 0, hi = round_end[r];
+        const unsigned T = (unsigned)std::max<size_t>(1, std::min<size_t>(max_threads, (hi - lo) / 4));
+        std::atomic<size_t> next{lo};
+        run_on_threads(T, [&](unsigned t) {
+            for (;;) {
+                const size_t i = next.fetch_add(1);
+                if (i >= hi) return;
+                Dir& d = *dirs[i];
+                size_t at_all = d.first_all, at_kept = d.first_kept;
+                for (Item& it : d.items) {
+                    if (it.state >= kLstatFailed && at_all < bads[t].at_all) bads[t] = Bad{at_all, at_kept, &it};
+                    if (it.state == kKept) out[at_kept++] = std::move(it.ent);
+                    ++at_all;
+                    if (it.sub) {
+                        it.sub->first_all = at_all;
+                        it.sub->first_kept = at_kept;
+                        at_all += it.sub->n_all;
+                        at_kept += it.sub->n_kept.load(std::memory_order_relaxed);
+                    }
+                }
+            }
+        });
+    }
+    if (trace) {
+        const auto t3 = std::chrono::steady_clock::now();
+        auto ms = [](auto a, auto b) { return std::chrono::duration<double, std::milli>(b - a).count(); };
+        fprintf(stderr, "snaphash walk: %zu directories in %zu rounds on up to %u threads (readdir + sort + Lstat + records) %.2f ms, "
+                        "counts of %zu entries summed and room made %.2f ms, %zu kept moved into Walk's order %.2f ms\n",
+                dirs.size(), round_end.size() - 1, max_threads, ms(t0, t1), 1 + dirs[0]->n_all, ms(t1, t2), n_out - base, ms(t2, t3));
+    }
+    Bad bad;
+    for (const Bad& b : bads)
+        if (b.at_all < bad.at_all) bad = b;
+    if (!bad.it) return 0;
+    *err = SweepError{bad.it->state == kRefused ? bad.it->err : 0, bad.it->state == kRefused ? 0 : bad.it->err, Sink::path(bad.it->ent)};
+    out.resize(bad.at_kept);
+    return -1;
+}
+
+}
```
